# CEED/Laghos

Measured on AMD Instinct MI355X. Metric: Mdofs×steps/s on 3D Sedov -pa (Q3/Q2), higher is better.
Workload: dtype f64; 1 GPU; 3D Sedov -p 1 -m cube01_hex -rs 4 -ok 3 -ot 2 -pa (32^3 elements, E0/2^dim = 0.125); transport=none (one rank), elements=32768, h1_dofs=2738019, l2_dofs=884736, quad_points_per_element=216, rk_stages_executed=1300, ode=RK4, parallelism=elements1x1x1, zones_per_gpu=32x32x32

## Files before the change

include/laghos_hip.h:

```cpp
#ifndef LAGHOS_HIP_H
#define LAGHOS_HIP_H

#ifdef __cplusplus
extern "C" {
#endif

#define LGH_OK 0
#define LGH_ERR_ARG 1
#define LGH_ERR_UNSUPPORTED 2
#define LGH_ERR_HIP 3
#define LGH_ERR_COMM 4

#define LGH_SPACE_H1 0
#define LGH_SPACE_L2 1

typedef struct lgh_ctx lgh_ctx;

typedef struct lgh_config
{
   int dim, NE;
   int D1D, Q1D, L1D;
   int N;
   const int *h1_map;
   const double *B_h1;
   const double *G_h1;
   const double *B_l2;
   const double *weights;
   const double *gamma;
   int ess_count[3];
   const int *ess[3];
   const double *owner;
   int use_viscosity, use_vorticity;
   double cfl;
   int order_v;
   int device;
   void *stream;
} lgh_config;

const char *lgh_last_error(void);
const char *lgh_version(void);

int lgh_create(const lgh_config *cfg, lgh_ctx **out);
int lgh_destroy(lgh_ctx *ctx);
int lgh_sync(lgh_ctx *ctx);
void *lgh_stream(lgh_ctx *ctx);

double *lgh_qdata_stressJinvT(lgh_ctx *ctx);
double *lgh_qdata_Jac0inv(lgh_ctx *ctx);
double *lgh_qdata_rho0DetJ0w(lgh_ctx *ctx);
double *lgh_mass_D(lgh_ctx *ctx);
int lgh_mass_data_form(lgh_ctx *ctx, int *form);
int lgh_jac0inv_form(lgh_ctx *ctx, int *compact);
int lgh_mass_data_changed(lgh_ctx *ctx);
double *lgh_mass_diag(lgh_ctx *ctx);
int lgh_set_h0(lgh_ctx *ctx, double h0);
int lgh_get_h0(lgh_ctx *ctx, double *h0);
int lgh_set_dt_est(lgh_ctx *ctx, double dt_est);
int lgh_get_dt_est(lgh_ctx *ctx, double *dt_est);

int lgh_setup_rho0detj0(lgh_ctx *ctx, const double *x0, const double *rho0_l2,
                        const double *rho0_q, double *volume);

int lgh_force_mult(lgh_ctx *ctx, const double *x_l2, double *y_h1);
int lgh_force_mult_transpose(lgh_ctx *ctx, const double *v_h1, double *y_l2);

int lgh_mass_set_essential_tdofs(lgh_ctx *ctx, int comp);
int lgh_mass_eliminate_rhs(lgh_ctx *ctx, double *b);
int lgh_mass_mult(lgh_ctx *ctx, int space, const double *x, double *y);
int lgh_mass_mult_full(lgh_ctx *ctx, int space, const double *x, double *y);

int lgh_cg_solve(lgh_ctx *ctx, int space, const double *b, double *x, double rel_tol,
                 int max_iter, int *iters);
int lgh_l2_mass_solve_local(lgh_ctx *ctx, const double *b, double *x);

int lgh_qupdate(lgh_ctx *ctx, const double *S);
int lgh_qupdate_set_tiny_grad(lgh_ctx *ctx, double tiny_grad);
int lgh_qupdate_discard(lgh_ctx *ctx, int *mode, double *C_F);
int lgh_set_fused_forces(lgh_ctx *ctx, int on);
int lgh_qupdate_store_stress(lgh_ctx *ctx, int on);
int lgh_qupdate_stores_stress(lgh_ctx *ctx, int *on);
int lgh_qupdate_form(lgh_ctx *ctx, int *form);
int lgh_reset_quadrature_data(lgh_ctx *ctx);
int lgh_fused_force_mult(lgh_ctx *ctx, double *y_h1);
int lgh_fused_force_mult_transpose(lgh_ctx *ctx, double *y_l2);
int lgh_fused_force_e(lgh_ctx *ctx, double *y_e);
int lgh_quadrature_generation(lgh_ctx *ctx, unsigned long *gen, int *f1_valid, int *ftv_valid);
int lgh_get_fused_forces(lgh_ctx *ctx, int *f1, int *ftv);

int lgh_solve_velocity(lgh_ctx *ctx, const double *S, double *dS_dt, const double *one_l2,
                       double *rhs_h1, double *work_B, double rel_tol, int max_iter,
                       int *h1_iters);
int lgh_solve_energy(lgh_ctx *ctx, const double *S, const double *v_h1, double *dS_dt,
                     double *e_rhs, const double *e_source, double rel_tol, int max_iter,
                     int *l2_iters);
int lgh_solve_energy_begin(lgh_ctx *ctx, const double *S, const double *v_h1, double *dS_dt,
                           double *e_rhs, const double *e_source, double rel_tol, int max_iter);
int lgh_solve_energy_end(lgh_ctx *ctx, int *l2_iters);
int lgh_energy_lockstep_stats(lgh_ctx *ctx, long out[4]);

int lgh_vec_set(lgh_ctx *ctx, double *y, double a, long n);
int lgh_vec_copy(lgh_ctx *ctx, double *y, const double *x, long n);
int lgh_vec_axpby_pair(lgh_ctx *ctx, double *z1, double a1, const double *x1, double b1, double *z2, double a2, const double *x2, double b2,
                       const double *y, long n);
int lgh_vec_axpby(lgh_ctx *ctx, double *z, double a, const double *x, double b,
                  const double *y, long n);
int lgh_vec_dot(lgh_ctx *ctx, const double *x, const double *y, long n, double *result);
int lgh_vec_fingerprint(lgh_ctx *ctx, const double *x, long n, unsigned long long offset, unsigned long long out[2]);
int lgh_vec_fingerprint_shape(lgh_ctx *ctx, const double *x, long n, long out[4]);
int lgh_fingerprint_host(const void *words, long n, unsigned long long offset, unsigned long long out[2]);

int lgh_set_velocity_source(lgh_ctx *ctx, const double *accel_h1);

int lgh_tg_source_2d(lgh_ctx *ctx, const double *S, double *e_source);

int lgh_internal_energy(lgh_ctx *ctx, const double *e_l2, double *result);
int lgh_kinetic_energy(lgh_ctx *ctx, const double *v_h1, double *result);

int lgh_sedov_setup(int dim, double gamma, double rho0, double blast_energy, double omega, double par[21]);
int lgh_sedov_shock(const double par[21], double t, double shock[6]);
int lgh_sedov_eval_point(const double par[21], double t, double r, double *rho, double *v, double *P);
int lgh_sedov_eval(lgh_ctx *ctx, const double par[21], double t, long n, const double *r, double *rho, double *v,
                   double *P);
int lgh_compute_density(lgh_ctx *ctx, const double *x_h1, double *rho_l2);
int lgh_sedov_density_error(lgh_ctx *ctx, const double *x_h1, const double *rho_l2, const double par[21], double t,
                            const double origin[3], int n1d, const double *weights, const double *B_h1,
                            const double *G_h1, const double *B_l2, double *err2);

int lgh_sample_fields(lgh_ctx *ctx, const double *S, const double *rho_l2 ,
                      int R1, const double *B_h1_lat ,
                      const double *B_l2_lat ,
                      double *x_out, double *v_out, double *e_out, double *rho_out, double *p_out);

int lgh_sample_derived(lgh_ctx *ctx, const double *S, int R1, const double *B_h1_lat ,
                       const double *G_h1_lat , const double *B_l2_lat ,
                       double *detj_out, double *gradv_out, double *div_out, double *vort_out, double *cs_out);

int lgh_sample_faces(lgh_ctx *ctx, const double *S, const double *rho_l2 , int R1,
                     const double *B_h1_lat , const double *G_h1_lat ,
                     const double *B_l2_lat , int nfaces, const int *faces ,
                     double *x_out, double *v_out, double *e_out, double *rho_out, double *p_out, double *detj_out,
                     double *gradv_out, double *div_out, double *vort_out, double *cs_out, double *an_out);
int lgh_sample_faces_fpb(lgh_ctx *ctx, int R1, int *fpb);
int lgh_mesh_boundary_faces_host(int dim, int NE, int N, int D1D, const int *h1_map, int *faces_out, int *nfaces);

#define LGH_DIAG_ZONE_COUNT 17
#define LGH_DIAG_COUNT 20
int lgh_diagnostics_zones(lgh_ctx *ctx, const double *S, double *zone_out);
int lgh_diagnostics(lgh_ctx *ctx, const double *S, double out[LGH_DIAG_COUNT]);

#define LGH_PROFILE_COLS 10
#define LGH_PROFILE_MAX_BINS 4096
typedef struct lgh_profile_spec {
   int axis;
   int nbins;
   double lo, hi;
   double origin[3];
} lgh_profile_spec;
int lgh_profile(lgh_ctx *ctx, const double *S, const lgh_profile_spec *spec, double *out, long *n_excluded);

#define LGH_MAP_COLS 11
#define LGH_MAP_MAX_CELLS (1 << 20)
typedef struct lgh_map_spec {
   int n[3];
   double lo[3], hi[3];
} lgh_map_spec;
int lgh_map(lgh_ctx *ctx, const double *S, const lgh_map_spec *spec,
            double *out , long *n_excluded);

int lgh_get_timers(lgh_ctx *ctx, double t[4], long c[3]);
int lgh_reset_timers(lgh_ctx *ctx);
int lgh_enable_timers(lgh_ctx *ctx, int on);

#define LGH_KERNEL_MASS_CG_H1 0
#define LGH_KERNEL_CG_UPDATE_H1 1
#define LGH_KERNEL_QUPDATE 2
#define LGH_KERNEL_FORCE_MULT 3
#define LGH_KERNEL_FORCE_MULT_T 4
#define LGH_KERNEL_MASS_CG_L2 5
#define LGH_KERNEL_HALO 6
#define LGH_KERNEL_ALLREDUCE 7
#define LGH_KERNEL_SAMPLE 8
#define LGH_KERNEL_FINGERPRINT 9
#define LGH_KERNEL_DIAG 10
#define LGH_KERNEL_PROFILE 11
#define LGH_KERNEL_DERIVED 12
#define LGH_KERNEL_MAP 13
#define LGH_KERNEL_FACES 14
int lgh_ktime_begin(lgh_ctx *ctx, int which, int max_samples);
int lgh_ktime_end(lgh_ctx *ctx, int *launches, double *mean_seconds);
int lgh_table_symmetry(lgh_ctx *ctx, int *h1, int *l2);
int lgh_k1_form(lgh_ctx *ctx, int *form);
int lgh_l2_mass_form(lgh_ctx *ctx, int *form, int *compact);
int lgh_vcg_layout_stats(lgh_ctx *ctx, long out[4]);

int lgh_mesh_order(lgh_ctx *ctx, long out[8]);
int lgh_mesh_order_host(int dim, int NE, int N, int D1D, const int *h1_map, int *zorder, int *nnum, long out[8]);

int lgh_comm_unique_id(char id_out[128]);
int lgh_comm_init(lgh_ctx *ctx, int nranks, int rank, const char unique_id[128]);
int lgh_comm_unique_id_shm(char id_out[128]);
int lgh_comm_set_neighbors(lgh_ctx *ctx, int n_nbr, const int *nbr_rank, const int *nbr_count,
                           const int *const *nbr_nodes);
int lgh_comm_stats(lgh_ctx *ctx, int *n_neighbours, long *max_nodes_per_neighbour, long *shared_nodes, int *all_pairs,
                   int *second_channel);
int lgh_groups_to_neighbors(int my_rank, int N, int n_groups, const int *group_off, const int *group_ranks,
                            const int *group_master, const int *ldof_off, const int *ldofs, double *owner,
                            int *n_nbr, int *nbr_rank, int *nbr_count, int cap_nbr, int *nbr_nodes, long cap_nodes);
int lgh_halo_sum(lgh_ctx *ctx, double *v_h1, int ncomp);
int lgh_allreduce(lgh_ctx *ctx, double *value, int op);

int lgh_force_mult_E(lgh_ctx *ctx, const double *sJit, const double *x_E, double *y_E);
int lgh_force_mult_transpose_E(lgh_ctx *ctx, const double *sJit, const double *v_E, double *y_E);
int lgh_mass_apply_E(lgh_ctx *ctx, int space, const double *x_E, double *y_E);
int lgh_test_vcg_k1(lgh_ctx *ctx, const double *r, const double *d_old, const double rz[3], const double rz_prev[3],
                    int first, double *y_E, double den[3]);
int lgh_test_vcg_merged_faces(lgh_ctx *ctx, unsigned char *mask, long *n_merged);
int lgh_test_vcg_k2(lgh_ctx *ctx, int it, const double *y_E, double *r, double *d, double *x, const double den[3],
                    const double rz[3], const double rz_prev[3], const double alpha_prev[3], double rz_out[3],
                    int *deferred_x);
int lgh_test_exact_sum(lgh_ctx *ctx, int mode, long n, int G, int E, const double *scale, const double *v,
                       const long long *w_in, long long *w_out, double *d_out, int *i_out);
int lgh_test_set_rank(lgh_ctx *ctx, int nranks, int rank);
int lgh_test_halo_pack(lgh_ctx *ctx, const double *v_h1, int ncomp, double *sendbuf_out);
int lgh_test_halo_combine(lgh_ctx *ctx, const double *recvbuf_in, double *v_h1, int ncomp);
int lgh_test_word_peers(lgh_ctx *ctx, int nwords, long *capacity_words);
int lgh_test_rccl_self_sendrecv(lgh_ctx *ctx, int n, double *max_abs_diff);
int lgh_test_eig(lgh_ctx *ctx, int dim, int n, const double *A, double *lambda, double *vec);
int lgh_test_sqrt(lgh_ctx *ctx, int n, const double *x, double *y);
int lgh_test_singular(lgh_ctx *ctx, int dim, int n, const double *A, double *sv_min);

#ifdef __cplusplus
}
#endif
#endif
```

laghos_amd/_lib.py:

```python
import ctypes
import os

_HERE = os.path.dirname(os.path.abspath(__file__))
LIB_PATH = os.path.join(_HERE, "liblaghos_hip.so")

c_dp = ctypes.c_void_p
c_int_p = ctypes.POINTER(ctypes.c_int)
c_dbl_p = ctypes.POINTER(ctypes.c_double)


class LghConfig(ctypes.Structure):
    _fields_ = [
        ("dim", ctypes.c_int), ("NE", ctypes.c_int),
        ("D1D", ctypes.c_int), ("Q1D", ctypes.c_int), ("L1D", ctypes.c_int),
        ("N", ctypes.c_int),
        ("h1_map", c_int_p),
        ("B_h1", c_dbl_p), ("G_h1", c_dbl_p), ("B_l2", c_dbl_p),
        ("weights", c_dbl_p), ("gamma", c_dbl_p),
        ("ess_count", ctypes.c_int * 3),
        ("ess", c_int_p * 3),
        ("owner", c_dbl_p),
        ("use_viscosity", ctypes.c_int), ("use_vorticity", ctypes.c_int),
        ("cfl", ctypes.c_double),
        ("order_v", ctypes.c_int),
        ("device", ctypes.c_int),
        ("stream", ctypes.c_void_p),
    ]


class LghProfileSpec(ctypes.Structure):
    _fields_ = [("axis", ctypes.c_int), ("nbins", ctypes.c_int), ("lo", ctypes.c_double), ("hi", ctypes.c_double),
                ("origin", ctypes.c_double * 3)]


class LghMapSpec(ctypes.Structure):
    _fields_ = [("n", ctypes.c_int * 3), ("lo", ctypes.c_double * 3), ("hi", ctypes.c_double * 3)]


_I, _D, _P, _L = ctypes.c_int, ctypes.c_double, ctypes.c_void_p, ctypes.c_long
SYMBOLS = {
    "lgh_last_error": (ctypes.c_char_p, []),
    "lgh_version": (ctypes.c_char_p, []),
    "lgh_create": (_I, [ctypes.POINTER(LghConfig), ctypes.POINTER(_P)]),
    "lgh_destroy": (_I, [_P]),
    "lgh_sync": (_I, [_P]),
    "lgh_stream": (_P, [_P]),
    "lgh_qdata_stressJinvT": (_P, [_P]),
    "lgh_qdata_Jac0inv": (_P, [_P]),
    "lgh_qdata_rho0DetJ0w": (_P, [_P]),
    "lgh_mass_D": (_P, [_P]),
    "lgh_mass_diag": (_P, [_P]),
    "lgh_set_h0": (_I, [_P, _D]),
    "lgh_get_h0": (_I, [_P, c_dbl_p]),
    "lgh_set_dt_est": (_I, [_P, _D]),
    "lgh_get_dt_est": (_I, [_P, c_dbl_p]),
    "lgh_setup_rho0detj0": (_I, [_P, _P, _P, _P, c_dbl_p]),
    "lgh_force_mult": (_I, [_P, _P, _P]),
    "lgh_force_mult_transpose": (_I, [_P, _P, _P]),
    "lgh_mass_set_essential_tdofs": (_I, [_P, _I]),
    "lgh_mass_eliminate_rhs": (_I, [_P, _P]),
    "lgh_mass_mult": (_I, [_P, _I, _P, _P]),
    "lgh_mass_mult_full": (_I, [_P, _I, _P, _P]),
    "lgh_cg_solve": (_I, [_P, _I, _P, _P, _D, _I, c_int_p]),
    "lgh_l2_mass_solve_local": (_I, [_P, _P, _P]),
    "lgh_qupdate": (_I, [_P, _P]),
    "lgh_solve_velocity": (_I, [_P, _P, _P, _P, _P, _P, _D, _I, c_int_p]),
    "lgh_solve_energy": (_I, [_P, _P, _P, _P, _P, _P, _D, _I, c_int_p]),
    "lgh_solve_energy_begin": (_I, [_P, _P, _P, _P, _P, _P, _D, _I]),
    "lgh_tg_source_2d": (_I, [_P, _P, _P]),
    "lgh_set_velocity_source": (_I, [_P, _P]),
    "lgh_solve_energy_end": (_I, [_P, c_int_p]),
    "lgh_vec_set": (_I, [_P, _P, _D, _L]),
    "lgh_vec_copy": (_I, [_P, _P, _P, _L]),
    "lgh_vec_axpby": (_I, [_P, _P, _D, _P, _D, _P, _L]),
    "lgh_vec_axpby_pair": (_I, [_P, _P, _D, _P, _D, _P, _D, _P, _D, _P, _L]),
    "lgh_vec_dot": (_I, [_P, _P, _P, _L, c_dbl_p]),
    "lgh_vec_fingerprint": (_I, [_P, _P, _L, ctypes.c_ulonglong, ctypes.POINTER(ctypes.c_ulonglong)]),
    "lgh_vec_fingerprint_shape": (_I, [_P, _P, _L, ctypes.POINTER(ctypes.c_long)]),
    "lgh_fingerprint_host": (_I, [_P, _L, ctypes.c_ulonglong, ctypes.POINTER(ctypes.c_ulonglong)]),
    "lgh_internal_energy": (_I, [_P, _P, c_dbl_p]),
    "lgh_kinetic_energy": (_I, [_P, _P, c_dbl_p]),
    "lgh_sedov_setup": (_I, [_I, _D, _D, _D, _D, c_dbl_p]),
    "lgh_sedov_shock": (_I, [c_dbl_p, _D, c_dbl_p]),
    "lgh_sedov_eval_point": (_I, [c_dbl_p, _D, _D, c_dbl_p, c_dbl_p, c_dbl_p]),
    "lgh_sedov_eval": (_I, [_P, c_dbl_p, _D, _L, _P, _P, _P, _P]),
    "lgh_compute_density": (_I, [_P, _P, _P]),
    "lgh_sedov_density_error": (_I, [_P, _P, _P, c_dbl_p, _D, c_dbl_p, _I, c_dbl_p, c_dbl_p, c_dbl_p, c_dbl_p, c_dbl_p]),
    "lgh_sample_fields": (_I, [_P, _P, _P, _I, c_dbl_p, c_dbl_p, _P, _P, _P, _P, _P]),
    "lgh_sample_derived": (_I, [_P, _P, _I, c_dbl_p, c_dbl_p, c_dbl_p, _P, _P, _P, _P, _P]),
    "lgh_sample_faces": (_I, [_P, _P, _P, _I, c_dbl_p, c_dbl_p, c_dbl_p, _I, c_int_p] + [_P] * 11),
    "lgh_sample_faces_fpb": (_I, [_P, _I, ctypes.POINTER(_I)]),
    "lgh_mesh_boundary_faces_host": (_I, [_I, _I, _I, _I, c_int_p, c_int_p, ctypes.POINTER(_I)]),
    "lgh_diagnostics_zones": (_I, [_P, _P, _P]),
    "lgh_diagnostics": (_I, [_P, _P, c_dbl_p]),
    "lgh_profile": (_I, [_P, _P, ctypes.POINTER(LghProfileSpec), c_dbl_p, ctypes.POINTER(ctypes.c_long)]),
    "lgh_map": (_I, [_P, _P, ctypes.POINTER(LghMapSpec), c_dbl_p, ctypes.POINTER(ctypes.c_long)]),
    "lgh_get_timers": (_I, [_P, c_dbl_p, ctypes.POINTER(ctypes.c_long)]),
    "lgh_reset_timers": (_I, [_P]),
    "lgh_enable_timers": (_I, [_P, _I]),
    "lgh_ktime_begin": (_I, [_P, _I, _I]),
    "lgh_ktime_end": (_I, [_P, c_int_p, c_dbl_p]),
    "lgh_table_symmetry": (_I, [_P, c_int_p, c_int_p]),
    "lgh_k1_form": (_I, [_P, c_int_p]),
    "lgh_l2_mass_form": (_I, [_P, c_int_p, c_int_p]),
    "lgh_vcg_layout_stats": (_I, [_P, ctypes.POINTER(ctypes.c_long)]),
    "lgh_energy_lockstep_stats": (_I, [_P, ctypes.POINTER(ctypes.c_long)]),
    "lgh_mesh_order": (_I, [_P, ctypes.POINTER(ctypes.c_long)]),
    "lgh_mesh_order_host": (_I, [_I, _I, _I, _I, c_int_p, c_int_p, c_int_p, ctypes.POINTER(ctypes.c_long)]),
    "lgh_mass_data_form": (_I, [_P, c_int_p]),
    "lgh_jac0inv_form": (_I, [_P, c_int_p]),
    "lgh_mass_data_changed": (_I, [_P]),
    "lgh_comm_stats": (_I, [_P, c_int_p, ctypes.POINTER(ctypes.c_long), ctypes.POINTER(ctypes.c_long), c_int_p, c_int_p]),
    "lgh_qupdate_set_tiny_grad": (_I, [_P, _D]),
    "lgh_qupdate_discard": (_I, [_P, c_int_p, c_dbl_p]),
    "lgh_set_fused_forces": (_I, [_P, _I]),
    "lgh_qupdate_store_stress": (_I, [_P, _I]),
    "lgh_qupdate_stores_stress": (_I, [_P, c_int_p]),
    "lgh_qupdate_form": (_I, [_P, c_int_p]),
    "lgh_reset_quadrature_data": (_I, [_P]),
    "lgh_fused_force_mult": (_I, [_P, _P]),
    "lgh_fused_force_mult_transpose": (_I, [_P, _P]),
    "lgh_fused_force_e": (_I, [_P, _P]),
    "lgh_quadrature_generation": (_I, [_P, ctypes.POINTER(ctypes.c_ulong), c_int_p, c_int_p]),
    "lgh_get_fused_forces": (_I, [_P, c_int_p, c_int_p]),
    "lgh_comm_unique_id": (_I, [ctypes.c_char_p]),
    "lgh_comm_unique_id_shm": (_I, [ctypes.c_char_p]),
    "lgh_comm_init": (_I, [_P, _I, _I, ctypes.c_char_p]),
    "lgh_comm_set_neighbors": (_I, [_P, _I, c_int_p, c_int_p, ctypes.POINTER(c_int_p)]),
    "lgh_groups_to_neighbors": (_I, [_I, _I, _I, c_int_p, c_int_p, c_int_p, c_int_p, c_int_p, c_dbl_p, c_int_p, c_int_p,
                                     c_int_p, _I, c_int_p, _L]),
    "lgh_halo_sum": (_I, [_P, _P, _I]),
    "lgh_allreduce": (_I, [_P, c_dbl_p, _I]),
    "lgh_force_mult_E": (_I, [_P, _P, _P, _P]),
    "lgh_force_mult_transpose_E": (_I, [_P, _P, _P, _P]),
    "lgh_mass_apply_E": (_I, [_P, _I, _P, _P]),
    "lgh_test_vcg_k1": (_I, [_P, _P, _P, c_dbl_p, c_dbl_p, _I, _P, c_dbl_p]),
    "lgh_test_vcg_merged_faces": (_I, [_P, _P, ctypes.POINTER(ctypes.c_long)]),
    "lgh_test_vcg_k2": (_I, [_P, _I, _P, _P, _P, _P, c_dbl_p, c_dbl_p, c_dbl_p, c_dbl_p, c_dbl_p, ctypes.POINTER(ctypes.c_int)]),
    "lgh_test_exact_sum": (_I, [_P, _I, _L, _I, _I, c_dbl_p, c_dbl_p, ctypes.POINTER(ctypes.c_longlong),
                                ctypes.POINTER(ctypes.c_longlong), c_dbl_p, c_int_p]),
    "lgh_test_set_rank": (_I, [_P, _I, _I]),
    "lgh_test_word_peers": (_I, [_P, _I, ctypes.POINTER(ctypes.c_long)]),
    "lgh_test_halo_pack": (_I, [_P, _P, _I, _P]),
    "lgh_test_halo_combine": (_I, [_P, _P, _P, _I]),
    "lgh_test_rccl_self_sendrecv": (_I, [_P, _I, c_dbl_p]),
    "lgh_test_eig": (_I, [_P, _I, _I, _P, _P, _P]),
    "lgh_test_singular": (_I, [_P, _I, _I, _P, _P]),
    "lgh_test_sqrt": (_I, [_P, _I, _P, _P]),
}

_lib = None


def _preload_torch_hip():
    try:
        import torch
    except Exception:
        pass


def load():
    global _lib
    if _lib is None:
        _preload_torch_hip()
        if not os.path.exists(LIB_PATH):
            raise RuntimeError(
                f"{LIB_PATH} is missing: build it with `python -c 'import __graft_entry__ as g; "
                "g.build()'` (hipcc --offload-arch=gfx950).  There is no CPU fallback.")
        lib = ctypes.CDLL(LIB_PATH)
        for name, (res, args) in SYMBOLS.items():
            fn = getattr(lib, name)
            fn.restype = res
            fn.argtypes = args
        _lib = lib
    return _lib


class LghError(RuntimeError):
    pass


def check(rc):
    if rc != 0:
        raise LghError(f"laghos_hip error {rc}: {load().lgh_last_error().decode()}")
```

laghos_amd/context.py:

```python
import ctypes

import numpy as np
import torch

from . import _lib
from ._lib import LghConfig, check


def _np_i32(a):
    return np.ascontiguousarray(a, dtype=np.int32)


def _np_f64(a):
    return np.ascontiguousarray(a, dtype=np.float64)


def _ptr(t):
    assert t.is_cuda and t.dtype == torch.float64 and t.is_contiguous()
    return ctypes.c_void_p(t.data_ptr())


def _dbl(a):
    assert isinstance(a, np.ndarray) and a.dtype == np.float64 and a.flags.c_contiguous
    return a.ctypes.data_as(_lib.c_dbl_p)
# ... 339 lines not shown
        return out

    def mass_data_form(self):
        f = ctypes.c_int(-1)
        check(self.lib.lgh_mass_data_form(self.h, ctypes.byref(f)))
        return "rank1" if f.value == 1 else "stored"

    def jac0inv_form(self):
        f = ctypes.c_int(-1)
        check(self.lib.lgh_jac0inv_form(self.h, ctypes.byref(f)))
        return "compact" if f.value == 1 else "stored"

    def qupdate_store_stress(self, on):
        check(self.lib.lgh_qupdate_store_stress(self.h, int(bool(on))))

    def set_fused_forces(self, on):
        check(self.lib.lgh_set_fused_forces(self.h, 1 if on else 0))

    def reset_quadrature_data(self):
        check(self.lib.lgh_reset_quadrature_data(self.h))

    def fused_force_mult(self, y_h1):
        return self.lib.lgh_fused_force_mult(self.h, _ptr(y_h1)) == 0

    def fused_force_e(self, y_e):
        return self.lib.lgh_fused_force_e(self.h, _ptr(y_e)) == 0

    def fused_force_mult_transpose(self, y_l2):
        return self.lib.lgh_fused_force_mult_transpose(self.h, _ptr(y_l2)) == 0

    def quadrature_generation(self):
        g, a, b = ctypes.c_ulong(0), ctypes.c_int(-1), ctypes.c_int(-1)
        check(self.lib.lgh_quadrature_generation(self.h, ctypes.byref(g), ctypes.byref(a), ctypes.byref(b)))
        return g.value, a.value, b.value

    def solve_velocity(self, S, dS, one, rhs, work, rel_tol, max_iter):
        it = ctypes.c_int(0)
        check(self.lib.lgh_solve_velocity(self.h, _ptr(S), _ptr(dS), _ptr(one) if one is not None else None, _ptr(rhs), _ptr(work),
                                          rel_tol, max_iter, ctypes.byref(it)))
        return it.value

    def solve_energy(self, S, v, dS, e_rhs, rel_tol, max_iter, e_source=None):
        it = ctypes.c_int(0)
        check(self.lib.lgh_solve_energy(self.h, _ptr(S), _ptr(v), _ptr(dS), _ptr(e_rhs),
                                        _ptr(e_source) if e_source is not None else None,
                                        rel_tol, max_iter, ctypes.byref(it)))
        return it.value

    def set_velocity_source(self, accel):
        check(self.lib.lgh_set_velocity_source(self.h, _ptr(accel) if accel is not None else None))

    def tg_source_2d(self, S, out):
        check(self.lib.lgh_tg_source_2d(self.h, _ptr(S), _ptr(out)))

    def compute_density(self, x, rho_l2):
        check(self.lib.lgh_compute_density(self.h, _ptr(x), _ptr(rho_l2)))

    def sedov_eval(self, par, t, r, rho, v, P):
        check(self.lib.lgh_sedov_eval(self.h, _dbl(par), float(t), r.numel(), _ptr(r), _ptr(rho), _ptr(v), _ptr(P)))

    def sedov_density_error(self, x, rho_l2, par, t, origin, weights, B_h1, G_h1, B_l2):
        import numpy as np
        w = np.ascontiguousarray(weights, dtype=np.float64)
        tabs = [np.ascontiguousarray(a, dtype=np.float64).ravel() for a in (B_h1, G_h1, B_l2)]
        org = np.zeros(3)
        org[:len(origin)] = origin
        out = ctypes.c_double()
        check(self.lib.lgh_sedov_density_error(self.h, _ptr(x), _ptr(rho_l2), _dbl(par), float(t), _dbl(org),
                                               int(w.size), _dbl(w), _dbl(tabs[0]), _dbl(tabs[1]), _dbl(tabs[2]),
                                               ctypes.byref(out)))
        return out.value

    def sample_fields(self, S, rho_l2, B_h1_lat, B_l2_lat, x=None, v=None, e=None, rho=None, p=None):
        Bh = _np_f64(np.asarray(B_h1_lat).T.reshape(-1))
        Bl = _np_f64(np.asarray(B_l2_lat).T.reshape(-1))
        R1 = int(np.asarray(B_h1_lat).shape[0])
        opt = lambda t: _ptr(t) if t is not None else None
        check(self.lib.lgh_sample_fields(self.h, _ptr(S), opt(rho_l2), R1, _dbl(Bh), _dbl(Bl), opt(x), opt(v), opt(e), opt(rho),
                                         opt(p)))

    def sample_derived(self, S, B_h1_lat, G_h1_lat, B_l2_lat, detj=None, grad_v=None, div_v=None, vorticity=None, sound_speed=None):
        Bh = _np_f64(np.asarray(B_h1_lat).T.reshape(-1))
        Gh = _np_f64(np.asarray(G_h1_lat).T.reshape(-1))
        Bl = _np_f64(np.asarray(B_l2_lat).T.reshape(-1))
        R1 = int(np.asarray(B_h1_lat).shape[0])
        opt = lambda t: _ptr(t) if t is not None else None
        check(self.lib.lgh_sample_derived(self.h, _ptr(S), R1, _dbl(Bh), _dbl(Gh), _dbl(Bl), opt(detj), opt(grad_v), opt(div_v), opt(vorticity),
                                          opt(sound_speed)))

    def sample_faces(self, S, rho_l2, B_h1_lat, G_h1_lat, B_l2_lat, faces, x=None, v=None, e=None, rho=None, p=None, detj=None, grad_v=None,
                     div_v=None, vorticity=None, sound_speed=None, area_normal=None):
        tab = lambda T: None if T is None else _np_f64(np.asarray(T).T.reshape(-1))
        Bh, Gh, Bl = tab(B_h1_lat), tab(G_h1_lat), tab(B_l2_lat)
        R1 = int(np.asarray(next(T for T in (B_h1_lat, G_h1_lat, B_l2_lat) if T is not None)).shape[0])
        f = np.ascontiguousarray(np.asarray(faces, dtype=np.int32).reshape(-1))
        assert f.size % 2 == 0
        opt = lambda t: _ptr(t) if t is not None else None
        dbl = lambda a: _dbl(a) if a is not None else None
        fp = f.ctypes.data_as(ctypes.POINTER(ctypes.c_int)) if f.size else None
        check(self.lib.lgh_sample_faces(self.h, _ptr(S), opt(rho_l2), R1, dbl(Bh), dbl(Gh), dbl(Bl), f.size // 2, fp, opt(x), opt(v), opt(e),
                                        opt(rho), opt(p), opt(detj), opt(grad_v), opt(div_v), opt(vorticity), opt(sound_speed), opt(area_normal)))

    def faces_per_block(self, R1):
        n = ctypes.c_int(-1)
        check(self.lib.lgh_sample_faces_fpb(self.h, int(R1), ctypes.byref(n)))
        return n.value

    def boundary_faces(self):
        return boundary_faces_host(self.dim, self.NE, self.N, self.D1D, self._keep["h1"])

    def diagnostics_zones(self, S, out):
        assert out.numel() == DIAG_ZONE_COUNT * self.NE
        check(self.lib.lgh_diagnostics_zones(self.h, _ptr(S), _ptr(out)))

    def diagnostics(self, S, raw=False):
        out = np.full(DIAG_COUNT, np.nan)
        check(self.lib.lgh_diagnostics(self.h, _ptr(S), _dbl(out)))
        return out if raw else diagnostics_dict(out)

    def profile(self, S, axis, nbins, lo, hi, origin=None):
        from ._lib import LghProfileSpec
        spec = LghProfileSpec()
        spec.axis, spec.nbins, spec.lo, spec.hi = int(PROFILE_AXES.get(axis, axis)), int(nbins), float(lo), float(hi)
        o = np.zeros(3) if origin is None else np.asarray(origin, dtype=np.float64).reshape(-1)
        for k in range(min(3, o.size)):
            spec.origin[k] = float(o[k])
        n_rows = max(0, min(int(nbins), PROFILE_MAX_BINS)) + 2
        rows = np.full((n_rows, len(PROFILE_COLS)), np.nan)
        n_excl = ctypes.c_long(-1)
        check(self.lib.lgh_profile(self.h, _ptr(S), ctypes.byref(spec), _dbl(rows), ctypes.byref(n_excl)))
        return profile_dict(rows, n_excl.value, spec.lo, spec.hi)

    def map(self, S, cells, lo, hi):
        from ._lib import LghMapSpec
        n, a, b, n_rows = map_spec(cells, lo, hi)
        spec = LghMapSpec()
        for k in range(3):
            spec.n[k], spec.lo[k], spec.hi[k] = n[k], a[k], b[k]
        rows = np.full((n_rows, len(MAP_COLS)), np.nan)
        n_excl = ctypes.c_long(-1)
        check(self.lib.lgh_map(self.h, _ptr(S), ctypes.byref(spec), _dbl(rows), ctypes.byref(n_excl)))
        return map_dict(rows, n_excl.value, self.dim, n, a, b)

    def solve_energy_begin(self, S, v, dS, e_rhs, rel_tol, max_iter, e_source=None):
        check(self.lib.lgh_solve_energy_begin(self.h, _ptr(S), _ptr(v), _ptr(dS), _ptr(e_rhs),
                                              _ptr(e_source) if e_source is not None else None,
                                              rel_tol, max_iter))

    def solve_energy_end(self):
        it = ctypes.c_int(0)
        check(self.lib.lgh_solve_energy_end(self.h, ctypes.byref(it)))
        return it.value

    def vec_axpby(self, z, a, x, b, y):
        check(self.lib.lgh_vec_axpby(self.h, _ptr(z), a, _ptr(x), b, _ptr(y), z.numel()))

    def vec_axpby_pair(self, z1, a1, x1, b1, z2, a2, x2, b2, y):
        check(self.lib.lgh_vec_axpby_pair(self.h, _ptr(z1), a1, _ptr(x1), b1, _ptr(z2), a2, _ptr(x2), b2, _ptr(y), z1.numel()))

    def vec_copy(self, y, x):
        check(self.lib.lgh_vec_copy(self.h, _ptr(y), _ptr(x), y.numel()))

    def vec_dot(self, x, y):
        v = ctypes.c_double()
        check(self.lib.lgh_vec_dot(self.h, _ptr(x), _ptr(y), x.numel(), ctypes.byref(v)))
        return v.value

    def fingerprint(self, t, offset=0):
        out = (ctypes.c_ulonglong * 2)()
        check(self.lib.lgh_vec_fingerprint(self.h, _ptr(t), t.numel(), int(offset), out))
        return int(out[0]), int(out[1])

    def fingerprint_shape(self, t):
        out = (ctypes.c_long * 4)()
        check(self.lib.lgh_vec_fingerprint_shape(self.h, _ptr(t), t.numel(), out))
        return tuple(out)

    def internal_energy(self, e):
        v = ctypes.c_double()
        check(self.lib.lgh_internal_energy(self.h, _ptr(e), ctypes.byref(v)))
        return v.value

    def kinetic_energy(self, vel):
        v = ctypes.c_double()
        check(self.lib.lgh_kinetic_energy(self.h, _ptr(vel), ctypes.byref(v)))
        return v.value

    def timers(self):
        t = (ctypes.c_double * 4)()
        c = (ctypes.c_long * 3)()
        check(self.lib.lgh_get_timers(self.h, t, c))
        return dict(cgH1=t[0], cgL2=t[1], force=t[2], qdata=t[3], H1iter=c[0], L2iter=c[1],
                    quad_tstep=c[2])

    def reset_timers(self):
        check(self.lib.lgh_reset_timers(self.h))

    def enable_timers(self, on):
        check(self.lib.lgh_enable_timers(self.h, int(on)))

    def force_mult_E(self, sJit, xE, yE):
        check(self.lib.lgh_force_mult_E(self.h, _ptr(sJit), _ptr(xE), _ptr(yE)))

    def force_mult_transpose_E(self, sJit, vE, yE):
        check(self.lib.lgh_force_mult_transpose_E(self.h, _ptr(sJit), _ptr(vE), _ptr(yE)))

    def mass_apply_E(self, space, xE, yE):
        check(self.lib.lgh_mass_apply_E(self.h, space, _ptr(xE), _ptr(yE)))

    def test_eig(self, dim, A, lam, vec):
        check(self.lib.lgh_test_eig(self.h, dim, lam.numel(), _ptr(A), _ptr(lam), _ptr(vec)))

    def test_singular(self, dim, A, sv):
        check(self.lib.lgh_test_singular(self.h, dim, sv.numel(), _ptr(A), _ptr(sv)))

    def test_sqrt(self, x, y):
        check(self.lib.lgh_test_sqrt(self.h, y.numel(), _ptr(x), _ptr(y)))

    def comm_init(self, nranks, rank, unique_id):
        check(self.lib.lgh_comm_init(self.h, nranks, rank, unique_id))

    def comm_set_neighbors(self, nbr_rank, nbr_nodes):
        n = len(nbr_rank)
        ranks = _np_i32(nbr_rank) if n else np.zeros(1, np.int32)
        counts = _np_i32([len(x) for x in nbr_nodes]) if n else np.zeros(1, np.int32)
        lists = [_np_i32(x) for x in nbr_nodes]
        ip = ctypes.POINTER(ctypes.c_int)
        arr = (ip * max(n, 1))(*[l.ctypes.data_as(ip) for l in lists])
        check(self.lib.lgh_comm_set_neighbors(self.h, n, ranks.ctypes.data_as(ip), counts.ctypes.data_as(ip), arr))

    def test_word_peers(self, nwords):
        cap = ctypes.c_long(-1)
        check(self.lib.lgh_test_word_peers(self.h, nwords, ctypes.byref(cap)))
        return cap.value

    def test_set_rank(self, nranks, rank):
        check(self.lib.lgh_test_set_rank(self.h, nranks, rank))

    def test_halo_pack(self, v, ncomp, out):
        check(self.lib.lgh_test_halo_pack(self.h, _ptr(v), ncomp, _ptr(out)))

    def test_halo_combine(self, inp, v, ncomp):
        check(self.lib.lgh_test_halo_combine(self.h, _ptr(inp), _ptr(v), ncomp))

    def halo_sum(self, v, ncomp):
        check(self.lib.lgh_halo_sum(self.h, _ptr(v), ncomp))

    def allreduce(self, value, op=0):
        v = ctypes.c_double(value)
        check(self.lib.lgh_allreduce(self.h, ctypes.byref(v), op))
        return v.value


def unique_id():
    buf = ctypes.create_string_buffer(128)
    check(_lib.load().lgh_comm_unique_id(buf))
    return buf.raw
```

laghos_amd/csrc/lgh_api.hip:

```cpp
#include <cstdarg>
#include <cstdlib>
#include <cmath>
#include <algorithm>
#include <limits>

#include "lgh_comm_transport.hpp"
#include "lgh_vcg.hpp"

#include <atomic>
#include <chrono>
#include <dlfcn.h>

namespace lgh
{

static thread_local char g_err[512] = "";
void set_error(const char *fmt, ...)
{
   va_list ap;
   va_start(ap, fmt);
   vsnprintf(g_err, sizeof(g_err), fmt, ap);
   va_end(ap);
}

// ... 689 lines not shown
int lgh_quadrature_generation(lgh_ctx *c, unsigned long *gen, int *f1_valid, int *ftv_valid)
{
   LGH_CHECK_ARG(c && gen && f1_valid && ftv_valid);
   *gen = c->qgen;
   *f1_valid = c->fused_f1_valid;
   *ftv_valid = c->fused_ftv_valid;
   return LGH_OK;
}
double *lgh_qdata_Jac0inv(lgh_ctx *c) { return c->Jac0inv; }
double *lgh_qdata_rho0DetJ0w(lgh_ctx *c) { return c->rho0DetJ0w; }
double *lgh_mass_D(lgh_ctx *c)
{
   c->mass_rank1 = -1;
   c->mass_gen++;
   return c->massD;
}
int lgh_mass_data_form(lgh_ctx *c, int *form)
{
   LGH_CHECK_ARG(c && form);
   if (c->dim == 1) { *form = 0; return LGH_OK; }
   const double *Dq, *Se;
   int dqs;
   int rc = mass_data(c, &Dq, &dqs, &Se);
   if (rc) { return rc; }
   *form = (c->mass_rank1 == 1) ? 1 : 0;
   return LGH_OK;
}
int lgh_mass_data_changed(lgh_ctx *c)
{
   LGH_CHECK_ARG(c);
   c->mass_rank1 = -1;
   c->mass_gen++;
   if (c->dim == 1) { return mass_changed_1d(c); }
   return mass_assemble_diag(c);
}
double *lgh_mass_diag(lgh_ctx *c) { return c->diagV; }
int lgh_set_h0(lgh_ctx *c, double h0) { LGH_CHECK_ARG(c); c->h0 = h0; return LGH_OK; }
int lgh_get_h0(lgh_ctx *c, double *h0) { LGH_CHECK_ARG(c && h0); *h0 = c->h0; return LGH_OK; }

int lgh_set_dt_est(lgh_ctx *c, double v)
{
   LGH_CHECK_ARG(c);
   hipLaunchKernelGGL(dt_est_set_k, dim3(1), dim3(256), 0, c->stream, c->dt_est_dev, v);
   LGH_HIP_CHECK(hipGetLastError());
   return LGH_OK;
}
int lgh_get_dt_est(lgh_ctx *c, double *v)
{
   LGH_CHECK_ARG(c && v);
   const unsigned long long token = ++c->look_token;
   hipLaunchKernelGGL(dt_est_fold_k, dim3(1), dim3(256), 0, c->stream, c->dt_est_dev, c->dev_flags + 4, c->host_pinned_dev + kPinDt, token);
   LGH_HIP_CHECK(hipGetLastError());
   {
      const int rc = host_wait_token(c, (volatile unsigned long long *)(c->host_pinned + kPinDtToken), token);
      if (rc) { return rc; }
   }
   *v = c->host_pinned[kPinDt];
   if (*(const int *)(c->host_pinned + kPinDtFlag) != 0)
   {
      LGH_HIP_CHECK(hipMemsetAsync(c->dev_flags + 4, 0, sizeof(int), c->stream));
      set_error("lgh_solve_energy was given a velocity other than the state's while the stress was kept in registers "
                "(lgh_qupdate_store_stress(ctx, 0)): its right-hand side is NaN");
      return LGH_ERR_ARG;
   }
   return LGH_OK;
}

int lgh_setup_rho0detj0(lgh_ctx *c, const double *x0, const double *rho0_l2, const double *rho0_q,
                        double *volume)
{
   LGH_CHECK_ARG(c && x0 && rho0_l2 && rho0_q && volume);
   invalidate_fused(c);
   c->mass_rank1 = -1;
   c->mass_gen++;
   int rc = (c->dim == 1) ? setup_1d(c, x0, rho0_l2, rho0_q, volume)
                          : setup_rho0detj0(c, x0, rho0_l2, rho0_q, volume);
   if (rc) { return rc; }
   if (c->dim != 1) { rc = mass_assemble_diag(c); }
   if (rc == LGH_OK) { c->setup_done = 1; }
   return rc;
}

int lgh_force_mult(lgh_ctx *c, const double *x_l2, double *y_h1)
{
   LGH_CHECK_ARG(c && x_l2 && y_h1);
   int rc = stress_on_hand(c, "lgh_force_mult");
   if (rc) { return rc; }
   if (c->dim == 1) { return force_mult_1d(c, x_l2, y_h1); }
   kt_begin(c, LGH_KERNEL_FORCE_MULT);
   rc = force_mult_E(c, c->stressJinvT, x_l2, c->YE);
   kt_end(c, LGH_KERNEL_FORCE_MULT);
   if (rc) { return rc; }
   rc = h1_transpose_gather(c, c->dim, c->YE, y_h1);
   if (rc) { return rc; }
   if (c->multi != 0) { rc = halo_sum(c, y_h1, c->dim); }
   return rc;
}
int lgh_force_mult_transpose(lgh_ctx *c, const double *v_h1, double *y_l2)
{
   LGH_CHECK_ARG(c && v_h1 && y_l2);
   const int rc0 = stress_on_hand(c, "lgh_force_mult_transpose");
   if (rc0) { return rc0; }
   if (c->dim == 1) { return force_mult_t_1d(c, v_h1, y_l2); }
   kt_begin(c, LGH_KERNEL_FORCE_MULT_T);
   const int rc = force_mult_t_L(c, c->stressJinvT, v_h1, y_l2);
   kt_end(c, LGH_KERNEL_FORCE_MULT_T);
   return rc;
}

int lgh_mass_set_essential_tdofs(lgh_ctx *c, int comp)
{
   LGH_CHECK_ARG(c && comp >= -1 && comp < c->dim);
   c->cur_ess = comp;
   return LGH_OK;
}
int lgh_mass_eliminate_rhs(lgh_ctx *c, double *b)
{
   LGH_CHECK_ARG(c && b);
   if (c->cur_ess < 0) { return LGH_OK; }
   return vec_zero_list(c, b, c->ess[c->cur_ess], c->ess_count[c->cur_ess]);
}
int lgh_mass_mult(lgh_ctx *c, int space, const double *x, double *y)
{
   LGH_CHECK_ARG(c && x && y && (space == LGH_SPACE_H1 || space == LGH_SPACE_L2));
   if (c->dim == 1) { return mass_apply_1d(c, space, x, y, true); }
   return space == LGH_SPACE_H1 ? mass_apply_h1(c, x, y, true) : mass_apply_l2(c, x, y);
}
int lgh_mass_mult_full(lgh_ctx *c, int space, const double *x, double *y)
{
   LGH_CHECK_ARG(c && x && y && (space == LGH_SPACE_H1 || space == LGH_SPACE_L2));
   if (c->dim == 1) { return mass_apply_1d(c, space, x, y, false); }
   return space == LGH_SPACE_H1 ? mass_apply_h1(c, x, y, false) : mass_apply_l2(c, x, y);
}

int lgh_cg_solve(lgh_ctx *c, int space, const double *b, double *x, double rel_tol, int max_iter,
                 int *iters)
{
   LGH_CHECK_ARG(c && b && x && (space == LGH_SPACE_H1 || space == LGH_SPACE_L2));
   if (c->dim == 1) { return cg_1d(c, space, b, x, rel_tol, max_iter, iters, false); }
   return cg_solve(c, space, b, x, rel_tol, max_iter, iters, false);
}

int lgh_l2_mass_solve_local(lgh_ctx *c, const double *b, double *x)
{
   LGH_CHECK_ARG(c && b && x);
   if (c->dim != 1)
   {
      set_error("lgh_l2_mass_solve_local: the zone-local energy solve belongs to the 1D (full-assembly) path; 2D/3D run the energy CG");
      return LGH_ERR_UNSUPPORTED;
   }
   return l2_solve_local_1d(c, b, x);
}

int lgh_qupdate(lgh_ctx *c, const double *S)
{
   LGH_CHECK_ARG(c && S);
   RoctxRange range("QUpdate-UpdateQuadratureData");
   timer_start(c);
   kt_begin(c, LGH_KERNEL_QUPDATE);
   int rc = (c->dim == 1) ? qupdate_1d(c, S) : qupdate(c, S);
   kt_end(c, LGH_KERNEL_QUPDATE);
   timer_stop(c, 3);
   c->timers.c[2] += c->NE;
   return rc;
}

__global__ void __launch_bounds__(256) not_all_ones_k(const double *x, const long n, int *flag)
{
   const long i = (long)blockIdx.x * blockDim.x + threadIdx.x;
   if (i < n && x[i] != 1.0) { *flag = 1; }
}
static bool is_the_one_vector(lgh_ctx *c, const double *one_l2)
{
   if (!one_l2) { return true; }
   int *flag = c->dev_flags + 1;
   if (hipMemsetAsync(flag, 0, sizeof(int), c->stream) != hipSuccess) { return false; }
   hipLaunchKernelGGL(not_all_ones_k, dim3(ceil_div(c->L2V, 256)), dim3(256), 0, c->stream, one_l2, (long)c->L2V, flag);
   int h = 1;
   if (hipMemcpyAsync(&h, flag, sizeof(int), hipMemcpyDeviceToHost, c->stream) != hipSuccess) { return false; }
   if (hipStreamSynchronize(c->stream) != hipSuccess) { return false; }
   return h == 0;
}
static int one_vector(lgh_ctx *c, const double *one_l2, const double **out)
{
   if (one_l2) { *out = one_l2; return LGH_OK; }
   if (!c->ones_l2)
   {
      LGH_PASS(c->ones_l2.alloc((size_t)c->L2V));
      const int rc = vec_set(c, c->ones_l2, 1.0, c->L2V);
      if (rc) { return rc; }
   }
   *out = c->ones_l2;
   return LGH_OK;
}

int lgh_solve_velocity(lgh_ctx *c, const double *S, double *dS_dt, const double *one_l2,
                       double *rhs_h1, double *work_B, double rel_tol, int max_iter, int *h1_iters)
{
   LGH_CHECK_ARG(c && S && dS_dt && rhs_h1 && work_B);
   const int dim = c->dim, N = c->N;
   double *dv = dS_dt + c->H1V;
   int rc;
   if (dim == 1)
   {
      LGH_CHECK_ARG(!c->accel_src);
      const double *ones = nullptr;
      rc = one_vector(c, one_l2, &ones);
      if (rc) { return rc; }
      rc = stress_on_hand(c, "lgh_solve_velocity");
      if (rc) { return rc; }
      return solve_velocity_1d(c, ones, dv, rhs_h1, rel_tol, max_iter, h1_iters);
   }
   if (!c->timers.enabled && !c->accel_src && vcg_fused_init_ok(c))
   {
      const double *force_E = c->YE;
      if (c->force_e_q && c->fused_f1_valid && is_the_one_vector(c, one_l2)) { force_E = c->force_e_q; }
      else
      {
         const double *ones = nullptr;
         rc = one_vector(c, one_l2, &ones);
         if (rc) { return rc; }
         rc = stress_on_hand(c, "lgh_solve_velocity (F.1 of a vector other than one, or of changed quadrature data)");
         if (rc) { return rc; }
         kt_begin(c, LGH_KERNEL_FORCE_MULT);
         rc = force_mult_E(c, c->stressJinvT, ones, c->YE);
         kt_end(c, LGH_KERNEL_FORCE_MULT);
         if (rc) { return rc; }
      }
      int its[3] = {0, 0, 0};
      RoctxRange range("SolveVelocity-CGVMass");
      rc = vcg_solve(c, rhs_h1, dv, rel_tol, max_iter, its, force_E);
      if (rc) { return rc; }
      for (int cc = 0; cc < dim; cc++)
      {
         c->timers.c[0] += its[cc];
         if (h1_iters) { *h1_iters += its[cc]; }
      }
      c->cur_ess = dim - 1;
      return LGH_OK;
   }
   rc = vec_set(c, dv, 0.0, c->H1V);
   if (rc) { return rc; }
   {
   RoctxRange range("SolveVelocity-ForcePA");
   timer_start(c);
   if (c->force_e_q && c->fused_f1_valid && is_the_one_vector(c, one_l2))
   {
      rc = h1_transpose_gather(c, c->dim, c->force_e_q, rhs_h1);
      if (rc == LGH_OK && c->multi != 0) { rc = halo_sum(c, rhs_h1, c->dim); }
   }
   else
   {
      const double *ones = nullptr;
      rc = one_vector(c, one_l2, &ones);
      if (rc == LGH_OK) { rc = lgh_force_mult(c, ones, rhs_h1); }
   }
   timer_stop(c, 2);
   }
   if (rc) { return rc; }
   rc = vec_neg_inplace(c, rhs_h1, c->H1V);
   if (rc) { return rc; }
   if (c->accel_src)
   {
      for (int cc = 0; cc < dim; cc++)
      {
         rc = mass_apply_h1(c, c->accel_src + (size_t)cc * N, work_B, false);
         if (rc) { return rc; }
         rc = vec_axpby(c, rhs_h1 + (size_t)cc * N, 1.0, rhs_h1 + (size_t)cc * N, 1.0, work_B, N);
         if (rc) { return rc; }
      }
   }
   {
      for (int cc = 0; cc < dim; cc++)
      {
         rc = vec_zero_list(c, rhs_h1 + (size_t)cc * N, c->ess[cc], c->ess_count[cc]);
         if (rc) { return rc; }
      }
      int its[3] = {0, 0, 0};
      RoctxRange range("SolveVelocity-CGVMass");
      timer_start(c);
      rc = vcg_solve(c, rhs_h1, dv, rel_tol, max_iter, its);
      if (rc == LGH_OK)
      {
         timer_stop(c, 0);
         for (int cc = 0; cc < dim; cc++)
         {
            c->timers.c[0] += its[cc];
            if (h1_iters) { *h1_iters += its[cc]; }
         }
         c->cur_ess = dim - 1;
         return LGH_OK;
      }
      if (rc != LGH_ERR_UNSUPPORTED) { return rc; }
   }
   for (int cc = 0; cc < dim; cc++)
   {
      LGH_HIP_CHECK(hipMemcpyAsync(work_B, rhs_h1 + (size_t)cc * N, sizeof(double) * N,
                                   hipMemcpyDeviceToDevice, c->stream));
      rc = lgh_mass_set_essential_tdofs(c, cc);
      if (rc) { return rc; }
      rc = lgh_mass_eliminate_rhs(c, work_B);
      if (rc) { return rc; }
      int it = 0;
      timer_start(c);
      rc = cg_solve(c, LGH_SPACE_H1, work_B, dv + (size_t)cc * N, rel_tol, max_iter, &it, true);
      timer_stop(c, 0);
      if (rc) { return rc; }
      c->timers.c[0] += it;
      if (h1_iters) { *h1_iters += it; }
   }
   return LGH_OK;
}

int lgh_vec_set(lgh_ctx *c, double *y, double a, long n) { LGH_CHECK_ARG(c && y); return vec_set(c, y, a, n); }
int lgh_vec_copy(lgh_ctx *c, double *y, const double *x, long n)
{
   LGH_CHECK_ARG(c && y && x);
   LGH_HIP_CHECK(hipMemcpyAsync(y, x, sizeof(double) * n, hipMemcpyDeviceToDevice, c->stream));
   return LGH_OK;
}
int lgh_vec_axpby(lgh_ctx *c, double *z, double a, const double *x, double b, const double *y, long n)
{
   LGH_CHECK_ARG(c && z && x && y);
   return vec_axpby(c, z, a, x, b, y, n);
}
int lgh_vec_axpby_pair(lgh_ctx *c, double *z1, double a1, const double *x1, double b1, double *z2, double a2, const double *x2, double b2,
                       const double *y, long n)
{
   LGH_CHECK_ARG(c && z1 && x1 && z2 && x2 && y && n >= 0);
   {
      auto overlap = [n](const double *p, const double *q) { return p < q + n && q < p + n; };
      LGH_CHECK_ARG(!overlap(z1, z2) && !overlap(z1, x2) && !overlap(z1, y));
      LGH_CHECK_ARG(!overlap(z2, y) && !overlap(z2, x1) && (z2 == x2 || !overlap(z2, x2)) && (z1 == x1 || !overlap(z1, x1)));
   }
   return vec_axpby_pair(c, z1, a1, x1, b1, z2, a2, x2, b2, y, n);
}
int lgh_vec_dot(lgh_ctx *c, const double *x, const double *y, long n, double *result)
{
   LGH_CHECK_ARG(c && x && y && result);
   int rc = vec_dot(c, x, y, nullptr, n, c->scal + 1);
   if (rc) { return rc; }
   LGH_HIP_CHECK(hipMemcpyAsync(c->host_pinned + kPinDot, c->scal + 1, sizeof(double), hipMemcpyDeviceToHost, c->stream));
   LGH_HIP_CHECK(hipStreamSynchronize(c->stream));
   *result = c->host_pinned[kPinDot];
   return LGH_OK;
}

int lgh_set_velocity_source(lgh_ctx *c, const double *accel_h1)
{
   LGH_CHECK_ARG(c);
   if (accel_h1)
   {
      const int rc = no_1d(c, "lgh_set_velocity_source");
      if (rc) { return rc; }
   }
   c->accel_src = accel_h1;
   return LGH_OK;
}

int lgh_tg_source_2d(lgh_ctx *c, const double *S, double *e_source)
{
   LGH_CHECK_ARG(c && S && e_source);
   const int rc = no_1d(c, "lgh_tg_source_2d");
   if (rc) { return rc; }
   return tg_source_2d(c, S, e_source);
}

int lgh_internal_energy(lgh_ctx *c, const double *e_l2, double *result)
{
   LGH_CHECK_ARG(c && e_l2 && result);
   if (c->dim == 1) { return energy_1d(c, 0, e_l2, result); }
   return interp_energy(c, 0, e_l2, result);
}
int lgh_kinetic_energy(lgh_ctx *c, const double *v_h1, double *result)
{
   LGH_CHECK_ARG(c && v_h1 && result);
   if (c->dim == 1) { return energy_1d(c, 1, v_h1, result); }
   return interp_energy(c, 1, v_h1, result);
}

int lgh_get_timers(lgh_ctx *c, double t[4], long n[3])
{
   LGH_CHECK_ARG(c && t && n);
   for (int i = 0; i < 4; i++) { t[i] = c->timers.t[i]; }
   for (int i = 0; i < 3; i++) { n[i] = c->timers.c[i]; }
   return LGH_OK;
}
int lgh_reset_timers(lgh_ctx *c)
{
   LGH_CHECK_ARG(c);
   for (int i = 0; i < 4; i++) { c->timers.t[i] = 0; }
   for (int i = 0; i < 3; i++) { c->timers.c[i] = 0; }
   return LGH_OK;
}
int lgh_enable_timers(lgh_ctx *c, int on)
{
   LGH_CHECK_ARG(c);
   c->timers.enabled = on != 0;
   return LGH_OK;
}

int lgh_ktime_begin(lgh_ctx *c, int which, int max_samples)
{
   LGH_CHECK_ARG(c && which >= 0 && max_samples > 0);
   if (!c->ktime) { c->ktime.reset(new KTime()); }
   KTime *k = c->ktime.get();
   while ((int)k->ev.size() < 2 * max_samples)
   {
      hipEvent_t e;
      LGH_HIP_CHECK(hipEventCreate(&e));
      k->ev.push_back(e);
   }
   k->which = which;
   k->max = max_samples;
   k->n = 0;
   return LGH_OK;
}
int lgh_ktime_end(lgh_ctx *c, int *launches, double *mean_seconds)
{
   LGH_CHECK_ARG(c && launches && mean_seconds && c->ktime);
   KTime *k = c->ktime.get();
   LGH_HIP_CHECK(hipStreamSynchronize(c->stream));
   double tot = 0.0;
   for (int i = 0; i < k->n; i++)
   {
      float ms = 0.f;
      LGH_HIP_CHECK(hipEventElapsedTime(&ms, k->ev[2 * i], k->ev[2 * i + 1]));
      tot += 1e-3 * ms;
   }
   *launches = k->n;
   *mean_seconds = k->n ? tot / k->n : 0.0;
   k->which = -1;
   return LGH_OK;
}

int lgh_set_fused_forces(lgh_ctx *c, int on)
{
   LGH_CHECK_ARG(c);
   if (c->fused_forces_off == (on ? 0 : 1)) { return LGH_OK; }
   c->fused_forces_off = on ? 0 : 1;
   invalidate_fused(c);
   return LGH_OK;
}

int lgh_get_fused_forces(lgh_ctx *c, int *f1, int *ftv)
{
   LGH_CHECK_ARG(c && f1 && ftv);
   *f1 = (c->force_e_q && !c->fused_forces_off) ? 1 : 0;
   *ftv = (c->erhs_q && !c->fused_forces_off) ? 1 : 0;
   return LGH_OK;
}

int lgh_qupdate_set_tiny_grad(lgh_ctx *c, double tiny_grad)
{
   LGH_CHECK_ARG(c);
   c->q_tiny_grad = tiny_grad;
   return LGH_OK;
}

int lgh_table_symmetry(lgh_ctx *c, int *h1, int *l2)
{
   LGH_CHECK_ARG(c && h1 && l2);
   *h1 = c->b_h1_sym;
   *l2 = c->b_l2_sym;
   return LGH_OK;
// ... 100 lines not shown
```

laghos_amd/csrc/lgh_common.hpp:

```cpp
#pragma once
#include <hip/hip_runtime.h>

#include <algorithm>
#include <cstdint>
#include <cstdio>
#include <cstring>
#include <memory>
#include <string>
#include <vector>

#include "../../include/laghos_hip.h"

namespace lgh
{

void set_error(const char *fmt, ...);

#define LGH_HIP_CHECK(expr)                                                              \
   do                                                                                    \
   {                                                                                     \
      hipError_t e_ = (expr);                                                            \
      if (e_ != hipSuccess)                                                              \
      {                                                                                  \
         lgh::set_error("HIP error %s at %s:%d: %s", hipGetErrorName(e_), __FILE__,      \
// ... 7 lines not shown
   {                                                                                     \
      if (!(cond))                                                                       \
      {                                                                                  \
         lgh::set_error("bad argument: %s (%s:%d)", #cond, __FILE__, __LINE__);          \
         return LGH_ERR_ARG;                                                             \
      }                                                                                  \
   } while (0)

#define LGH_PASS(call) do { const int rc_ = (call); if (rc_ != LGH_OK) { return rc_; } } while (0)

constexpr int kWave = 64;

template <typename T> struct DevPtr
{
   T *p = nullptr;
   DevPtr() = default;
   DevPtr(DevPtr &&o) noexcept : p(o.p) { o.p = nullptr; }
   DevPtr &operator=(DevPtr &&o) noexcept { std::swap(p, o.p); return *this; }
   ~DevPtr() { reset(); }
   operator T *() const { return p; }
   T *operator->() const { return p; }
   void reset() { if (p) { (void)hipFree(p); p = nullptr; } }
   int alloc(const size_t n, const bool zero = false)
   {
      reset();
      LGH_HIP_CHECK(hipMalloc((void **)&p, n * sizeof(T)));
      if (zero)
      {
         LGH_HIP_CHECK(hipMemset(p, 0, n * sizeof(T)));
         LGH_HIP_CHECK(hipStreamSynchronize(nullptr));
      }
      return LGH_OK;
   }
   int upload(const T *host, const size_t n)
   {
      const int rc = alloc(n);
      if (rc != LGH_OK) { return rc; }
      LGH_HIP_CHECK(hipMemcpy(p, host, n * sizeof(T), hipMemcpyHostToDevice));
      return LGH_OK;
   }
};
template <typename T> int ctx_buffer(DevPtr<T> &d, const size_t n, const T *src = nullptr)
{
   const int rc = d.alloc(std::max<size_t>(n, 1), !src);
   if (rc != LGH_OK || !src || !n) { return rc; }
   LGH_HIP_CHECK(hipMemcpy(d.p, src, n * sizeof(T), hipMemcpyHostToDevice));
   return LGH_OK;
}

struct CgScalars
{
   double rz;
   double rz_prev;
   double den;
   double r0;
   double nom0;
   double rel_tol2;
   int done;
   int iters;
   int first;
   int pad;
};

constexpr int kPinDoubles = 96;
constexpr int kPinResult = 0;
constexpr int kPinDot = 1;
constexpr int kPinReduceOut = 2, kPinReduceIn = 3;
constexpr int kPinDt = 8, kPinDtFlag = 9, kPinDtToken = 10;
constexpr int kPinVcg = 32;
constexpr int kPinVcgToken = 80;
static_assert(sizeof(CgScalars) <= kPinDt * sizeof(double) && kPinDtFlag == kPinDt + 1 && kPinDtToken == kPinDt + 2 && kPinDtToken < kPinVcg &&
              kPinVcgToken < kPinDoubles, "slots of the pinned block: disjoint, inside the allocation");

struct Timers
{
   bool enabled = true;
   hipEvent_t ev[2] = {nullptr, nullptr};
   Timers() = default;
   Timers(const Timers &) = delete;
   Timers &operator=(const Timers &) = delete;
   ~Timers() { for (hipEvent_t e : ev) { if (e) { (void)hipEventDestroy(e); } } }
   double t[4] = {0, 0, 0, 0};
   long c[3] = {0, 0, 0};
};

struct KTime
{
   int which = -1, max = 0, n = 0;
   std::vector<hipEvent_t> ev;
   KTime() = default;
   KTime(const KTime &) = delete;
   KTime &operator=(const KTime &) = delete;
   ~KTime() { for (hipEvent_t e : ev) { (void)hipEventDestroy(e); } }
};

struct Comm;
struct VcgScalars;
struct VcgAux;

struct MeshOrder
{
   bool structured = false, identity = true;
   int components = 0, extent[3] = {0, 0, 0};
   std::vector<int> zorder;
   std::vector<int> nnum;
   std::vector<int> ncaller;
   DevPtr<int> zorder_d, ncaller_d, nnum_d;
};

constexpr double kMassRank1Tol = 1e-12;
constexpr double kJac0Tol = 1e-12;

struct Switches
{
   int vcg_variant;
   int slab_wide, slab_exact, slab_merge, slab_defer, slab_ye_wide;
   int slab_dyn;
   int rz_limbs, kron_neb, fused_init;
   int k2p, k2_skip, k2_grid;
   long k2_node_weight;
   int order, order_multi;
   int comm2;
   int force_multi, halo_piggyback, halo_fused_pack, overlap, energy_lockstep, spin;
   int mass_sep, mass_kron, mass_rank1, l2_neb, l2_plane, l2_fused;
   double mass_rank1_tol;
   int q_form, q_ppt, q_swz, fused_ftv, fused_f1, b_sym, jac0_compact;
   int q_occ4;
   int q_discard;
   double q_tiny_grad;
   double jac0_tol;
   int profile_fold;
   int map_fold;
   int roctx, vcg_trace_phases, q_trace_call;
   std::string vcg_trace, q_trace;
};
Switches read_switches();

struct ScalarCg;
void cg_l2_free(ScalarCg *r);

struct EnergySolve
{
   enum Mode
   {
      Idle,
      Overlapped,
      Deferred,
      Lockstep
   };
   Mode mode = Idle;
   bool polled = false;
   int iters = 0;
   struct { const double *S, *v; double *dS, *e_rhs; const double *src; double tol; int maxit; } args = {};
};

struct CtxHandles
{
   int device = 0;
   hipStream_t stream = nullptr;
   bool own_stream = false;
   hipStream_t stream2 = nullptr;
   hipEvent_t ev_fork = nullptr, ev_join = nullptr;
   double *host_pinned = nullptr;
   double *host_pinned_dev = nullptr;
   CtxHandles() = default;
   CtxHandles(const CtxHandles &) = delete;
   CtxHandles &operator=(const CtxHandles &) = delete;
   ~CtxHandles();
};

}

struct lgh_ctx : lgh::CtxHandles
{
   lgh_ctx();
   ~lgh_ctx();
   lgh::Switches sw;
   int dim = 0, NE = 0, D1D = 0, Q1D = 0, L1D = 0, ND = 0, NQ = 0, NL = 0, N = 0, H1V = 0, L2V = 0;
   int kid = 0;
   bool visc = false, vort = false;
   double cfl = 0.0, h0 = 0.0, h1order = 0.0;
   double q_tiny_grad = 0.0;
   int q_discard = 0;
   double q_cF = 0.0;
   int on_stream2 = 0;
   std::unique_ptr<lgh::ScalarCg, void (*)(lgh::ScalarCg *)> l2run{nullptr, lgh::cg_l2_free};
   const double *accel_src = nullptr;
   lgh::EnergySolve energy;
   long ls_stats[3] = {0, 0, 0};

   lgh::DevPtr<double> B, G, Bl, W, gamma;
   lgh::DevPtr<int> h1map;
   lgh::DevPtr<int> t_off;
   lgh::DevPtr<int> t_idx;
   lgh::DevPtr<int> t_ell;
   int t_deg = 0;
   lgh::DevPtr<uint8_t> essmask[3];
   lgh::DevPtr<int> ess[3];
   int ess_count[3] = {0, 0, 0};
   lgh::DevPtr<double> owner;
   int cur_ess = -1;

   lgh::DevPtr<double> stressJinvT, Jac0inv, rho0DetJ0w, massD, diagV, dinvV;
   lgh::DevPtr<double> Jac0inv_soa;
   lgh::DevPtr<double> Jac0inv_e;
   int jac0_compact = 0;
   lgh::DevPtr<double> massS, ones_ne;
   lgh::DevPtr<double> M1h, M1l;
   lgh::DevPtr<double> w1d;
   int mass_rank1 = -1;
   lgh::DevPtr<double> dt_est_dev;
   lgh::DevPtr<double> erhs_q;
   lgh::DevPtr<double> v_snap;
   lgh::DevPtr<double> force_e_q;
   int fused_ftv_valid = 0, fused_f1_valid = 0;
   unsigned long qgen = 0;
   lgh::DevPtr<int> dev_flags;
   lgh::DevPtr<double> ones_l2;
   int stress_store = 1;
   int stress_current = 0;
   int fused_forces_off = 0;
   lgh::DevPtr<double> XE;
   lgh::DevPtr<double> YE;
   lgh::DevPtr<double> cg_r, cg_z, cg_d0, cg_d1, cg_y;
   lgh::DevPtr<double> partials;
   int part_stride = 0;
   lgh::DevPtr<unsigned int> tickets;
   lgh::DevPtr<lgh::CgScalars> cgs;
   lgh::DevPtr<double> scal;
   unsigned long long look_token = 0;

   lgh::DevPtr<lgh::VcgScalars> vcg_s;
   lgh::DevPtr<double> vcg_vec, vcg_partials;
   lgh::DevPtr<unsigned int> vcg_tickets;
   unsigned vcg_stride = 0;
   int vcg_last = 0;
   int vcg_grid = 0;
   int b_h1_sym = 0, b_l2_sym = 0;
   int ncu = 0;
   std::unique_ptr<lgh::VcgAux> vcg_aux;

   lgh::Timers timers;
   std::unique_ptr<lgh::KTime> ktime;
   int cg_last_iters[2][3] = {{0, 0, 0}, {0, 0, 0}};
   std::unique_ptr<lgh::Comm> comm;
   int nranks = 1, rank = 0;
   int multi = 0;
   lgh::DevPtr<unsigned long long> q_trace_dev;
   int q_trace_n = 0, q_trace_calls = 0;
   std::unique_ptr<lgh::MeshOrder> order;
   unsigned long mass_gen = 0;
   lgh::DevPtr<double> me_fac;
   int setup_done = 0;
   lgh::DevPtr<double> diag_dev;
   lgh::DevPtr<char> prof_dev;
   int prof_rows = 0;
   lgh::DevPtr<char> map_dev;
   int map_rows = 0;
   lgh::DevPtr<int> faces_dev;
   int faces_cap = 0;
   lgh::DevPtr<unsigned long long> fp_dev;
};

namespace lgh
{

template <int CTRL, int ROW_MASK>
__device__ __forceinline__ double dpp_f64(const double old, const double src)
{
   const int lo = __builtin_amdgcn_update_dpp(__double2loint(old), __double2loint(src), CTRL, ROW_MASK, 0xF, false);
   const int hi = __builtin_amdgcn_update_dpp(__double2hiint(old), __double2hiint(src), CTRL, ROW_MASK, 0xF, false);
   return __hiloint2double(hi, lo);
}
__device__ __forceinline__ double wave_bcast_f64(const double v, const int src_lane )
{
   const int lo = __builtin_amdgcn_readlane(__double2loint(v), src_lane);
   const int hi = __builtin_amdgcn_readlane(__double2hiint(v), src_lane);
   return __hiloint2double(hi, lo);
}
__device__ __forceinline__ double wave_sum(double v, const int lane, const int nact)
{
   (void)lane;
   v += dpp_f64<0x111, 0xF>(0.0, v);
   v += dpp_f64<0x112, 0xF>(0.0, v);
   v += dpp_f64<0x114, 0xF>(0.0, v);
   v += dpp_f64<0x118, 0xF>(0.0, v);
   v += dpp_f64<0x142, 0xA>(0.0, v);
   v += dpp_f64<0x143, 0xC>(0.0, v);
   return wave_bcast_f64(v, nact - 1);
}
__device__ __forceinline__ double wave_min(double v, const int lane, const int nact)
{
   (void)lane;
   v = fmin(v, dpp_f64<0x111, 0xF>(v, v));
   v = fmin(v, dpp_f64<0x112, 0xF>(v, v));
   v = fmin(v, dpp_f64<0x114, 0xF>(v, v));
   v = fmin(v, dpp_f64<0x118, 0xF>(v, v));
   v = fmin(v, dpp_f64<0x142, 0xA>(v, v));
   v = fmin(v, dpp_f64<0x143, 0xC>(v, v));
   return wave_bcast_f64(v, nact - 1);
}

__device__ __forceinline__ double uniform_f64(const double v)
{
   const int lo = __builtin_amdgcn_readfirstlane(__double2loint(v));
   const int hi = __builtin_amdgcn_readfirstlane(__double2hiint(v));
// ... 20 lines not shown
__device__ __forceinline__ void block_sum3(const double v0, const double v1, const double v2, double *red, double out[3])
{
   const int tid = threadIdx.x + blockDim.x * (threadIdx.y + blockDim.y * threadIdx.z);
   const int nthr = blockDim.x * blockDim.y * blockDim.z;
   const int lane = tid & 63, wid = tid >> 6, nw = (nthr + 63) >> 6;
   const int nact = min(64, nthr - (wid << 6));
   const double a0 = wave_sum(v0, lane, nact), a1 = wave_sum(v1, lane, nact), a2 = wave_sum(v2, lane, nact);
   __syncthreads();
   if (lane == 0)
   {
      red[3 * wid + 0] = a0;
      red[3 * wid + 1] = a1;
      red[3 * wid + 2] = a2;
   }
   __syncthreads();
   out[0] = out[1] = out[2] = 0.0;
   if (tid == 0)
   {
      for (int w = 0; w < nw; w++)
      {
         out[0] += red[3 * w + 0];
         out[1] += red[3 * w + 1];
         out[2] += red[3 * w + 2];
      }
   }
   __syncthreads();
}
__device__ __forceinline__ double block_min(double v, double *red)
{
   const int tid = threadIdx.x + blockDim.x * (threadIdx.y + blockDim.y * threadIdx.z);
   const int nthr = blockDim.x * blockDim.y * blockDim.z;
   const int lane = tid & 63, wid = tid >> 6, nw = (nthr + 63) >> 6;
   const int nact = min(64, nthr - (wid << 6));
   v = wave_min(v, lane, nact);
   __syncthreads();
   if (lane == 0) { red[wid] = v; }
   __syncthreads();
   double s = v;
   if (tid == 0)
   {
      s = red[0];
      for (int w = 1; w < nw; w++) { s = fmin(s, red[w]); }
   }
   return s;
}

#if defined(__HIP_DEVICE_COMPILE__) && !defined(__gfx950__) && !defined(__gfx942__) && !defined(__gfx90a__)
#error "lgh_common.hpp: the grid reductions rely on gfx9-family vmcnt / sc1 semantics (see comment)"
#endif
constexpr unsigned kShards = 64;
constexpr unsigned kTicketStride = 32;
constexpr unsigned kTicketSlot = (kShards + 1) * kTicketStride;

template <bool IS_MIN>
__device__ __forceinline__ bool grid_reduce_last_block(double block_partial ,
                                                       double *partials, const unsigned shard_off,
                                                       unsigned int *ticket, double *red, double &total)
{
   const int tid = threadIdx.x + blockDim.x * (threadIdx.y + blockDim.y * threadIdx.z);
   const int nthr = blockDim.x * blockDim.y * blockDim.z;
   const unsigned int nblk = gridDim.x * gridDim.y * gridDim.z;
   const unsigned int bid = blockIdx.x + gridDim.x * (blockIdx.y + gridDim.y * blockIdx.z);
   const unsigned s = bid % kShards;
   const unsigned cnt = nblk / kShards + ((s < nblk % kShards) ? 1u : 0u);
   const unsigned nsh = nblk < kShards ? nblk : kShards;
   unsigned int *t1 = ticket + s * kTicketStride;
   unsigned int *t2 = ticket + kShards * kTicketStride;
   const double ident = IS_MIN ? INFINITY : 0.0;
   __shared__ unsigned int s_flag;
   if (tid == 0)
   {
      __hip_atomic_store(&partials[bid], block_partial, __ATOMIC_RELAXED, __HIP_MEMORY_SCOPE_AGENT);
      asm volatile("s_waitcnt vmcnt(0)" ::: "memory");
      const unsigned a = __hip_atomic_fetch_add(t1, 1u, __ATOMIC_RELAXED, __HIP_MEMORY_SCOPE_AGENT);
      s_flag = (a == cnt - 1) ? 1u : 0u;
   }
   __syncthreads();
   if (!s_flag) { return false; }
   double v = ident;
   for (unsigned int i = tid; i < cnt; i += nthr)
   {
      const double p = __hip_atomic_load(&partials[s + kShards * i], __ATOMIC_RELAXED, __HIP_MEMORY_SCOPE_AGENT);
      v = IS_MIN ? fmin(v, p) : v + p;
   }
   const double ssum = IS_MIN ? block_min(v, red) : block_sum(v, red);
   __syncthreads();
   if (tid == 0)
   {
      __hip_atomic_store(&partials[shard_off + s], ssum, __ATOMIC_RELAXED, __HIP_MEMORY_SCOPE_AGENT);
      asm volatile("s_waitcnt vmcnt(0)" ::: "memory");
      __hip_atomic_store(t1, 0u, __ATOMIC_RELAXED, __HIP_MEMORY_SCOPE_AGENT);
      const unsigned b = __hip_atomic_fetch_add(t2, 1u, __ATOMIC_RELAXED, __HIP_MEMORY_SCOPE_AGENT);
      s_flag = (b == nsh - 1) ? 1u : 0u;
      if (s_flag) { __hip_atomic_store(t2, 0u, __ATOMIC_RELAXED, __HIP_MEMORY_SCOPE_AGENT); }
   }
   __syncthreads();
   if (!s_flag) { return false; }
   v = ident;
   for (unsigned int i = tid; i < nsh; i += nthr)
   {
      const double p = __hip_atomic_load(&partials[shard_off + i], __ATOMIC_RELAXED, __HIP_MEMORY_SCOPE_AGENT);
      v = IS_MIN ? fmin(v, p) : v + p;
   }
   total = IS_MIN ? block_min(v, red) : block_sum(v, red);
   return true;
}
__device__ __forceinline__ bool grid_sum_last_block(double bp, double *partials, unsigned int *ticket,
                                                    double *red, double &total)
{
   const unsigned nblk = gridDim.x * gridDim.y * gridDim.z;
   return grid_reduce_last_block<false>(bp, partials, nblk, ticket, red, total);
}
__device__ __forceinline__ bool grid_min_last_block(double bp, double *partials, unsigned int *ticket,
                                                    double *red, double &total)
{
   const unsigned nblk = gridDim.x * gridDim.y * gridDim.z;
   return grid_reduce_last_block<true>(bp, partials, nblk, ticket, red, total);
}

__device__ __forceinline__ int xcd_swizzle(const int b, const int nblocks)
{
   const int per = nblocks >> 3;
   const int main = per << 3;
   if (b >= main) { return b; }
   return (b & 7) * per + (b >> 3);
}

inline int ceil_div(long a, long b) { return (int)((a + b - 1) / b); }
inline int grid_for(long n) { return (int)std::min<long>(std::max<long>((n + 255) / 256, 1), 2048); }

int mesh_order_build(lgh_ctx *c, const int *map_host);
inline const MeshOrder *mesh_order(const lgh_ctx *c)
{
   const MeshOrder *o = c->order.get();
   return (o && !o->identity) ? o : nullptr;
}
int order_gather_nodes(lgh_ctx *c, const double *in, double *out, int ncomp);
int order_scatter_nodes(lgh_ctx *c, const double *in, double *out, int ncomp);
int order_gather_bytes(lgh_ctx *c, const uint8_t *in, uint8_t *out);
int order_zone_blocks(lgh_ctx *c, const double *in, double *out, int per, bool to_caller);

int force_mult_E(lgh_ctx *c, const double *sJit, const double *xE, double *yE);
int force_mult_t_L(lgh_ctx *c, const double *sJit, const double *v_h1, double *y_l2, const int *guard = nullptr);
int force_mult_t_E(lgh_ctx *c, const double *sJit, const double *vE, double *y_l2);
int h1_transpose_gather(lgh_ctx *c, int ncomp, const double *YE, double *yL);
int mass_apply_h1(lgh_ctx *c, const double *x, double *y, bool eliminate);
int mass_apply_l2(lgh_ctx *c, const double *x, double *y);
int mass_apply_E(lgh_ctx *c, int space, const double *xE, double *yE);
int mass_assemble_diag(lgh_ctx *c);
int qupdate_form(lgh_ctx *c);
int mass_data(lgh_ctx *c, const double **Dq, int *dqs, const double **Se);
int l2_mass_form(lgh_ctx *c, int *form, int *compact);
int vcg_solve(lgh_ctx *c, double *B, double *X, double rel_tol, int max_iter, int iters[3],
              const double *force_E = nullptr);
bool vcg_fused_init_ok(const lgh_ctx *c);
int partition_nodes_by_cost(lgh_ctx *c, int W, DevPtr<int> &out, const std::vector<int> *valence = nullptr);
int make_ellz(lgh_ctx *c, DevPtr<unsigned> &out, const int *ell = nullptr, int deg = 0);
int vcg_test_merged_faces(lgh_ctx *c, unsigned char *mask, long *n_merged);
int vcg_layout_stats(lgh_ctx *c, long out[4]);
int make_essbits(lgh_ctx *c, DevPtr<uint8_t> &out);
void vcg_free(lgh_ctx *c);
constexpr int kDtSlots = 256, kDtSlotStride = 16;
constexpr int kDtHint = 1;
enum { kQDiscardDt = 1, kQDiscardF1 = 2 };
constexpr int kYePad = 16;
bool vcg_available(const lgh_ctx *c);
int vcg_test_k1(lgh_ctx *c, const double *r, const double *d_old, const double rz[3], const double rz_prev[3], int first,
                double *YE_out, double den_out[3]);
int vcg_test_k2(lgh_ctx *c, int it, const double *YE_in, double *r, double *d, double *x, const double den[3], const double rz[3],
                const double rz_prev[3], const double alpha_prev[3], double rz_out[3], int *deferred_x);
int vcg_test_exact_sum(lgh_ctx *c, int mode, long n, int G, int E, const double *scale, const double *v, const long long *w_in,
                       long long *w_out, double *d_out, int *i_out);
int vcg_k1_form(lgh_ctx *c);
void comm_shared_nodes(const lgh_ctx *c, const uint8_t **hmask, const int **sh_node, int *n_shared);
int energy_overlap_poll(lgh_ctx *c);
int host_wait_token(lgh_ctx *c, volatile unsigned long long *word, unsigned long long token);
constexpr int kLsWord = 50;
constexpr int kLsWordsPerSet = 56;
struct LockstepWords { const long long *own; const long long *peers; int n_peers, before; };
bool l2_lockstep_possible(lgh_ctx *c);
int cg_l2_begin_lockstep(lgh_ctx *c, const double *b, double *x, double rel_tol, int max_iter);
int l2_lockstep_limit(lgh_ctx *c);
int l2_lockstep_apply(lgh_ctx *c, int it, const LockstepWords &prev, double *den_mirror);
int l2_lockstep_update(lgh_ctx *c, int it, const double *den_src, long long *word_out);
int l2_lockstep_fold(lgh_ctx *c, int it, const LockstepWords &last);
int cg_l2_end_lockstep(lgh_ctx *c, int *iters);
int comm_ranks_before(const lgh_ctx *c);
bool vcg_lockstep_ready(const lgh_ctx *c);
int cg_l2_begin(lgh_ctx *c, const double *b, double *x, double rel_tol, int max_iter);
int cg_l2_end(lgh_ctx *c, int *iters);
int cg_solve(lgh_ctx *c, int space, const double *b, double *x, double rel_tol, int max_iter,
             int *iters, bool x_is_zero);
int stress_on_hand(lgh_ctx *c, const char *who);
int qupdate(lgh_ctx *c, const double *S);
int setup_rho0detj0(lgh_ctx *c, const double *x0, const double *rho0_l2, const double *rho0_q,
                    double *volume);
int interp_energy(lgh_ctx *c, int which, const double *vec, double *result);
int tg_source_2d(lgh_ctx *c, const double *S, double *out);
int test_eig(lgh_ctx *c, int dim, int n, const double *A, double *lambda, double *vec);
int test_singular(lgh_ctx *c, int dim, int n, const double *A, double *sv);
int test_sqrt(lgh_ctx *c, int n, const double *x, double *y);
int vec_set(lgh_ctx *c, double *y, double a, long n);
int vec_axpby(lgh_ctx *c, double *z, double a, const double *x, double b, const double *y, long n);
int vec_axpby_pair(lgh_ctx *c, double *z1, double a1, const double *x1, double b1, double *z2, double a2, const double *x2, double b2,
                   const double *y, long n);
int vec_neg_inplace(lgh_ctx *c, double *y, long n);
int vec_zero_list(lgh_ctx *c, double *y, const int *list, int n);
int vec_dot(lgh_ctx *c, const double *x, const double *y, const double *w, long n, double *dev_out);
struct HaloNodeAlias { const int *nodes, *sh_node; };
int halo_sum(lgh_ctx *c, double *v, int ncomp, double *extra = nullptr, int nextra = 0, bool packed = false, const HaloNodeAlias *alias = nullptr);
void comm_node_lists(const lgh_ctx *c, const int **nodes, int *total, const int **sh_node, int *n_shared);
struct HaloPackTables
{
   const int *sh_off, *sh_src;
   const int *pos, *cnt;
   const int *base, *ncnt;
   double *sbuf;
   int n_nbr;
};
bool comm_pack_tables(const lgh_ctx *c, HaloPackTables *t);
bool halo_can_piggyback(const lgh_ctx *c);
bool comm_second_channel(const lgh_ctx *c);
int exchange_words(lgh_ctx *c, const long long *src, int nwords);
int comm_word_peers(lgh_ctx *c, int nwords, const long long **peers, int *n_peers);
int allreduce_dev_n(lgh_ctx *c, double *dev, long count, int op);
int allreduce_dev(lgh_ctx *c, double *dev, int count, int op, bool packed = false);

bool kernel_id_supported_1d(int kid);
int create_common(const lgh_config *cfg, lgh_ctx *c, std::vector<int> &t_off, std::vector<int> &t_idx);
int create_1d(const lgh_config *cfg, lgh_ctx *c);
int setup_1d(lgh_ctx *c, const double *x0, const double *rho0_l2, const double *rho0_q, double *volume);
int mass_changed_1d(lgh_ctx *c);
int force_mult_1d(lgh_ctx *c, const double *x_l2, double *y_h1);
int force_mult_t_1d(lgh_ctx *c, const double *v_h1, double *y_l2);
int mass_apply_1d(lgh_ctx *c, int space, const double *x, double *y, bool eliminate);
int l2_solve_local_1d(lgh_ctx *c, const double *b, double *x);
int cg_1d(lgh_ctx *c, int space, const double *b, double *x, double rel_tol, int max_iter, int *iters, bool x_is_zero);
int qupdate_1d(lgh_ctx *c, const double *S);
int solve_velocity_1d(lgh_ctx *c, const double *ones, double *dv, double *rhs, double rel_tol, int max_iter, int *h1_iters);
int solve_energy_1d(lgh_ctx *c, const double *v_h1, double *de, double *e_rhs, const double *e_source, int *l2_iters);
int density_1d(lgh_ctx *c, const double *x_h1, double *rho_l2);
int energy_1d(lgh_ctx *c, int which, const double *vec, double *result);
int sedov_density_error_1d(lgh_ctx *c, const double *x_h1, const double *rho_l2, const double par[21], double t,
                           const double origin[3], int n1d, const double *weights, const double *B_h1, const double *G_h1,
                           const double *B_l2, double *err2);

inline void kt_begin(lgh_ctx *c, int id)
{
   KTime *k = c->ktime.get();
   if (k && k->which == id && k->n < k->max) { (void)hipEventRecord(k->ev[2 * k->n], c->stream); }
}
inline void kt_end(lgh_ctx *c, int id)
{
   KTime *k = c->ktime.get();
   if (k && k->which == id && k->n < k->max) { (void)hipEventRecord(k->ev[2 * k->n + 1], c->stream); k->n++; }
}

struct KtScope
{
   lgh_ctx *c;
   int id;
   KtScope(lgh_ctx *c_, int id_) : c(c_), id(id_) { kt_begin(c, id); }
   ~KtScope() { kt_end(c, id); }
   KtScope(const KtScope &) = delete;
   KtScope &operator=(const KtScope &) = delete;
};

void timer_start(lgh_ctx *c);
void timer_stop(lgh_ctx *c, int which);
struct RoctxRange
{
   bool on;
   explicit RoctxRange(const char *name);
   ~RoctxRange();
   RoctxRange(const RoctxRange &) = delete;
   RoctxRange &operator=(const RoctxRange &) = delete;
};

}
```

laghos_amd/csrc/lgh_energy.hip:

```cpp
#include <algorithm>

#include "lgh_common.hpp"

extern "C"
{

__global__ void __launch_bounds__(256) vec_differs_k(const double *__restrict__ a, const double *__restrict__ b, const long n, int *flag)
{
   const long stride = (long)gridDim.x * blockDim.x, t = (long)blockIdx.x * blockDim.x + threadIdx.x;
   bool diff = false;
   if (((((uintptr_t)a) | ((uintptr_t)b)) & 15u) == 0)
   {
      const longlong2 *a2 = (const longlong2 *)a, *b2 = (const longlong2 *)b;
      for (long i = t; i < n / 2; i += stride)
      {
         const longlong2 p = a2[i], q = b2[i];
         diff = diff || p.x != q.x || p.y != q.y;
      }
      if ((n & 1) && t == 0) { diff = diff || __double_as_longlong(a[n - 1]) != __double_as_longlong(b[n - 1]); }
   }
   else
   {
      for (long i = t; i < n; i += stride) { diff = diff || __double_as_longlong(a[i]) != __double_as_longlong(b[i]); }
   }
   if (diff) { *flag = 1; }
}
__global__ void __launch_bounds__(256) erhs_take_or_poison_k(double *__restrict__ y, const double *__restrict__ x, const long n, const int *__restrict__ flag, int *err)
{
   const long i = (long)blockIdx.x * blockDim.x + threadIdx.x;
   if (*flag != 0)
   {
      if (i < n) { y[i] = __builtin_nan(""); }
      if (i == 0) { *err = 1; }
      return;
   }
   if (i < n) { y[i] = x[i]; }
}
__global__ void __launch_bounds__(256) copy_unless_k(double *__restrict__ y, const double *__restrict__ x, const long n, const int *__restrict__ flag)
{
   if (*flag != 0) { return; }
   const long i = (long)blockIdx.x * blockDim.x + threadIdx.x;
   if (i < n) { y[i] = x[i]; }
}

}

namespace lgh
{

struct Stream2Scope
{
   lgh_ctx *c;
   explicit Stream2Scope(lgh_ctx *c_) : c(c_) { flip(1); }
   ~Stream2Scope() { flip(0); }
   Stream2Scope(const Stream2Scope &) = delete;
   Stream2Scope &operator=(const Stream2Scope &) = delete;

private:
   void flip(const int on)
   {
      std::swap(c->stream, c->stream2);
      c->on_stream2 = on;
   }
};

static int energy_rhs(lgh_ctx *c, const double *v_h1, double *e_rhs)
{
   RoctxRange range("SolveEnergy-ForcePA");
   if (c->erhs_q && c->fused_ftv_valid)
   {
      int *flag = c->dev_flags + (c->on_stream2 ? 2 : 0);
      LGH_HIP_CHECK(hipMemsetAsync(flag, 0, sizeof(int), c->stream));
      hipLaunchKernelGGL(vec_differs_k, dim3(grid_for((c->H1V + 1) / 2)), dim3(256), 0, c->stream, v_h1, c->v_snap, (long)c->H1V, flag);
      LGH_HIP_CHECK(hipGetLastError());
      if (c->stress_current)
      {
         const int rc = force_mult_t_L(c, c->stressJinvT, v_h1, e_rhs, flag);
         if (rc) { return rc; }
         hipLaunchKernelGGL(copy_unless_k, dim3(ceil_div(c->L2V, 256)), dim3(256), 0, c->stream, e_rhs, c->erhs_q, (long)c->L2V, flag);
      }
      else
      {
         hipLaunchKernelGGL(erhs_take_or_poison_k, dim3(ceil_div(c->L2V, 256)), dim3(256), 0, c->stream, e_rhs, c->erhs_q, (long)c->L2V, flag, c->dev_flags + 4);
      }
      LGH_HIP_CHECK(hipGetLastError());
      return LGH_OK;
   }
   return lgh_force_mult_transpose(c, v_h1, e_rhs);
}
static int energy_rhs_with_source(lgh_ctx *c, const double *v_h1, double *e_rhs, const double *e_source)
{
   timer_start(c);
   int rc = energy_rhs(c, v_h1, e_rhs);
   timer_stop(c, 2);
   if (rc == LGH_OK && e_source) { rc = vec_axpby(c, e_rhs, 1.0, e_rhs, 1.0, e_source, c->L2V); }
   return rc;
}
static void count_l2(lgh_ctx *c, const int it, int *l2_iters)
{
   const int counted = (it == 0) ? 1 : it;
   c->timers.c[1] += counted;
   if (l2_iters) { *l2_iters += counted; }
}

static int create_stream2(lgh_ctx *c)
{
   int least = 0, greatest = 0;
   if (hipDeviceGetStreamPriorityRange(&least, &greatest) == hipSuccess && least != greatest)
   {
      LGH_HIP_CHECK(hipStreamCreateWithPriority(&c->stream2, hipStreamNonBlocking, least));
   }
   else { LGH_HIP_CHECK(hipStreamCreateWithFlags(&c->stream2, hipStreamNonBlocking)); }
   LGH_HIP_CHECK(hipEventCreateWithFlags(&c->ev_fork, hipEventDisableTiming));
   LGH_HIP_CHECK(hipEventCreateWithFlags(&c->ev_join, hipEventDisableTiming));
   return LGH_OK;
}

static bool energy_quiet(const lgh_ctx *c)
{
   return c->sw.overlap && !c->timers.enabled && !(c->ktime && c->ktime->which >= 0) && vcg_available(c);
}
static bool energy_second_channel_free(const lgh_ctx *c)
{
   return c->multi == 0 || comm_second_channel(c);
}
static bool energy_lockstep_capable(lgh_ctx *c)
{
   return c->multi != 0 && !comm_second_channel(c) && l2_lockstep_possible(c) && vcg_lockstep_ready(c);
}
static EnergySolve::Mode energy_mode(lgh_ctx *c)
{
   if (c->dim == 1) { return EnergySolve::Deferred; }
   if (!energy_quiet(c)) { return EnergySolve::Deferred; }
   if (energy_second_channel_free(c)) { return EnergySolve::Overlapped; }
   return (c->sw.energy_lockstep && energy_lockstep_capable(c)) ? EnergySolve::Lockstep : EnergySolve::Deferred;
}

static int energy_overlapped_finish(lgh_ctx *c, int *it)
{
   Stream2Scope on2(c);
   const int rc = cg_l2_end(c, it);
   if (rc) { return rc; }
   LGH_HIP_CHECK(hipEventRecord(c->ev_join, c->stream));
   return LGH_OK;
}
int energy_overlap_poll(lgh_ctx *c)
{
   EnergySolve &e = c->energy;
   if (e.mode != EnergySolve::Overlapped || e.polled) { return LGH_OK; }
   int it = 0;
   const int rc = energy_overlapped_finish(c, &it);
   if (rc) { return rc; }
   e.polled = true;
   e.iters = it;
   return LGH_OK;
}

}

using namespace lgh;

extern "C"
{

int lgh_solve_energy(lgh_ctx *c, const double *S, const double *v_h1, double *dS_dt, double *e_rhs,
                     const double *e_source, double rel_tol, int max_iter, int *l2_iters)
{
   LGH_CHECK_ARG(c && S && v_h1 && dS_dt && e_rhs);
   (void)S;
   double *de = dS_dt + 2 * (size_t)c->H1V;
   if (c->dim == 1)
   {
      const int rc1 = stress_on_hand(c, "lgh_solve_energy");
      if (rc1) { return rc1; }
      return solve_energy_1d(c, v_h1, de, e_rhs, e_source, l2_iters);
   }
   int rc = energy_rhs_with_source(c, v_h1, e_rhs, e_source);
   if (rc) { return rc; }
   int it = 0;
   RoctxRange range("SolveEnergy-CGEMass");
   timer_start(c);
   rc = cg_solve(c, LGH_SPACE_L2, e_rhs, de, rel_tol, max_iter, &it, true);
   timer_stop(c, 1);
   if (rc) { return rc; }
   count_l2(c, it, l2_iters);
   return LGH_OK;
}

int lgh_solve_energy_begin(lgh_ctx *c, const double *S, const double *v_h1, double *dS_dt, double *e_rhs,
                           const double *e_source, double rel_tol, int max_iter)
{
   LGH_CHECK_ARG(c && S && v_h1 && dS_dt && e_rhs);
   EnergySolve &e = c->energy;
   e = EnergySolve{};
   e.args = {S, v_h1, dS_dt, e_rhs, e_source, rel_tol, max_iter};
   double *de = dS_dt + 2 * (size_t)c->H1V;
   const EnergySolve::Mode mode = energy_mode(c);
   if (mode == EnergySolve::Lockstep)
   {
      int rc = energy_rhs_with_source(c, v_h1, e_rhs, e_source);
      if (rc == LGH_OK) { rc = cg_l2_begin_lockstep(c, e_rhs, de, rel_tol, max_iter); }
      if (rc) { return rc; }
   }
   if (mode == EnergySolve::Overlapped)
   {
      if (!c->stream2)
      {
         const int rc2 = create_stream2(c);
         if (rc2) { return rc2; }
      }
      LGH_HIP_CHECK(hipEventRecord(c->ev_fork, c->stream));
      LGH_HIP_CHECK(hipStreamWaitEvent(c->stream2, c->ev_fork, 0));
      Stream2Scope on2(c);
      int rc = energy_rhs_with_source(c, v_h1, e_rhs, e_source);
      if (rc == LGH_OK)
      {
         RoctxRange range("SolveEnergy-CGEMass");
         rc = cg_l2_begin(c, e_rhs, de, rel_tol, max_iter);
      }
      if (rc) { return rc; }
   }
   e.mode = mode;
   return LGH_OK;
}
int lgh_energy_lockstep_stats(lgh_ctx *c, long out[4])
{
   LGH_CHECK_ARG(c && out);
   out[0] = c->ls_stats[0]; out[1] = c->ls_stats[1]; out[2] = c->ls_stats[2];
   out[3] = (vcg_available(c) && energy_lockstep_capable(c)) ? 1 : 0;
   return LGH_OK;
}
int lgh_solve_energy_end(lgh_ctx *c, int *l2_iters)
{
   LGH_CHECK_ARG(c && c->energy.mode != EnergySolve::Idle);
   const EnergySolve e = c->energy;
   c->energy = EnergySolve{};
   int it = 0;
   switch (e.mode)
   {
      case EnergySolve::Deferred:
         return lgh_solve_energy(c, e.args.S, e.args.v, e.args.dS, e.args.e_rhs, e.args.src, e.args.tol, e.args.maxit, l2_iters);
      case EnergySolve::Lockstep:
      {
         const int rc = cg_l2_end_lockstep(c, &it);
         if (rc) { return rc; }
         break;
      }
      case EnergySolve::Overlapped:
         if (e.polled) { it = e.iters; }
         else
         {
            const int rc = energy_overlapped_finish(c, &it);
            if (rc) { return rc; }
         }
         LGH_HIP_CHECK(hipStreamWaitEvent(c->stream, c->ev_join, 0));
         break;
      case EnergySolve::Idle: break;
   }
   count_l2(c, it, l2_iters);
   return LGH_OK;
}

}
```

laghos_amd/csrc/lgh_qupdate.hip:

```cpp
#include "lgh_qpoint.hpp"
#include "lgh_qrows.hpp"

namespace lgh
{

int qupdate_form(lgh_ctx *c);
int qupdate(lgh_ctx *c, const double *S)
{
   QArgs a = q_base(c);
   a.x = S;
   a.v = S + c->H1V;
   a.e = S + 2 * (size_t)c->H1V;
   a.result = c->dt_est_dev;
   a.Jac0inv_e = (c->jac0_compact == 1) ? c->Jac0inv_e : nullptr;
   const bool keep = !c->stress_store && a.erhs_q && a.force_e && c->v_snap;
   if (keep) { a.stressJinvT = nullptr; }
   const int form = qupdate_form(c);
   const int rc = (form == 1) ? launch_qrows(c, a) : launch_q<QMODE_UPDATE>(c, a);
   c->qgen++;
   c->stress_current = (rc == LGH_OK && !keep) ? 1 : 0;
   c->fused_ftv_valid = (rc == LGH_OK && a.erhs_q && c->v_snap) ? 1 : 0;
   c->fused_f1_valid = (rc == LGH_OK && a.force_e) ? 1 : 0;
   if (c->fused_ftv_valid)
   {
      LGH_HIP_CHECK(hipMemcpyAsync(c->v_snap, S + c->H1V, sizeof(double) * (size_t)c->H1V, hipMemcpyDeviceToDevice, c->stream));
   }
   return rc;
}

int qupdate_form(lgh_ctx *c)
{
   return (qrows_available(c) && c->sw.q_form) ? 1 : 0;
}

int interp_energy(lgh_ctx *c, int which, const double *vec, double *result)
{
   QArgs a = q_base(c);
   a.result = c->scal;
   int rc;
   if (which == 0)
   {
      a.e = vec;
      rc = launch_q<QMODE_IE>(c, a);
   }
   else
   {
      a.v = vec;
      rc = launch_q<QMODE_KE>(c, a);
   }
   if (rc) { return rc; }
   if (c->multi != 0)
   {
      rc = allreduce_dev(c, c->scal, 1, 0);
      if (rc) { return rc; }
   }
   LGH_HIP_CHECK(hipMemcpyAsync(c->host_pinned + kPinResult, c->scal, sizeof(double), hipMemcpyDeviceToHost, c->stream));
   LGH_HIP_CHECK(hipStreamSynchronize(c->stream));
   *result = (which == 0) ? c->host_pinned[kPinResult] : 0.5 * c->host_pinned[kPinResult];
   return LGH_OK;
}

__global__ void __launch_bounds__(128)
tg_source_2d_k(const int NE, const int N, const int D, const int Q, const int L, const int *__restrict__ map,
               const double *__restrict__ B, const double *__restrict__ G, const double *__restrict__ Bl,
               const double *__restrict__ W, const double *__restrict__ x, double *__restrict__ out)
{
   __shared__ double sx[2 * 36], ss[100];
   const int e = blockIdx.x, t = threadIdx.x;
   const int ND = D * D, NQ = Q * Q, NL = L * L;
   for (int i = t; i < 2 * ND; i += blockDim.x)
   {
      const int c = i / ND, d = i - c * ND;
      sx[i] = x[(size_t)c * N + map[(size_t)e * ND + d]];
   }
   __syncthreads();
   if (t < NQ)
   {
      const int qx = t % Q, qy = t / Q;
      double v[2] = {0.0, 0.0}, gx[2] = {0.0, 0.0}, gy[2] = {0.0, 0.0};
      for (int dy = 0; dy < D; dy++)
      {
         for (int dx = 0; dx < D; dx++)
         {
            const double bb = B[qx + Q * dx] * B[qy + Q * dy];
            const double gb = G[qx + Q * dx] * B[qy + Q * dy];
            const double bg = B[qx + Q * dx] * G[qy + Q * dy];
            for (int c = 0; c < 2; c++)
            {
               const double u = sx[c * ND + dx + D * dy];
               v[c] += bb * u;
               gx[c] += gb * u;
               gy[c] += bg * u;
            }
         }
      }
      const double det = gx[0] * gy[1] - gx[1] * gy[0];
      const double f = 3.0 / 8.0 * M_PI * (cos(3.0 * M_PI * v[0]) * cos(M_PI * v[1]) - cos(M_PI * v[0]) * cos(3.0 * M_PI * v[1]));
      ss[t] = W[t] * det * f;
   }
   __syncthreads();
   if (t < NL)
   {
      const int lx = t % L, ly = t / L;
      double s = 0.0;
      for (int qy = 0; qy < Q; qy++)
      {
         for (int qx = 0; qx < Q; qx++) { s += ss[qx + Q * qy] * Bl[qx + Q * lx] * Bl[qy + Q * ly]; }
      }
      out[t + (size_t)NL * e] = s;
   }
}
int tg_source_2d(lgh_ctx *c, const double *S, double *out)
{
   if (c->dim != 2) { set_error("the Taylor-Green energy source is the 2D one (laghos_solver.cpp:448)"); return LGH_ERR_ARG; }
   if (c->D1D > 6 || c->Q1D > 10 || c->NQ > 128) { return LGH_ERR_UNSUPPORTED; }
   hipLaunchKernelGGL(tg_source_2d_k, dim3(c->NE), dim3(128), 0, c->stream, c->NE, c->N, c->D1D, c->Q1D, c->L1D,
                      c->h1map, c->B, c->G, c->Bl, c->W, S, out);
   LGH_HIP_CHECK(hipGetLastError());
   return LGH_OK;
}

template <int DIM>
__global__ void test_eig_k(int n, const double *A, double *lambda, double *vec)
{
   const int i = blockIdx.x * blockDim.x + threadIdx.x;
   if (i >= n) { return; }
   double a[DIM * DIM], v[DIM], l;
   for (int k = 0; k < DIM * DIM; k++) { a[k] = A[(size_t)i * DIM * DIM + k]; }
   sm::min_eigenpair<DIM>(a, l, v);
   lambda[i] = l;
   for (int k = 0; k < DIM; k++) { vec[(size_t)i * DIM + k] = v[k]; }
}
template <int DIM>
__global__ void test_sv_k(int n, const double *A, double *sv)
{
   const int i = blockIdx.x * blockDim.x + threadIdx.x;
   if (i >= n) { return; }
   double a[DIM * DIM];
   for (int k = 0; k < DIM * DIM; k++) { a[k] = A[(size_t)i * DIM * DIM + k]; }
   sv[i] = sm::min_singular<DIM>(a);
}
__global__ void test_sqrt_k(int n, const double *x, double *y)
{
   const int i = blockIdx.x * blockDim.x + threadIdx.x;
   if (i < n) { y[i] = sm::fsqrt(x[i]); }
}
int test_sqrt(lgh_ctx *c, int n, const double *x, double *y)
{
   hipLaunchKernelGGL(test_sqrt_k, dim3(ceil_div(n, 256)), dim3(256), 0, c->stream, n, x, y);
   LGH_HIP_CHECK(hipGetLastError());
   return LGH_OK;
}
int test_eig(lgh_ctx *c, int dim, int n, const double *A, double *lambda, double *vec)
{
   if (dim == 2) { hipLaunchKernelGGL(test_eig_k<2>, dim3(ceil_div(n, 128)), dim3(128), 0, c->stream, n, A, lambda, vec); }
   else { hipLaunchKernelGGL(test_eig_k<3>, dim3(ceil_div(n, 128)), dim3(128), 0, c->stream, n, A, lambda, vec); }
   LGH_HIP_CHECK(hipGetLastError());
   return LGH_OK;
}
int test_singular(lgh_ctx *c, int dim, int n, const double *A, double *sv)
{
   if (dim == 2) { hipLaunchKernelGGL(test_sv_k<2>, dim3(ceil_div(n, 128)), dim3(128), 0, c->stream, n, A, sv); }
   else { hipLaunchKernelGGL(test_sv_k<3>, dim3(ceil_div(n, 128)), dim3(128), 0, c->stream, n, A, sv); }
   LGH_HIP_CHECK(hipGetLastError());
   return LGH_OK;
}

}
```

laghos_amd/csrc/lgh_vcg.hip:

```cpp
#include "lgh_vcg.hpp"

namespace lgh
{
typedef unsigned v4u_ __attribute__((ext_vector_type(4)));

__device__ __forceinline__ double vcg_ld(const double *base, const unsigned off) { return *(const double *)((const char *)base + off); }
__device__ __forceinline__ double *vcg_ptr(double *base, const unsigned off) { return (double *)((char *)base + off); }

__device__ __forceinline__ void vcg_reset_accumulators(const VcgArgs &a)
{
   if (!a.reset || blockIdx.x != 0) { return; }
   if (a.limbs) { for (int i = threadIdx.x; i < 2 * kLimbWords + 8 * 16; i += blockDim.x) { a.limbs[i] = 0; } }
   if (a.rzl) { for (int i = threadIdx.x; i < 3 * kLimbWords; i += blockDim.x) { a.rzl[i] = 0; } }
}
__device__ __forceinline__ void vcg_reset_scalars(const VcgArgs &a, VcgScalars *s)
{
   if (!a.reset) { return; }
   s->rel_tol2 = a.reset_tol2;
   s->all_done = 0;
   s->first = 1;
   for (int c = 0; c < kVC; c++) { s->done[c] = 0; s->iters[c] = 0; s->nupd[c] = 0; s->alpha_last[c] = 0.0; s->alpha_hist[0][c] = s->alpha_hist[1][c] = 0.0; s->rzh[0][c] = s->rzh[1][c] = 0.0; }
}

__global__ void __launch_bounds__(256)
vcg_init_k(const VcgArgs a)
{
   vcg_reset_accumulators(a);
   __shared__ double red[48];
   const int n = xcd_swizzle(blockIdx.x, gridDim.x) * blockDim.x + threadIdx.x;
   double part[kVC] = {0.0, 0.0, 0.0};
   if (n < a.N)
   {
      const double di = a.dinv[n];
      const double ow = a.owner ? a.owner[n] : 1.0;
#pragma unroll
      for (int c = 0; c < kVC; c++)
      {
         const size_t i = (size_t)c * a.N + n;
         const double rv = a.b[(size_t)c * a.N + (a.ncaller ? a.ncaller[n] : n)];
         a.r[i] = rv;
         part[c] = ow * __dmul_rn(rv, di) * rv;
      }
   }
   double bp[kVC], total[kVC];
   block_sum3(part[0], part[1], part[2], red, bp);
   if (grid_sum3_last_block(bp, a.partials, a.stride, a.ticket, red, total))
   {
      if (threadIdx.x == 0)
      {
         VcgScalars *s = a.s;
         int all = 1;
         vcg_reset_scalars(a, s);
         for (int c = 0; c < kVC; c++)
         {
            s->rz[c] = s->rz_prev[c] = total[c];
            s->iters[c] = 0;
            if (!a.multi)
            {
               s->r0[c] = fmax(total[c] * s->rel_tol2, 0.0);
               s->done[c] = (total[c] < 0.0 || total[c] <= s->r0[c]) ? 1 : 0;
               all = all && s->done[c];
            }
         }
         s->first = 1;
         if (!a.multi) { s->all_done = all; }
      }
   }
}
template <int DEG>
__global__ void __launch_bounds__(256)
vcg_init_force_k(const VcgArgs a, const double *__restrict__ FE, const int ND, double *__restrict__ bout, const int *__restrict__ ellc, const int degc)
{
   vcg_reset_accumulators(a);
   __shared__ double red[48];
   const int n = xcd_swizzle(blockIdx.x, gridDim.x) * blockDim.x + threadIdx.x;
   double part[kVC] = {0.0, 0.0, 0.0};
   if (n < a.N)
   {
      long pos[DEG];
#pragma unroll
      for (int j = 0; j < DEG; j++)
      {
         const int p = (j < degc) ? ellc[(size_t)j * a.N + n] : -1;
         const int e = p / ND;
         pos[j] = (p >= 0) ? (long)kVC * ND * e + (p - e * ND) : -1;
      }
      const double di = a.dinv[n];
#pragma unroll
      for (int c = 0; c < kVC; c++)
      {
         double s = 0.0;
#pragma unroll
         for (int j = 0; j < DEG; j++) { if (pos[j] >= 0) { s += FE[pos[j] + (long)ND * c]; } }
         double bv = -s;
         if (a.ess[c] && a.ess[c][n]) { bv = 0.0; }
         const size_t i = (size_t)c * a.N + n;
         bout[(size_t)c * a.N + (a.ncaller ? a.ncaller[n] : n)] = bv;
         a.r[i] = bv;
         a.x[i] = 0.0;
         part[c] = __dmul_rn(bv, di) * bv;
      }
   }
   double bp[kVC], total[kVC];
   block_sum3(part[0], part[1], part[2], red, bp);
   if (grid_sum3_last_block(bp, a.partials, a.stride, a.ticket, red, total))
   {
      if (threadIdx.x == 0)
      {
         VcgScalars *s = a.s;
         int all = 1;
         vcg_reset_scalars(a, s);
         for (int c = 0; c < kVC; c++)
         {
            s->rz[c] = s->rz_prev[c] = total[c];
            s->iters[c] = 0;
            s->r0[c] = fmax(total[c] * s->rel_tol2, 0.0);
            s->done[c] = (total[c] < 0.0 || total[c] <= s->r0[c]) ? 1 : 0;
            all = all && s->done[c];
         }
         s->first = 1;
         s->all_done = all;
      }
   }
}
__global__ void __launch_bounds__(256)
vcg_init_force_z_k(const VcgArgs a, const double *__restrict__ FE, const unsigned compb_fe, const unsigned *__restrict__ ellf,
                   double *__restrict__ bout)
{
   vcg_reset_accumulators(a);
   __shared__ double red[48];
   const int n = xcd_swizzle(blockIdx.x, gridDim.x) * blockDim.x + threadIdx.x;
   const bool ok = n < a.N;
   const unsigned nn = (unsigned)(ok ? n : a.N - 1);
   const unsigned rowb = 4u * (unsigned)a.N;
   unsigned ix[8];
#pragma unroll
   for (int j = 0; j < 8; j++) { ix[j] = *(const unsigned *)((const char *)ellf + (4u * nn + (unsigned)j * rowb)); }
   const double di = vcg_ld(a.dinv, 8u * nn);
   const unsigned es = a.essbits[nn];
   const unsigned zoff = 8u * (unsigned)kVC * (unsigned)(a.ye_stride - kYePad);
   double fe[kVC][8];
#pragma unroll
   for (int j = 0; j < 8; j++)
   {
      if (j == 0 || __any(ix[j] != zoff))
      {
#pragma unroll
         for (int c = 0; c < kVC; c++) { fe[c][j] = vcg_ld(FE, ix[j] + (unsigned)c * compb_fe); }
      }
      else
      {
#pragma unroll
         for (int c = 0; c < kVC; c++) { fe[c][j] = 0.0; }
      }
   }
   double part[kVC];
#pragma unroll
   for (int c = 0; c < kVC; c++)
   {
      double s = 0.0;
#pragma unroll
      for (int j = 0; j < 8; j++) { s += fe[c][j]; }
      double bv = -s;
      if ((es >> c) & 1u) { bv = 0.0; }
      part[c] = ok ? __dmul_rn(bv, di) * bv : 0.0;
      if (ok)
      {
         const size_t i = (size_t)c * a.N + n;
         bout[(size_t)c * a.N + (a.ncaller ? a.ncaller[n] : n)] = bv;
         a.r[i] = bv;
         a.x[i] = 0.0;
      }
   }
   double bp[kVC], total[kVC];
   block_sum3(part[0], part[1], part[2], red, bp);
   if (grid_sum3_last_block(bp, a.partials, a.stride, a.ticket, red, total))
   {
      if (threadIdx.x == 0)
      {
         VcgScalars *s = a.s;
         int all = 1;
         vcg_reset_scalars(a, s);
         for (int c = 0; c < kVC; c++)
         {
            s->rz[c] = s->rz_prev[c] = total[c];
            s->iters[c] = 0;
            s->r0[c] = fmax(total[c] * s->rel_tol2, 0.0);
            s->done[c] = (total[c] < 0.0 || total[c] <= s->r0[c]) ? 1 : 0;
            all = all && s->done[c];
         }
         s->first = 1;
         s->all_done = all;
      }
   }
}
__global__ void vcg_init_finish_k(VcgScalars *s)
{
   int all = 1;
   for (int c = 0; c < kVC; c++)
   {
      s->rz_prev[c] = s->rz[c];
      s->r0[c] = fmax(s->rz[c] * s->rel_tol2, 0.0);
      s->done[c] = (s->rz[c] < 0.0 || s->rz[c] <= s->r0[c]) ? 1 : 0;
      all = all && s->done[c];
   }
   s->all_done = all;
}
__global__ void vcg_set_tol_k(VcgScalars *s, double rel_tol2, long long *limbs, long long *rzl)
{
   if (limbs) { for (int i = 0; i < 2 * kLimbWords + 8 * 16; i++) { limbs[i] = 0; } }
   if (rzl) { for (int i = 0; i < 3 * kLimbWords; i++) { rzl[i] = 0; } }
   s->rel_tol2 = rel_tol2;
   s->all_done = 0;
   s->first = 1;
   for (int c = 0; c < kVC; c++) { s->done[c] = 0; s->iters[c] = 0; s->nupd[c] = 0; s->alpha_last[c] = 0.0; s->alpha_hist[0][c] = s->alpha_hist[1][c] = 0.0; s->rzh[0][c] = s->rzh[1][c] = 0.0; }
}
__global__ void vcg_update_finish_k(VcgScalars *s, int iter, VcgScalars *host_out, unsigned long long *host_token, const unsigned long long token)
{
   int all = 1;
   for (int c = 0; c < kVC; c++)
   {
      if (!s->done[c])
      {
         s->iters[c] = iter;
         if (s->rz[c] < 0.0 || s->rz[c] <= s->r0[c]) { s->done[c] = 1; }
      }
      if (s->done[c]) { s->rz[c] = 0.0; s->den[c] = 0.0; }
      all = all && s->done[c];
   }
   s->all_done = all;
   if (host_out)
   {
      *host_out = *s;
      __threadfence_system();
      __hip_atomic_store(host_token, token, __ATOMIC_RELEASE, __HIP_MEMORY_SCOPE_SYSTEM);
   }
}

__global__ void vcg_rz_finish_k(VcgScalars *s, const long long *rzl, const int last, const long long *peers, const int n_peers, VcgScalars *host_out,
                                unsigned long long *host_token, const unsigned long long token)
{
   long long set[kLimbWords];
   for (int i = 0; i <= kLimbShards * kVC * kLimbs; i++)
   {
      long long w = rzl[(last % 3) * kLimbWords + i];
      for (int p = 0; p < n_peers; p++) { w += peers[p * kLimbWords + i]; }
      set[i] = w;
   }
   double cur[kVC];
   bool dn[kVC];
   for (int k = 0; k < kVC; k++)
   {
      const double before = (last > 1) ? s->rzh[(last - 1) & 1][k] : s->rz[k];
      cur[k] = exact_fold(set, k, exact_scale(before));
      dn[k] = s->done[k] != 0 || vcg_rz_converged(last + 1, cur[k], s->r0[k]);
   }
   vcg_rz_commit(s, last + 1, cur, dn);
   if (host_out)
   {
      *host_out = *s;
      __threadfence_system();
      __hip_atomic_store(host_token, token, __ATOMIC_RELEASE, __HIP_MEMORY_SCOPE_SYSTEM);
   }
}

template <bool FUSED_GATHER, int DEG>
__global__ void __launch_bounds__(256)
vcg_update_k(const VcgArgs a)
{
   __shared__ double red[48];
   if (a.s->all_done) { return; }
   const bool it1 = (a.iter == 1);
   const int n = xcd_swizzle(blockIdx.x, gridDim.x) * blockDim.x + threadIdx.x;
   const bool ok = n < a.N;
   const int nn = ok ? n : a.N - 1;
   double part[kVC] = {0.0, 0.0, 0.0};
   int pidx[DEG > 0 ? DEG : 1];
   if (FUSED_GATHER)
   {
#pragma unroll
      for (int j = 0; j < DEG; j++) { pidx[j] = (j < a.deg) ? a.ell[(size_t)j * a.N + nn] : -1; }
   }
   const double di = a.dinv[nn];
   const double ow = a.owner ? a.owner[nn] : 1.0;
   const bool shared = FUSED_GATHER && a.hmask && a.hmask[nn];
#pragma unroll 1
   for (int c = 0; c < kVC; c++)
   {
      if (a.s->done[c]) { continue; }
      if (a.multi && vcg_pending_den(a.s, c, blockIdx.x == 0 && threadIdx.x == 0)) { continue; }
      const double alpha = a.s->rz[c] / a.s->den[c];
      const double beta = it1 ? 0.0 : a.s->rz[c] / a.s->rz_prev[c];
      const size_t i = (size_t)c * a.N + nn;
      double zv;
      if (FUSED_GATHER)
      {
         if (shared) { zv = a.yL[i]; }
         else
         {
            const double *yc = a.YE + (size_t)c * a.ye_stride;
            zv = 0.0;
#pragma unroll
            for (int j = 0; j < DEG; j++) { if (pidx[j] >= 0) { zv += yc[pidx[j]]; } }
         }
      }
      else { zv = a.yL[i]; }
      if (a.ess[c] && a.ess[c][nn]) { zv = 0.0; }
      const double ro = a.r[i];
      double dv = __dmul_rn(ro, di);
      if (!it1) { dv = fma(beta, a.d[i], dv); }
      const double xv = a.x[i] + alpha * dv;
      const double rv = ro - alpha * zv;
      const double pz = __dmul_rn(rv, di);
      if (ok)
      {
         a.d[i] = dv;
         a.x[i] = xv;
         a.r[i] = rv;
         part[c] = ow * rv * pz;
      }
   }
   double bp[kVC], total[kVC];
// ... 417 lines not shown
   m.k2p = aux->ellz != nullptr && c->sw.k2p;
   m.limbs = c->sw.slab_exact && m.k2p && k1.form == kK1Slab && aux->limbs != nullptr;
   m.rz_words = m.limbs && (!m.multi || ((halo_can_piggyback(c) || c->nranks == 1) && c->t_deg <= 8)) && c->sw.rz_limbs;
   HaloPackTables hp;
   const uint8_t *hmask = nullptr;
   const int *sh_node = nullptr;
   if (m.multi) { comm_shared_nodes(c, &hmask, &sh_node, &m.n_shared); }
   if (m.multi && m.rz_words)
   {
      m.ls_mine = m.k2p && c->t_deg <= 8 && l2_lockstep_possible(c) && comm_ranks_before(c) >= 0 &&
                  (m.n_shared == 0 || (c->sw.halo_fused_pack && halo_can_piggyback(c) && comm_pack_tables(c, &hp)));
   }
   if (m.multi && c->nranks == 1) { aux->ls_all = m.ls_mine ? 1 : 0; }
   if (m.multi && c->nranks > 1) { LGH_VCG_TRY(vcg_mode_collective(c, aux, k1, in_solve, m)); }
   m.rzl = m.rz_words && c->sw.slab_defer && aux->rzl != nullptr;
   m.den_limbs = (m.limbs && c->sw.slab_defer) ? (m.multi ? 2 : 1) : 0;
   if (c->sw.halo_fused_pack && m.mixed && m.k2p && m.n_shared > 0 && comm_pack_tables(c, &hp))
   {
      m.pack_halo = 1;
      m.nx_den = halo_can_piggyback(c) ? (c->energy.mode == EnergySolve::Lockstep ? kVC + 1 : kVC) : 0;
      m.pack_rz = (halo_can_piggyback(c) && !m.rzl) ? 1 : 0;
   }
   if (in_solve)
   {
      aux->ls_ready = (m.multi && aux->ls_all == 1 && m.ls_mine && m.rzl && (m.n_shared == 0 || (m.pack_halo && halo_can_piggyback(c)))) ? 1 : 0;
   }
   m.ls = c->energy.mode == EnergySolve::Lockstep && m.multi && m.rzl && aux->ls_ready && (m.n_shared == 0 || m.nx_den == kVC + 1);
   return LGH_OK;
}

static int vcg_fill_internal_order(lgh_ctx *c, VcgAux *aux, const VcgK1 &k1, const VcgMode &m, VcgArgs &a)
{
   const bool need_table = a.dqs != 0 || k1.form == kK1Column;
   if (aux->o_mass_gen != c->mass_gen)
   {
      LGH_VCG_TRY(order_gather_nodes(c, c->dinvV, aux->o_dinv, 1));
      if (a.dqs == 0) { LGH_VCG_TRY(order_zone_blocks(c, a.Se, aux->o_Se, 1, false)); }
      if (need_table)
      {
         if (!aux->o_massD) { LGH_VCG_TRY(aux->o_massD.alloc((size_t)c->NE * c->NQ + 2048, true)); }
         LGH_VCG_TRY(order_zone_blocks(c, c->massD, aux->o_massD, c->NQ, false));
      }
      aux->o_mass_gen = c->mass_gen;
   }
   if (a.dqs == 0) { a.Se = aux->o_Se; }
   else { a.Dq = aux->o_massD; }
   a.DqFull = need_table ? aux->o_massD.p : nullptr;
   a.map = aux->o_map;
   a.ell = aux->o_ell;
   for (int k = 0; k < kVC; k++) { a.ess[k] = aux->o_ess[k]; }
   a.dinv = aux->o_dinv;
   a.owner = m.multi ? aux->o_owner.p : nullptr;
   a.ncaller = aux->ord->ncaller_d;
   a.x = aux->o_x;
   return LGH_OK;
}

static int vcg_fill_args(lgh_ctx *c, VcgAux *aux, const VcgK1 &k1, const VcgMode &m, double *B, double *X, const double rel_tol, const bool in_solve, VcgArgs &a)
{
   const size_t N = (size_t)c->N;
   memset(&a, 0, sizeof(a));
   a.NE = c->NE;
   a.N = c->N;
   a.B = c->B;
   a.DqFull = c->massD;
   LGH_VCG_TRY(mass_data(c, &a.Dq, &a.dqs, &a.Se));
   a.w1 = (a.dqs == 0) ? c->w1d : nullptr;
   a.M1 = (a.dqs == 0 && c->w1d) ? c->M1h : nullptr;
   a.map = c->h1map;
   a.ell = c->t_ell;
   a.deg = c->t_deg;
   for (int k = 0; k < kVC; k++) { a.ess[k] = c->essmask[k]; }
   a.dinv = c->dinvV;
   a.owner = m.multi ? c->owner : nullptr;
   a.b = B;
   a.x = X;
   if (aux->ord) { LGH_VCG_TRY(vcg_fill_internal_order(c, aux, k1, m, a)); }
   a.r = c->vcg_vec;
   a.d = c->vcg_vec + kVC * N;
   a.yL = c->vcg_vec + 2 * kVC * N;
   a.YE = aux->ye;
   a.ye_stride = (size_t)c->NE * c->ND + kYePad;
   a.ye_wide = (a.ye_stride * 8 * kVC >= 0xffffffffull || c->sw.slab_ye_wide) ? 1 : 0;
   a.ellz = aux->ellz;
   a.essbits = aux->essbits;
   a.nstart = aux->nstart;
   a.mapb = aux->mapb;
   a.map_xrows = aux->map_xrows;
   if (k1.form == kK1Slab && aux->settab)
   {
      a.settab = aux->settab;
      a.ell = aux->ellm;
      a.deg = aux->degm;
      a.ellz = aux->ellzm;
      a.nstart = aux->nstartm;
   }
   a.limbs = m.limbs ? aux->limbs.p : nullptr;
   a.rzl = m.rzl ? aux->rzl.p : nullptr;
   a.reset = in_solve ? 1 : 0;
   a.reset_tol2 = rel_tol * rel_tol;
   if (m.rzl && m.multi) { LGH_VCG_TRY(comm_word_peers(c, kLimbWords, &a.rzl_peers, &a.n_rz_peers)); }
   a.queue = a.limbs ? (unsigned *)(a.limbs + 2 * kLimbWords) : nullptr;
   a.den_limbs = m.den_limbs;
   a.k2_skip = c->sw.k2_skip;
   a.s = c->vcg_s;
   a.stride = c->vcg_stride;
   a.multi = m.multi ? 1 : 0;
   if (!c->sw.vcg_trace.empty())
   {
      if (!aux->trace) { (void)aux->trace.alloc((size_t)kTraceRec * kTraceBlocks, true); }
      a.trace = aux->trace;
      if (a.trace) { (void)hipMemsetAsync(a.trace, 0, (size_t)kTraceRec * kTraceBlocks * sizeof(unsigned long long), c->stream); }
   }
   if (m.multi)
   {
      comm_shared_nodes(c, &a.hmask, &a.sh_node, &a.n_shared);
      if (aux->ord && a.n_shared > 0) { a.hmask = aux->o_hmask; a.sh_node = aux->o_shnode; }
   }
   if (m.pack_halo) { (void)comm_pack_tables(c, &a.hp); }
   a.pack_halo = m.pack_halo;
   a.nx_den = m.nx_den;
   a.pack_rz = m.pack_rz;
   return LGH_OK;
}

int vcg_prepare(lgh_ctx *c, double *B, double *X, double rel_tol, VcgPlan &plan, const bool in_solve)
{
   LGH_VCG_TRY(vcg_work_buffers(c));
   if (!c->vcg_aux) { LGH_VCG_TRY(vcg_build_aux(c)); }
   VcgAux *aux = c->vcg_aux.get();
   plan.aux = aux;
   plan.k1 = vcg_resolve_k1(c);
   LGH_VCG_TRY(vcg_mode(c, aux, plan.k1, in_solve, plan.mode));
   const VcgMode &m = plan.mode;
   if (!in_solve)
   {
      hipLaunchKernelGGL(vcg_set_tol_k, dim3(1), dim3(1), 0, c->stream, c->vcg_s.p, rel_tol * rel_tol, m.limbs ? aux->limbs.p : nullptr,
                         m.rzl ? aux->rzl.p : nullptr);
   }
   return vcg_fill_args(c, aux, plan.k1, m, B, X, rel_tol, in_solve, plan.a);
}

static_assert((kPinVcg + (sizeof(VcgScalars) + sizeof(double) - 1) / sizeof(double)) <= (size_t)kPinVcgToken, "VcgScalars ends before the token slot of the pinned block");

struct VcgRun
{
   VcgScalars *ds, *hs;
   const HaloNodeAlias *alias;
   int max_iter, chunk, it = 0, looks = 0;
   bool energy_polled = false;
   int ls_limit, ls_before;
};

static int vcg_start(lgh_ctx *c, VcgPlan &plan, double *B, const double *force_E)
{
   VcgArgs &a = plan.a;
   const VcgAux *aux = plan.aux;
   const int nb = ceil_div(a.N, 256);
   a.partials = c->vcg_partials;
   a.ticket = c->vcg_tickets;
   if (force_E)
   {
      if (!plan.mode.direct) { set_error("vcg_solve: fused init is single-rank, degree <= 8"); return LGH_ERR_ARG; }
      if (aux->ellf && aux->essbits) { hipLaunchKernelGGL(vcg_init_force_z_k, dim3(nb), dim3(256), 0, c->stream, a, force_E, 8u * (unsigned)c->ND, aux->ellf, B); }
      else { hipLaunchKernelGGL(vcg_init_force_k<8>, dim3(nb), dim3(256), 0, c->stream, a, force_E, c->ND, B, aux->o_ellc ? aux->o_ellc : c->t_ell, c->t_deg); }
   }
   else
   {
      if (aux->ord) { LGH_HIP_CHECK(hipMemsetAsync(a.x, 0, kVC * (size_t)a.N * sizeof(double), c->stream)); }
      hipLaunchKernelGGL(vcg_init_k, dim3(nb), dim3(256), 0, c->stream, a);
   }
   LGH_HIP_CHECK(hipGetLastError());
   if (plan.mode.multi)
   {
      LGH_VCG_TRY(allreduce_dev(c, a.s->rz, kVC, 0));
      hipLaunchKernelGGL(vcg_init_finish_k, dim3(1), dim3(1), 0, c->stream, a.s);
   }
   return LGH_OK;
}

static int vcg_look(lgh_ctx *c, const VcgPlan &plan, VcgRun &r, bool &stop)
{
   const VcgArgs &a = plan.a;
   VcgScalars *hs_dev = (VcgScalars *)(c->host_pinned_dev + kPinVcg);
   unsigned long long *tok_dev = (unsigned long long *)(c->host_pinned_dev + kPinVcgToken);
   volatile unsigned long long *tok = (volatile unsigned long long *)(c->host_pinned + kPinVcgToken);
   const unsigned long long token = ++c->look_token;
   bool copied = false;
   if (!r.energy_polled) { r.energy_polled = true; LGH_VCG_TRY(energy_overlap_poll(c)); }
   if (plan.mode.multi && !a.rzl && r.it > 0) { hipLaunchKernelGGL(vcg_update_finish_k, dim3(1), dim3(1), 0, c->stream, r.ds, r.it, hs_dev, tok_dev, token); copied = true; }
   if (a.rzl && r.it > 0) { vcg_launch_rz_finish(c, a, r.it, hs_dev, tok_dev, token); copied = true; }
   if (copied)
   {
      LGH_VCG_TRY(host_wait_token(c, tok, token));
   }
   else
   {
      LGH_HIP_CHECK(hipMemcpyAsync(r.hs, r.ds, sizeof(VcgScalars), hipMemcpyDeviceToHost, c->stream));
      LGH_HIP_CHECK(hipStreamSynchronize(c->stream));
   }
   stop = r.hs->all_done || r.it >= r.max_iter;
   if (!stop) { r.chunk = (++r.looks <= 2) ? 2 : std::min(64, 2 * r.chunk); }
   return LGH_OK;
}

static int vcg_step_k1(lgh_ctx *c, const VcgPlan &plan, VcgArgs &a)
{
   a.partials = c->vcg_partials + (size_t)kVC * c->vcg_stride;
   a.ticket = c->vcg_tickets + kTicketSlot;
   kt_begin(c, LGH_KERNEL_MASS_CG_H1);
   vcg_launch_k1(c, plan, a);
   kt_end(c, LGH_KERNEL_MASS_CG_H1);
   LGH_HIP_CHECK(hipGetLastError());
   a.partials = c->vcg_partials;
   a.ticket = c->vcg_tickets;
   return LGH_OK;
}

static int vcg_iterate_direct(lgh_ctx *c, const VcgPlan &plan, VcgArgs &a)
{
   LGH_VCG_TRY(vcg_step_k1(c, plan, a));
   if (plan.mode.k2p) { vcg_launch_k2p(c, plan, a, a.iter); }
   else { kt_begin(c, LGH_KERNEL_CG_UPDATE_H1); vcg_launch_update(c, a, true); kt_end(c, LGH_KERNEL_CG_UPDATE_H1); }
   LGH_HIP_CHECK(hipGetLastError());
   return LGH_OK;
}

static int vcg_iterate_exchange(lgh_ctx *c, const VcgPlan &plan, VcgArgs &a, const VcgRun &r, const int upto)
{
   const VcgMode &m = plan.mode;
   const int it = a.iter, nb = ceil_div(a.N, 256);
   const bool ls_it = m.ls && it <= r.ls_limit;
   auto ls_words = [&](const int set_it) { return LockstepWords{a.rzl + (set_it % 3) * kLimbWords, a.rzl_peers, a.n_rz_peers, r.ls_before}; };
   LGH_VCG_TRY(vcg_step_k1(c, plan, a));
   if (ls_it) { LGH_VCG_TRY(l2_lockstep_apply(c, it, ls_words(it - 1), &r.ds->den_e)); }
   if (m.mixed)
   {
      if (a.n_shared > 0) { hipLaunchKernelGGL(vcg_gather_list_k, dim3(ceil_div(a.n_shared, 256)), dim3(256), 0, c->stream, a); }
      else if (a.den_limbs == 2) { vcg_launch_fold_den(c, a); }
   }
   else
   {
      if (a.den_limbs == 2) { vcg_launch_fold_den(c, a); }
      hipLaunchKernelGGL(vcg_gather_k, dim3(nb), dim3(256), 0, c->stream, a);
   }
   LGH_HIP_CHECK(hipGetLastError());
   if (m.multi)
   {
      const bool ride = halo_can_piggyback(c);
      LGH_VCG_TRY(halo_sum(c, a.yL, kVC, ride ? r.ds->den : nullptr, ride ? std::max(a.nx_den, kVC) : 0, a.pack_halo != 0, r.alias));
      if (!ride) { LGH_VCG_TRY(allreduce_dev(c, r.ds->den, kVC, 0)); }
   }
   if (m.mixed && m.k2p) { vcg_launch_k2p(c, plan, a, it); }
   else { vcg_launch_update(c, a, m.mixed); }
   if (ls_it) { LGH_VCG_TRY(l2_lockstep_update(c, it, &r.ds->den_e, a.rzl + (it % 3) * kLimbWords)); }
   if (m.multi && a.rzl)
   {
      LGH_VCG_TRY(exchange_words(c, a.rzl + (it % 3) * kLimbWords, kLimbWords));
      if (ls_it && (it == r.ls_limit || it == upto))
      {
         LGH_VCG_TRY(l2_lockstep_fold(c, it, ls_words(it)));
      }
   }
   else if (m.multi) { LGH_VCG_TRY(allreduce_dev(c, r.ds->rz, kVC, 0, a.pack_rz != 0 && m.mixed && m.k2p)); }
   LGH_HIP_CHECK(hipGetLastError());
   return LGH_OK;
}

static int vcg_finish(lgh_ctx *c, const VcgPlan &plan, const VcgRun &r, double *X, int iters[3])
{
   const VcgArgs &a = plan.a;
   const int nb = ceil_div(a.N, 256);
   if (plan.aux->ord)
   {
      hipLaunchKernelGGL(vcg_xout_k, dim3(nb), dim3(256), 0, c->stream, a, X);
      LGH_HIP_CHECK(hipGetLastError());
   }
   else if (plan.mode.k2p && ((r.hs->nupd[0] | r.hs->nupd[1] | r.hs->nupd[2]) & 1))
   {
      hipLaunchKernelGGL(vcg_xfix_k, dim3(nb), dim3(256), 0, c->stream, a);
      LGH_HIP_CHECK(hipGetLastError());
   }
   FILE *f = a.trace ? fopen(c->sw.vcg_trace.c_str(), "w") : nullptr;
   if (f)
   {
      std::vector<unsigned long long> h((size_t)kTraceRec * kTraceBlocks);
      (void)hipMemcpy(h.data(), a.trace, h.size() * 8, hipMemcpyDeviceToHost);
      for (int i = 0; i < kTraceBlocks; i++)
      {
         if (h[(size_t)kTraceRec * i] == 0) { continue; }
         fprintf(f, "%d", i);
         for (int k = 0; k < kTraceRec; k++) { fprintf(f, " %llu", h[(size_t)kTraceRec * i + k]); }
         fprintf(f, "\n");
      }
      fclose(f);
   }
   int mx = 0;
   for (int k = 0; k < kVC; k++)
   {
      int fin = r.hs->iters[k];
      if (!r.hs->done[k] && r.it >= r.max_iter) { fin = r.max_iter; }
      iters[k] = fin;
      mx = std::max(mx, fin);
   }
   c->vcg_last = mx;
   return LGH_OK;
}

int vcg_solve(lgh_ctx *c, double *B, double *X, double rel_tol, int max_iter, int iters[3], const double *force_E)
{
   if (!vcg_available(c)) { return LGH_ERR_UNSUPPORTED; }
   VcgPlan plan;
   LGH_VCG_TRY(vcg_prepare(c, B, X, rel_tol, plan, true));
   VcgArgs &a = plan.a;
   const VcgMode &m = plan.mode;
   VcgRun r;
   r.ds = a.s;
   r.hs = (VcgScalars *)(c->host_pinned + kPinVcg);
   r.alias = (plan.aux->ord && plan.aux->o_alias.nodes) ? &plan.aux->o_alias : nullptr;
   r.max_iter = max_iter;
   r.chunk = c->vcg_last > 0 ? c->vcg_last : 8;
   r.ls_limit = m.ls ? std::min(l2_lockstep_limit(c), max_iter) : 0;
   r.ls_before = m.ls ? comm_ranks_before(c) : 0;
   LGH_VCG_TRY(vcg_start(c, plan, B, force_E));
   for (bool first_look = true;; first_look = false)
   {
      if (!first_look || max_iter <= 0)
      {
         bool stop = false;
         LGH_VCG_TRY(vcg_look(c, plan, r, stop));
         if (stop) { break; }
      }
      const int upto = std::min(max_iter, r.it + r.chunk);
      while (r.it < upto)
      {
         a.iter = ++r.it;
         LGH_VCG_TRY(m.direct ? vcg_iterate_direct(c, plan, a) : vcg_iterate_exchange(c, plan, a, r, upto));
      }
   }
   return vcg_finish(c, plan, r, X, iters);
}

}
```

laghos_amd/host/laghos_solver.cpp:

```cpp
#include "laghos_solver.hpp"

#include <cmath>
#include <cstdlib>
#include <cstring>
#include <iomanip>
#include <iostream>
#include <limits>

namespace laghos
{
namespace hydrodynamics
{

void AbortWithLghError(const char *where)
{
   std::fprintf(stderr, "%s failed: %s\n", where, lgh_last_error());
   std::abort();
}

LagrangianHydroOperator::LagrangianHydroOperator(const Discretization &d, const std::vector<double> &S0,
                                                 const std::vector<double> &rho0_l2,
                                                 const std::vector<double> &gamma,
                                                 const std::vector<double> &rho0_q, double cfl,
                                                 double cgt, int cgiter, int device, const char *nccl_id)
   : disc(d), ctx(nullptr), dim(d.dim), NE(d.NE), H1Vsize(d.H1V), L2Vsize(d.L2V),
     H1GTVSize(d.dim * d.global_N), L2GTVSize(d.global_NE * d.NL), cg_rel_tol(cgt),
     cg_max_iter(cgiter), qdata_is_current(false), volume(0.0)
{
   lgh_config cfg;
   std::memset(&cfg, 0, sizeof(cfg));
   cfg.dim = dim;
   cfg.NE = NE;
   cfg.D1D = d.tab.D1D;
   cfg.Q1D = d.tab.Q1D;
   cfg.L1D = d.tab.L1D;
   cfg.N = d.N;
   cfg.h1_map = d.h1map.data();
   cfg.B_h1 = d.tab.B.data();
   cfg.G_h1 = d.tab.G.data();
   cfg.B_l2 = d.tab.Bl.data();
   cfg.weights = d.W.data();
   cfg.gamma = gamma.data();
   for (int c = 0; c < 3; c++)
   {
      cfg.ess_count[c] = (c < dim) ? (int)d.ess[c].size() : 0;
      cfg.ess[c] = (c < dim) ? d.ess[c].data() : nullptr;
   }
   const char *force_env = std::getenv("LGH_FORCE_MULTI");
   const bool force_multi = (force_env && force_env[0] == '1' && d.part.nranks == 1);
   const bool multi = d.part.nranks > 1 || force_multi;
   cfg.owner = multi ? d.owner.data() : nullptr;
   cfg.use_viscosity = d.UseViscosity();
   cfg.use_vorticity = d.UseVorticity() ? 1 : 0;
   cfg.cfl = cfl;
   cfg.order_v = d.tab.order_v;
   cfg.device = device;
   cfg.stream = nullptr;
   LGH_VERIFY(lgh_create(&cfg, &ctx));
   if (multi)
   {
      char self_id[128];
      if (!nccl_id && force_multi)
      {
         LGH_VERIFY(lgh_comm_unique_id(self_id));
         nccl_id = self_id;
      }
      if (!nccl_id) { std::fprintf(stderr, "multi-rank run needs an RCCL unique id\n"); std::abort(); }
      LGH_VERIFY(lgh_comm_init(ctx, d.part.nranks, d.part.rank, nccl_id));
      std::vector<int> cnt;
      std::vector<const int *> ptrs;
      for (auto &l : d.nbr_nodes) { cnt.push_back((int)l.size()); ptrs.push_back(l.data()); }
      LGH_VERIFY(lgh_comm_set_neighbors(ctx, (int)d.nbr_rank.size(), d.nbr_rank.data(), cnt.data(), ptrs.data()));
   }
   qdata.reset(new QuadratureData(ctx));
   qupdate.reset(new QUpdate(ctx));
   ForcePA.reset(new ForcePAOperator(*qdata, ctx));
   VMassPA.reset(new MassPAOperator(ctx, LGH_SPACE_H1));
   EMassPA.reset(new MassPAOperator(ctx, LGH_SPACE_L2));
   timer.L2dof = L2Vsize;

   Vector x0((long)H1Vsize), r_l2, r_q;
   {
      std::vector<double> xh(S0.begin(), S0.begin() + H1Vsize);
      x0.FromHost(xh);
   }
   r_l2.FromHost(rho0_l2);
   r_q.FromHost(rho0_q);
   double vol = 0.0;
   LGH_VERIFY(lgh_setup_rho0detj0(ctx, x0.Read(), r_l2.Read(), r_q.Read(), &vol));
   double ne = (double)NE;
   if (multi)
   {
      LGH_VERIFY(lgh_allreduce(ctx, &vol, 0));
      LGH_VERIFY(lgh_allreduce(ctx, &ne, 0));
   }
   volume = vol;
   qdata->h0 = std::pow(vol / ne, 1.0 / dim) / (double)d.tab.order_v;
   LGH_VERIFY(lgh_set_h0(ctx, qdata->h0));

   one.SetSize(L2Vsize);
   LGH_VERIFY(lgh_vec_set(ctx, one.Write(), 1.0, L2Vsize));
   rhs.SetSize(H1Vsize);
   e_rhs.SetSize(L2Vsize);
   source_type = d.SourceType();
   if (source_type == 1) { e_source.SetSize(L2Vsize); }
   if (source_type == 2)
   {
      std::vector<double> acc((size_t)H1Vsize, 0.0);
      for (long i = H1Vsize / dim; i < 2 * (H1Vsize / dim); i++) { acc[i] = -1.0; }
      accel_src.FromHost(acc);
      LGH_VERIFY(lgh_set_velocity_source(ctx, accel_src.Read()));
   }
   B.SetSize(d.N);
   LGH_VERIFY(lgh_sync(ctx));
}

LagrangianHydroOperator::~LagrangianHydroOperator() { lgh_destroy(ctx); }

void LagrangianHydroOperator::Mult(const Vector &S, Vector &dS_dt) const
{
   UpdateMesh(S);
   LGH_VERIFY(lgh_vec_copy(ctx, dS_dt.Write(), S.Read() + H1Vsize, H1Vsize));
   UpdateQuadratureData(S);
   if (source_type == 1) { LGH_VERIFY(lgh_tg_source_2d(ctx, S.Read(), e_source.Write())); }
   LGH_VERIFY(lgh_solve_energy_begin(ctx, S.Read(), S.Read() + H1Vsize, dS_dt.Write(), e_rhs.Write(),
                                     source_type == 1 ? e_source.Read() : nullptr, cg_rel_tol, cg_max_iter));
   SolveVelocity(S, dS_dt);
   int it = 0;
   LGH_VERIFY(lgh_solve_energy_end(ctx, &it));
   qdata_is_current = false;
}

void LagrangianHydroOperator::SolveVelocity(const Vector &S, Vector &dS_dt) const
{
   UpdateQuadratureData(S);
   int it = 0;
   LGH_VERIFY(lgh_solve_velocity(ctx, S.Read(), dS_dt.Write(), nullptr, rhs.Write(), B.Write(),
                                 cg_rel_tol, cg_max_iter, &it));
}

void LagrangianHydroOperator::SolveEnergy(const Vector &S, const Vector &v, Vector &dS_dt) const
{
   UpdateQuadratureData(S);
   int it = 0;
   if (source_type == 1) { LGH_VERIFY(lgh_tg_source_2d(ctx, S.Read(), e_source.Write())); }
   LGH_VERIFY(lgh_solve_energy(ctx, S.Read(), v.Read(), dS_dt.Write(), e_rhs.Write(),
                               source_type == 1 ? e_source.Read() : nullptr,
                               cg_rel_tol, cg_max_iter, &it));
}

void LagrangianHydroOperator::UpdateQuadratureData(const Vector &S) const
{
   unsigned long gen = 0;
   int f1 = 0, ftv = 0;
   LGH_VERIFY(lgh_quadrature_generation(ctx, &gen, &f1, &ftv));
   if (qdata_is_current && gen == qdata_gen) { return; }
   qdata_is_current = true;
   qupdate->UpdateQuadratureData(S, *qdata);
   LGH_VERIFY(lgh_quadrature_generation(ctx, &gen, &f1, &ftv));
   qdata_gen = gen;
}

double LagrangianHydroOperator::GetTimeStepEstimate(const Vector &S) const
{
   UpdateMesh(S);
   UpdateQuadratureData(S);
   double dt = qdata->GetDtEst();
   if (disc.part.nranks > 1) { LGH_VERIFY(lgh_allreduce(ctx, &dt, 1)); }
   return dt;
}

void LagrangianHydroOperator::ResetTimeStepEstimate() const
{
   qdata->SetDtEst(std::numeric_limits<double>::infinity());
}

double LagrangianHydroOperator::InternalEnergy(const Vector &S) const
{
   double r;
   LGH_VERIFY(lgh_internal_energy(ctx, S.Read() + 2 * (long)H1Vsize, &r));
   return r;
}
double LagrangianHydroOperator::KineticEnergy(const Vector &S) const
{
   double r;
   LGH_VERIFY(lgh_kinetic_energy(ctx, S.Read() + H1Vsize, &r));
   return r;
}
double LagrangianHydroOperator::ENorm(const Vector &S) const
{
   double n2;
   const double *e = S.Read() + 2 * (long)H1Vsize;
   LGH_VERIFY(lgh_vec_dot(ctx, e, e, L2Vsize, &n2));
   if (disc.part.nranks > 1) { LGH_VERIFY(lgh_allreduce(ctx, &n2, 0)); }
   return std::sqrt(n2);
}

void LagrangianHydroOperator::ComputeDensity(const Vector &S, Vector &rho) const
{
   if (rho.Size() != L2Vsize) { rho.SetSize(L2Vsize); }
   LGH_VERIFY(lgh_compute_density(ctx, S.Read(), rho.Write()));
}

double LagrangianHydroOperator::SedovDensityError(const Vector &S, const Vector &rho, const double par[21], double t,
                                                  const double origin[3], int err_order) const
{
   const int n1 = err_order / 2 + 1;
   std::vector<double> pts, wts, Bh, Gh, Bl;
   GaussLegendre(n1, pts, wts);
   LagrangeTables(disc.tab.gll, pts, Bh, Gh);
   BernsteinTable(disc.tab.order_e, pts, Bl);
   double err2 = 0;
   LGH_VERIFY(lgh_sedov_density_error(ctx, S.Read(), rho.Read(), par, t, origin, n1, wts.data(), Bh.data(), Gh.data(),
                                      Bl.data(), &err2));
   return std::sqrt(err2);
}

long LagrangianHydroOperator::SamplePoints(int R) const
{
   long np = NE;
   for (int a = 0; a < dim; a++) { np *= R + 1; }
   return np;
}

void LagrangianHydroOperator::SampleFields(const Vector &S, const Vector &rho, int R, Vector &out) const
{
   const long NP = SamplePoints(R);
   if (out.Size() < (2 * dim + 3) * NP) { out.SetSize((2 * dim + 3) * NP); }
   std::vector<double> Bh, Bl;
   LatticeTables(disc.tab.order_v, disc.tab.order_e, R, Bh, Bl);
   double *o = out.Write();
   LGH_VERIFY(lgh_sample_fields(ctx, S.Read(), rho.Read(), R + 1, Bh.data(), Bl.data(), o, o + dim * NP, o + 2 * dim * NP,
                                o + (2 * dim + 1) * NP, o + (2 * dim + 2) * NP));
}

long LagrangianHydroOperator::DerivedSize(int R) const
{
   const int nv = (dim == 3) ? 3 : (dim == 2 ? 1 : 0);
   return (3 + dim * dim + nv) * SamplePoints(R);
}

void LagrangianHydroOperator::SampleDerived(const Vector &S, int R, unsigned mask, Vector &out, long offset) const
{
   if (out.Size() < offset + DerivedSize(R)) { out.SetSize(offset + DerivedSize(R)); }
   std::vector<double> Bh, Bl, Gh;
   LatticeTables(disc.tab.order_v, disc.tab.order_e, R, Bh, Bl);
   LatticeGradTable(disc.tab.order_v, R, Gh);
   const DerivedBlocks<double> b(out.Write() + offset, dim, SamplePoints(R));
   LGH_VERIFY(lgh_sample_derived(ctx, S.Read(), R + 1, Bh.data(), Gh.data(), Bl.data(), (mask & DERIVED_DETJ) ? b.detj : nullptr,
                                 (mask & DERIVED_GRAD) ? b.grad : nullptr, (mask & DERIVED_DIV) ? b.div : nullptr,
                                 (mask & DERIVED_VORT) ? b.vort : nullptr, (mask & DERIVED_CS) ? b.cs : nullptr));
}

long LagrangianHydroOperator::FacePoints(int R, long nfaces) const
{
   long np = nfaces;
   for (int a = 0; a < dim - 1; a++) { np *= R + 1; }
   return np;
}

long LagrangianHydroOperator::FacesSize(int R, long nfaces) const
{
   const int nv = (dim == 3) ? 3 : (dim == 2 ? 1 : 0);
   return (2 * dim + 3 + 3 + dim * dim + nv + dim) * FacePoints(R, nfaces);
}

void LagrangianHydroOperator::SampleFaces(const Vector &S, const Vector &rho, int R, const std::vector<int> &faces, unsigned mask, Vector &out) const
{
   const long nfaces = (long)faces.size() / 2, NPt = FacePoints(R, nfaces);
   if (out.Size() < FacesSize(R, nfaces)) { out.SetSize(FacesSize(R, nfaces)); }
   if (nfaces == 0) { return; }
   std::vector<double> Bh, Bl, Gh;
   LatticeTables(disc.tab.order_v, disc.tab.order_e, R, Bh, Bl);
   LatticeGradTable(disc.tab.order_v, R, Gh);
   double *o = out.Write();
   double *x = o, *v = x + dim * NPt, *e = v + dim * NPt, *r = e + NPt, *p = r + NPt;
   const DerivedBlocks<double> b(p + NPt, dim, NPt);
   LGH_VERIFY(lgh_sample_faces(ctx, S.Read(), rho.Read(), R + 1, Bh.data(), Gh.data(), Bl.data(), (int)nfaces, faces.data(), x, v, e, r, p,
                               (mask & DERIVED_DETJ) ? b.detj : nullptr, (mask & DERIVED_GRAD) ? b.grad : nullptr, (mask & DERIVED_DIV) ? b.div : nullptr,
                               (mask & DERIVED_VORT) ? b.vort : nullptr, (mask & DERIVED_CS) ? b.cs : nullptr, b.end));
}

void LagrangianHydroOperator::Diagnostics(const Vector &S, double out[LGH_DIAG_COUNT]) const
{
   LGH_VERIFY(lgh_diagnostics(ctx, S.Read(), out));
}

void LagrangianHydroOperator::Profile(const Vector &S, const lgh_profile_spec &spec, double *rows, long *n_excluded) const
{
   LGH_VERIFY(lgh_profile(ctx, S.Read(), &spec, rows, n_excluded));
}

void LagrangianHydroOperator::Map(const Vector &S, const lgh_map_spec &spec, double *rows, long *n_excluded) const
{
   LGH_VERIFY(lgh_map(ctx, S.Read(), &spec, rows, n_excluded));
}

void LagrangianHydroOperator::SedovEval(const double par[21], double t, const std::vector<double> &r, std::vector<double> &rho,
                                        std::vector<double> &v, std::vector<double> &p) const
{
   const long n = (long)r.size();
   Vector dev(4 * n);
   std::vector<double> h(4 * n, 0.0);
   std::copy(r.begin(), r.end(), h.begin());
   dev.FromHost(h);
   double *d = dev.Write();
   LGH_VERIFY(lgh_sedov_eval(ctx, par, t, n, d, d + n, d + 2 * n, d + 3 * n));
   Sync();
   dev.ToHost(h);
   rho.assign(h.begin() + n, h.begin() + 2 * n);
   v.assign(h.begin() + 2 * n, h.begin() + 3 * n);
   p.assign(h.begin() + 3 * n, h.end());
}

double LagrangianHydroOperator::AllReduce(double v, int op) const
{
   if (disc.part.nranks > 1) { LGH_VERIFY(lgh_allreduce(ctx, &v, op)); }
   return v;
}
// ... 74 lines not shown
   if (!fom) { return; }
   const long ndofs = 2 * H1GTVSize + L2GTVSize + (long)NQ * (long)zones;
   cout << endl;
   cout << "| Ranks | Zones   | H1 dofs | L2 dofs | QP | N dofs   | FOM0   | FOM1   | T1   | FOM2   | T2   "
           "| FOM3   | T3   | FOM    | TT   |" << endl;
   cout << setprecision(3);
   cout << "| " << setw(6) << disc.part.nranks << "| " << setw(8) << (long)zones << "| " << setw(8)
        << H1GTVSize << "| " << setw(8) << L2GTVSize << "| " << setw(3) << NQ << "| " << setw(9) << ndofs
        << "| " << setw(7) << FOM0 << "| " << setw(7) << FOM1 << "| " << setw(5) << T[0] << "| " << setw(7)
        << FOM2 << "| " << setw(5) << T[2] << "| " << setw(7) << FOM3 << "| " << setw(5) << T[3] << "| "
        << setw(7) << FOM << "| " << setw(5) << T[4] << "| " << endl;
}

}

void ForwardEulerSolver::Init(hydrodynamics::LagrangianHydroOperator &op)
{
   ODESolver::Init(op);
   k.SetSize(op.Size());
}
void ForwardEulerSolver::Step(Vector &S, double &t, double &dt)
{
   f->Mult(S, k);
   f->Add(S, 1.0, S, dt, k);
   t += dt;
}

void RK2Solver::Init(hydrodynamics::LagrangianHydroOperator &op)
{
   ODESolver::Init(op);
   k.SetSize(op.Size());
   x1.SetSize(op.Size());
}
void RK2Solver::Step(Vector &S, double &t, double &dt)
{
   const double b = 0.5 / a;
   f->Mult(S, k);
   f->Add(x1, 1.0, S, (1. - b) * dt, k);
   f->Add(S, 1.0, S, a * dt, k);
   f->Mult(S, k);
   f->Add(S, 1.0, x1, b * dt, k);
   t += dt;
}

void RK3SSPSolver::Init(hydrodynamics::LagrangianHydroOperator &op)
{
   ODESolver::Init(op);
   k.SetSize(op.Size());
   y.SetSize(op.Size());
}
void RK3SSPSolver::Step(Vector &S, double &t, double &dt)
{
   f->Mult(S, k);
   f->Add(y, 1.0, S, dt, k);
   f->Mult(y, k);
   f->Add(y, 1.0, y, dt, k);
   f->Add(y, 3. / 4, S, 1. / 4, y);
   f->Mult(y, k);
   f->Add(y, 1.0, y, dt, k);
   f->Add(S, 1. / 3, S, 2. / 3, y);
   t += dt;
}

void RK4Solver::Init(hydrodynamics::LagrangianHydroOperator &op)
{
   ODESolver::Init(op);
   k.SetSize(op.Size());
   y.SetSize(op.Size());
   z.SetSize(op.Size());
}

void RK4Solver::Step(Vector &S, double &t, double &dt)
{
   f->Mult(S, k);
   f->Add2(y, 1.0, S, dt / 2, z, 1.0, S, dt / 6, k);
   f->Mult(y, k);
   f->Add2(y, 1.0, S, dt / 2, z, 1.0, z, dt / 3, k);
   f->Mult(y, k);
   f->Add2(y, 1.0, S, dt, z, 1.0, z, dt / 3, k);
   f->Mult(y, k);
   f->Add(S, 1.0, z, dt / 6, k);
   t += dt;
}

void ExplicitRKSolver::Init(hydrodynamics::LagrangianHydroOperator &op)
{
   ODESolver::Init(op);
   y.SetSize(op.Size());
   k.resize(s);
   for (int i = 0; i < s; i++) { k[i].SetSize(op.Size()); }
}
void ExplicitRKSolver::Step(Vector &S, double &t, double &dt)
{
   f->Mult(S, k[0]);
   for (int l = 0, i = 1; i < s; i++)
   {
      f->Add(y, 1.0, S, a[l++] * dt, k[0]);
      for (int j = 1; j < i; j++) { f->Add(y, 1.0, y, a[l++] * dt, k[j]); }
      f->Mult(y, k[i]);
   }
   for (int i = 0; i < s; i++) { f->Add(S, 1.0, S, b[i] * dt, k[i]); }
   t += dt;
}
const double RK6Solver::a[] = {
   .6e-1,
   .1923996296296296296296296296296296296296e-1,
   .7669337037037037037037037037037037037037e-1,
   .35975e-1,
   0.,
   .107925,
   1.318683415233148260919747276431735612861,
   0.,
   -5.042058063628562225427761634715637693344,
   4.220674648395413964508014358284402080483,
   -41.87259166432751461803757780644346812905,
   0.,
   159.4325621631374917700365669070346830453,
   -122.1192135650100309202516203389242140663,
   5.531743066200053768252631238332999150076,
   -54.43015693531650433250642051294142461271,
   0.,
   207.0672513650184644273657173866509835987,
   -158.6108137845899991828742424365058599469,
   6.991816585950242321992597280791793907096,
   -.1859723106220323397765171799549294623692e-1,
   -54.66374178728197680241215648050386959351,
   0.,
   207.9528062553893734515824816699834244238,
   -159.2889574744995071508959805871426654216,
   7.018743740796944434698170760964252490817,
   -.1833878590504572306472782005141738268361e-1,
   -.5119484997882099077875432497245168395840e-3};
const double RK6Solver::b[] = {
   .3438957868357036009278820124728322386520e-1,
   0.,
   0.,
   .2582624555633503404659558098586120858767,
   .4209371189673537150642551514069801967032,
   4.405396469669310170148836816197095664891,
   -176.4831190242986576151740942499002125029,
   172.3641334014150730294022582711902413315};
const double RK6Solver::c[] = {
   .6e-1,
   .9593333333333333333333333333333333333333e-1,
   .1439,
   .4973,
   .9725,
   .9995,
   1.};

void RK2AvgSolver::Init(hydrodynamics::LagrangianHydroOperator &op)
{
   ODESolver::Init(op);
   V.SetSize(op.H1VSize());
   dS_dt.SetSize(op.Size());
   S0.SetSize(op.Size());
}

void RK2AvgSolver::Step(Vector &S, double &t, double &dt)
{
   const long h1v = f->H1VSize();
   Vector v0, dx_dt, dv_dt;
   f->Copy(S0, S);
   v0.MakeRef(S0, h1v, h1v);
   dx_dt.MakeRef(dS_dt, 0, h1v);
   dv_dt.MakeRef(dS_dt, h1v, h1v);
   f->UpdateMesh(S);
   f->SolveVelocity(S, dS_dt);
   f->Add(V, 1.0, v0, 0.5 * dt, dv_dt);
   f->SolveEnergy(S, V, dS_dt);
   f->Copy(dx_dt, V);
   f->Add(S, 1.0, S0, 0.5 * dt, dS_dt);
   f->ResetQuadratureData();
   f->UpdateMesh(S);
   f->SolveVelocity(S, dS_dt);
   f->Add(V, 1.0, v0, 0.5 * dt, dv_dt);
   f->SolveEnergy(S, V, dS_dt);
   f->Copy(dx_dt, V);
   f->Add(S, 1.0, S0, dt, dS_dt);
   f->ResetQuadratureData();
   t += dt;
}

}
```

laghos_amd/host/laghos_solver.hpp:

```cpp
#pragma once
#include <memory>

#include "fem.hpp"
#include "laghos_assembly.hpp"

namespace laghos
{

template <class T> struct DerivedBlocks
{
   T *detj, *grad, *div, *vort, *cs, *end;
   DerivedBlocks(T *p, int dim, long NP)
      : detj(p), grad(detj + NP), div(grad + (long)dim * dim * NP), vort(div + NP), cs(vort + (dim == 3 ? 3 : (dim == 2 ? 1 : 0)) * NP), end(cs + NP) {}
};

namespace hydrodynamics
{

struct TimingData
{
   double sw_cgH1 = 0, sw_cgL2 = 0, sw_force = 0, sw_qdata = 0;
   long L2dof = 0, H1iter = 0, L2iter = 0, quad_tstep = 0;
};

class QUpdate
{
   lgh_ctx *ctx;

public:
   explicit QUpdate(lgh_ctx *c) : ctx(c) {}
   void UpdateQuadratureData(const Vector &S, QuadratureData &) { LGH_VERIFY(lgh_qupdate(ctx, S.Read())); }
};

class LagrangianHydroOperator
{
protected:
   const Discretization &disc;
   lgh_ctx *ctx;
   const int dim, NE;
   const int H1Vsize, L2Vsize;
   const long H1GTVSize, L2GTVSize;
   const double cg_rel_tol;
   const int cg_max_iter;
   std::unique_ptr<QuadratureData> qdata;
   mutable bool qdata_is_current;
   mutable unsigned long qdata_gen = 0;
   std::unique_ptr<ForcePAOperator> ForcePA;
   std::unique_ptr<MassPAOperator> VMassPA, EMassPA;
   std::unique_ptr<QUpdate> qupdate;
   mutable Vector one, rhs, e_rhs, B;
   Vector accel_src;
   mutable Vector e_source;
   int source_type = 0;
   mutable TimingData timer;
   double volume;

public:
   LagrangianHydroOperator(const Discretization &disc, const std::vector<double> &S0,
                           const std::vector<double> &rho0_l2, const std::vector<double> &gamma,
                           const std::vector<double> &rho0_q, double cfl, double cgt, int cgiter,
                           int device, const char *nccl_id);
   ~LagrangianHydroOperator();

   int Size() const { return 2 * H1Vsize + L2Vsize; }
   int H1VSize() const { return H1Vsize; }
   int L2VSize() const { return L2Vsize; }
   void Mult(const Vector &S, Vector &dS_dt) const;
   void SolveVelocity(const Vector &S, Vector &dS_dt) const;
   void SolveEnergy(const Vector &S, const Vector &v, Vector &dS_dt) const;
   void UpdateMesh(const Vector &) const {}
   void UpdateQuadratureData(const Vector &S) const;
   double GetTimeStepEstimate(const Vector &S) const;
   void ResetTimeStepEstimate() const;
   void ResetQuadratureData() const { qdata_is_current = false; LGH_VERIFY(lgh_reset_quadrature_data(ctx)); }
   double InternalEnergy(const Vector &S) const;
   double KineticEnergy(const Vector &S) const;
   double ENorm(const Vector &S) const;
   void ComputeDensity(const Vector &S, Vector &rho) const;
   double SedovDensityError(const Vector &S, const Vector &rho, const double par[21], double t,
                            const double origin[3], int err_order) const;
   void SampleFields(const Vector &S, const Vector &rho, int R, Vector &out) const;
   long SamplePoints(int R) const;
   enum { DERIVED_DIV = 1, DERIVED_VORT = 2, DERIVED_GRAD = 4, DERIVED_DETJ = 8, DERIVED_CS = 16, DERIVED_ALL = 31 };
   void SampleDerived(const Vector &S, int R, unsigned mask, Vector &out, long offset = 0) const;
   long DerivedSize(int R) const;
   void SampleFaces(const Vector &S, const Vector &rho, int R, const std::vector<int> &faces, unsigned mask, Vector &out) const;
   long FacePoints(int R, long nfaces) const;
   long FacesSize(int R, long nfaces) const;
   void Diagnostics(const Vector &S, double out[LGH_DIAG_COUNT]) const;
   void Profile(const Vector &S, const lgh_profile_spec &spec, double *rows, long *n_excluded) const;
   void Map(const Vector &S, const lgh_map_spec &spec, double *rows, long *n_excluded) const;
   void SedovEval(const double par[21], double t, const std::vector<double> &r, std::vector<double> &rho, std::vector<double> &v,
                  std::vector<double> &p) const;
   void PrintTimingData(bool IamRoot, int steps, bool fom) const;
   const TimingData &Timing() const;
   void ResetTiming();
   void EnableTimers(bool on);
   lgh_ctx *Context() const { return ctx; }
   long GlobalH1Size() const { return H1GTVSize; }
   long GlobalL2Size() const { return L2GTVSize; }
   int Rank() const { return disc.part.rank; }
   int NRanks() const { return disc.part.nranks; }
   double AllReduce(double v, int op) const;
   void Add(Vector &z, double a, const Vector &x, double b, const Vector &y) const;
   void Add2(Vector &z1, double a1, const Vector &x1, double b1, Vector &z2, double a2, const Vector &x2, double b2, const Vector &y) const;
   void Copy(Vector &y, const Vector &x) const;
   void Sync() const;
};

}

class ODESolver
{
protected:
   hydrodynamics::LagrangianHydroOperator *f = nullptr;

public:
   virtual ~ODESolver() {}
   virtual void Init(hydrodynamics::LagrangianHydroOperator &op) { f = &op; }
   virtual void Step(Vector &S, double &t, double &dt) = 0;
   virtual int Stages() const = 0;
};

class ForwardEulerSolver : public ODESolver
{
   Vector k;

public:
   void Init(hydrodynamics::LagrangianHydroOperator &op) override;
   void Step(Vector &S, double &t, double &dt) override;
   int Stages() const override { return 1; }
};
class RK2Solver : public ODESolver
{
   Vector k, x1;
   double a;

public:
   explicit RK2Solver(double a_ = 0.5) : a(a_) {}
   void Init(hydrodynamics::LagrangianHydroOperator &op) override;
   void Step(Vector &S, double &t, double &dt) override;
   int Stages() const override { return 2; }
};
class RK3SSPSolver : public ODESolver
{
   Vector k, y;

public:
   void Init(hydrodynamics::LagrangianHydroOperator &op) override;
   void Step(Vector &S, double &t, double &dt) override;
   int Stages() const override { return 3; }
};

class RK4Solver : public ODESolver
{
   Vector k, y, z;

public:
   void Init(hydrodynamics::LagrangianHydroOperator &op) override;
   void Step(Vector &S, double &t, double &dt) override;
   int Stages() const override { return 4; }
};

class ExplicitRKSolver : public ODESolver
{
   int s;
   const double *a, *b, *c;
   Vector y;
   std::vector<Vector> k;

public:
   ExplicitRKSolver(int s_, const double *a_, const double *b_, const double *c_) : s(s_), a(a_), b(b_), c(c_) {}
   void Init(hydrodynamics::LagrangianHydroOperator &op) override;
   void Step(Vector &S, double &t, double &dt) override;
   int Stages() const override { return s; }
};
class RK6Solver : public ExplicitRKSolver
{
   static const double a[28], b[8], c[7];

public:
   RK6Solver() : ExplicitRKSolver(8, a, b, c) {}
};

class RK2AvgSolver : public ODESolver
{
   Vector V, dS_dt, S0;

public:
   void Init(hydrodynamics::LagrangianHydroOperator &op) override;
   void Step(Vector &S, double &t, double &dt) override;
   int Stages() const override { return 2; }
};

}
```

Before: 1730 Mdofs*steps/s.

## Add fused hydro_mult stage entry that skips velocity snapshot and RHS stores

Adds lgh_hydro_mult, a single device-side stage call that runs the quadrature update, energy begin, velocity solve and energy end. In stage mode the velocity snapshot copy is skipped (ftv_valid=2), the precomputed F^T v is copied directly, and the CG init kernel no longer writes the B vector. The dS_dt velocity copy moves onto the energy stream when overlapped. The aim is to cut redundant device-to-device copies and writes per RK stage. The cost is extra state modes, plus an error path when a different velocity is later supplied.

```diff
diff --git a/include/laghos_hip.h b/include/laghos_hip.h
--- a/include/laghos_hip.h
+++ b/include/laghos_hip.h
@@ -96,6 +96,9 @@
 int lgh_solve_energy_begin(lgh_ctx *ctx, const double *S, const double *v_h1, double *dS_dt,
                            double *e_rhs, const double *e_source, double rel_tol, int max_iter);
 int lgh_solve_energy_end(lgh_ctx *ctx, int *l2_iters);
+int lgh_hydro_mult(lgh_ctx *ctx, const double *S, double *dS_dt, double *rhs_h1, double *work_B, double *e_rhs,
+                   const double *e_source, int qdata_current, double rel_tol, int max_iter, int *h1_iters, int *l2_iters);
+int lgh_qupdate_state(lgh_ctx *ctx, const double *S);
 int lgh_energy_lockstep_stats(lgh_ctx *ctx, long out[4]);
 
 int lgh_vec_set(lgh_ctx *ctx, double *y, double a, long n);
@@ -228,6 +231,7 @@
 int lgh_test_eig(lgh_ctx *ctx, int dim, int n, const double *A, double *lambda, double *vec);
 int lgh_test_sqrt(lgh_ctx *ctx, int n, const double *x, double *y);
 int lgh_test_singular(lgh_ctx *ctx, int dim, int n, const double *A, double *sv_min);
+int lgh_test_vec_copy(lgh_ctx *ctx, double *y, const double *x, long n);
 
 #ifdef __cplusplus
 }
diff --git a/laghos_amd/_lib.py b/laghos_amd/_lib.py
--- a/laghos_amd/_lib.py
+++ b/laghos_amd/_lib.py
@@ -64,6 +64,9 @@
     "lgh_cg_solve": (_I, [_P, _I, _P, _P, _D, _I, c_int_p]),
     "lgh_l2_mass_solve_local": (_I, [_P, _P, _P]),
     "lgh_qupdate": (_I, [_P, _P]),
+    "lgh_qupdate_state": (_I, [_P, _P]),
+    "lgh_hydro_mult": (_I, [_P, _P, _P, _P, _P, _P, _P, _I, _D, _I, c_int_p, c_int_p]),
+    "lgh_test_vec_copy": (_I, [_P, _P, _P, _L]),
     "lgh_solve_velocity": (_I, [_P, _P, _P, _P, _P, _P, _D, _I, c_int_p]),
     "lgh_solve_energy": (_I, [_P, _P, _P, _P, _P, _P, _D, _I, c_int_p]),
     "lgh_solve_energy_begin": (_I, [_P, _P, _P, _P, _P, _P, _D, _I]),
diff --git a/laghos_amd/context.py b/laghos_amd/context.py
--- a/laghos_amd/context.py
+++ b/laghos_amd/context.py
@@ -515,6 +515,19 @@
         check(self.lib.lgh_solve_energy_end(self.h, ctypes.byref(it)))
         return it.value
 
+    def qupdate_state(self, S):
+        check(self.lib.lgh_qupdate_state(self.h, _ptr(S)))
+
+    def hydro_mult(self, S, dS, rhs, work, e_rhs, rel_tol, max_iter, e_source=None, qdata_current=False):
+        h1, l2 = ctypes.c_int(0), ctypes.c_int(0)
+        check(self.lib.lgh_hydro_mult(self.h, _ptr(S), _ptr(dS), _ptr(rhs), _ptr(work), _ptr(e_rhs),
+                                      _ptr(e_source) if e_source is not None else None, 1 if qdata_current else 0,
+                                      rel_tol, max_iter, ctypes.byref(h1), ctypes.byref(l2)))
+        return h1.value, l2.value
+
+    def test_vec_copy(self, y, x, n):
+        check(self.lib.lgh_test_vec_copy(self.h, _ptr(y), _ptr(x), int(n)))
+
     def vec_axpby(self, z, a, x, b, y):
         check(self.lib.lgh_vec_axpby(self.h, _ptr(z), a, _ptr(x), b, _ptr(y), z.numel()))
 
diff --git a/laghos_amd/csrc/lgh_api.hip b/laghos_amd/csrc/lgh_api.hip
--- a/laghos_amd/csrc/lgh_api.hip
+++ b/laghos_amd/csrc/lgh_api.hip
@@ -865,17 +865,27 @@
    return l2_solve_local_1d(c, b, x);
 }
 
-int lgh_qupdate(lgh_ctx *c, const double *S)
-{
-   LGH_CHECK_ARG(c && S);
+}
+namespace lgh
+{
+int qupdate_region(lgh_ctx *c, const double *S, const bool snapshot)
+{
    RoctxRange range("QUpdate-UpdateQuadratureData");
    timer_start(c);
    kt_begin(c, LGH_KERNEL_QUPDATE);
-   int rc = (c->dim == 1) ? qupdate_1d(c, S) : qupdate(c, S);
+   int rc = (c->dim == 1) ? qupdate_1d(c, S) : qupdate(c, S, snapshot);
    kt_end(c, LGH_KERNEL_QUPDATE);
    timer_stop(c, 3);
    c->timers.c[2] += c->NE;
    return rc;
+}
+}
+extern "C"
+{
+int lgh_qupdate(lgh_ctx *c, const double *S)
+{
+   LGH_CHECK_ARG(c && S);
+   return qupdate_region(c, S, true);
 }
 
 __global__ void __launch_bounds__(256) not_all_ones_k(const double *x, const long n, int *flag)
@@ -911,6 +921,12 @@
                        double *rhs_h1, double *work_B, double rel_tol, int max_iter, int *h1_iters)
 {
    LGH_CHECK_ARG(c && S && dS_dt && rhs_h1 && work_B);
+   return solve_velocity(c, S, dS_dt, one_l2, rhs_h1, work_B, rel_tol, max_iter, h1_iters, false);
+}
+}
+int lgh::solve_velocity(lgh_ctx *c, const double *S, double *dS_dt, const double *one_l2, double *rhs_h1, double *work_B, double rel_tol,
+                        int max_iter, int *h1_iters, const bool rhs_is_scratch)
+{
    const int dim = c->dim, N = c->N;
    double *dv = dS_dt + c->H1V;
    int rc;
@@ -942,7 +958,7 @@
       }
       int its[3] = {0, 0, 0};
       RoctxRange range("SolveVelocity-CGVMass");
-      rc = vcg_solve(c, rhs_h1, dv, rel_tol, max_iter, its, force_E);
+      rc = vcg_solve(c, rhs_h1, dv, rel_tol, max_iter, its, force_E, !rhs_is_scratch);
       if (rc) { return rc; }
       for (int cc = 0; cc < dim; cc++)
       {
@@ -1024,6 +1040,8 @@
    }
    return LGH_OK;
 }
+extern "C"
+{
 
 int lgh_vec_set(lgh_ctx *c, double *y, double a, long n) { LGH_CHECK_ARG(c && y); return vec_set(c, y, a, n); }
 int lgh_vec_copy(lgh_ctx *c, double *y, const double *x, long n)
diff --git a/laghos_amd/csrc/lgh_common.hpp b/laghos_amd/csrc/lgh_common.hpp
--- a/laghos_amd/csrc/lgh_common.hpp
+++ b/laghos_amd/csrc/lgh_common.hpp
@@ -183,6 +183,7 @@
    bool polled = false;
    int iters = 0;
    struct { const double *S, *v; double *dS, *e_rhs; const double *src; double tol; int maxit; } args = {};
+   bool stage = false;
 };
 
 struct CtxHandles
@@ -509,7 +510,7 @@
 int mass_data(lgh_ctx *c, const double **Dq, int *dqs, const double **Se);
 int l2_mass_form(lgh_ctx *c, int *form, int *compact);
 int vcg_solve(lgh_ctx *c, double *B, double *X, double rel_tol, int max_iter, int iters[3],
-              const double *force_E = nullptr);
+              const double *force_E = nullptr, bool store_b = true);
 bool vcg_fused_init_ok(const lgh_ctx *c);
 int partition_nodes_by_cost(lgh_ctx *c, int W, DevPtr<int> &out, const std::vector<int> *valence = nullptr);
 int make_ellz(lgh_ctx *c, DevPtr<unsigned> &out, const int *ell = nullptr, int deg = 0);
@@ -549,7 +550,15 @@
 int cg_solve(lgh_ctx *c, int space, const double *b, double *x, double rel_tol, int max_iter,
              int *iters, bool x_is_zero);
 int stress_on_hand(lgh_ctx *c, const char *who);
-int qupdate(lgh_ctx *c, const double *S);
+int qupdate(lgh_ctx *c, const double *S, bool snapshot = true);
+int qupdate_region(lgh_ctx *c, const double *S, bool snapshot);
+int solve_velocity(lgh_ctx *c, const double *S, double *dS_dt, const double *one_l2, double *rhs_h1, double *work_B, double rel_tol,
+                   int max_iter, int *h1_iters, bool rhs_is_scratch);
+int solve_energy(lgh_ctx *c, const double *S, const double *v_h1, double *dS_dt, double *e_rhs, const double *e_source, double rel_tol,
+                 int max_iter, int *l2_iters, bool stage);
+int solve_energy_begin(lgh_ctx *c, const double *S, const double *v_h1, double *dS_dt, double *e_rhs, const double *e_source,
+                       double rel_tol, int max_iter, bool stage);
+int vec_copy(lgh_ctx *c, double *y, const double *x, long n);
 int setup_rho0detj0(lgh_ctx *c, const double *x0, const double *rho0_l2, const double *rho0_q,
                     double *volume);
 int interp_energy(lgh_ctx *c, int which, const double *vec, double *result);
diff --git a/laghos_amd/csrc/lgh_energy.hip b/laghos_amd/csrc/lgh_energy.hip
--- a/laghos_amd/csrc/lgh_energy.hip
+++ b/laghos_amd/csrc/lgh_energy.hip
@@ -64,10 +64,22 @@
    }
 };
 
-static int energy_rhs(lgh_ctx *c, const double *v_h1, double *e_rhs)
+static int energy_rhs(lgh_ctx *c, const double *v_h1, double *e_rhs, const bool stage)
 {
    RoctxRange range("SolveEnergy-ForcePA");
-   if (c->erhs_q && c->fused_ftv_valid)
+   if (c->erhs_q && c->fused_ftv_valid == 2)
+   {
+      if (stage) { return vec_copy(c, e_rhs, c->erhs_q, c->L2V); }
+      if (!c->stress_current)
+      {
+         set_error("lgh_solve_energy: F^T v on hand belongs to the state of a stage call (lgh_hydro_mult, lgh_qupdate_state) and the "
+                   "stress was kept in registers (lgh_qupdate_store_stress(ctx, 0)): a separately given velocity cannot be served - "
+                   "call lgh_qupdate first");
+         return LGH_ERR_ARG;
+      }
+      return lgh_force_mult_transpose(c, v_h1, e_rhs);
+   }
+   if (c->erhs_q && c->fused_ftv_valid == 1)
    {
       int *flag = c->dev_flags + (c->on_stream2 ? 2 : 0);
       LGH_HIP_CHECK(hipMemsetAsync(flag, 0, sizeof(int), c->stream));
@@ -88,10 +100,10 @@
    }
    return lgh_force_mult_transpose(c, v_h1, e_rhs);
 }
-static int energy_rhs_with_source(lgh_ctx *c, const double *v_h1, double *e_rhs, const double *e_source)
+static int energy_rhs_with_source(lgh_ctx *c, const double *v_h1, double *e_rhs, const double *e_source, const bool stage)
 {
    timer_start(c);
-   int rc = energy_rhs(c, v_h1, e_rhs);
+   int rc = energy_rhs(c, v_h1, e_rhs, stage);
    timer_stop(c, 2);
    if (rc == LGH_OK && e_source) { rc = vec_axpby(c, e_rhs, 1.0, e_rhs, 1.0, e_source, c->L2V); }
    return rc;
@@ -156,17 +168,9 @@
    return LGH_OK;
 }
 
-}
-
-using namespace lgh;
-
-extern "C"
-{
-
-int lgh_solve_energy(lgh_ctx *c, const double *S, const double *v_h1, double *dS_dt, double *e_rhs,
-                     const double *e_source, double rel_tol, int max_iter, int *l2_iters)
-{
-   LGH_CHECK_ARG(c && S && v_h1 && dS_dt && e_rhs);
+int solve_energy(lgh_ctx *c, const double *S, const double *v_h1, double *dS_dt, double *e_rhs, const double *e_source, double rel_tol,
+                 int max_iter, int *l2_iters, const bool stage)
+{
    (void)S;
    double *de = dS_dt + 2 * (size_t)c->H1V;
    if (c->dim == 1)
@@ -175,7 +179,7 @@
       if (rc1) { return rc1; }
       return solve_energy_1d(c, v_h1, de, e_rhs, e_source, l2_iters);
    }
-   int rc = energy_rhs_with_source(c, v_h1, e_rhs, e_source);
+   int rc = energy_rhs_with_source(c, v_h1, e_rhs, e_source, stage);
    if (rc) { return rc; }
    int it = 0;
    RoctxRange range("SolveEnergy-CGEMass");
@@ -187,18 +191,23 @@
    return LGH_OK;
 }
 
-int lgh_solve_energy_begin(lgh_ctx *c, const double *S, const double *v_h1, double *dS_dt, double *e_rhs,
-                           const double *e_source, double rel_tol, int max_iter)
-{
-   LGH_CHECK_ARG(c && S && v_h1 && dS_dt && e_rhs);
+int solve_energy_begin(lgh_ctx *c, const double *S, const double *v_h1, double *dS_dt, double *e_rhs, const double *e_source,
+                       double rel_tol, int max_iter, const bool stage)
+{
    EnergySolve &e = c->energy;
    e = EnergySolve{};
    e.args = {S, v_h1, dS_dt, e_rhs, e_source, rel_tol, max_iter};
+   e.stage = stage;
    double *de = dS_dt + 2 * (size_t)c->H1V;
    const EnergySolve::Mode mode = energy_mode(c);
+   if (stage && mode != EnergySolve::Overlapped)
+   {
+      const int rc = vec_copy(c, dS_dt, v_h1, c->H1V);
+      if (rc) { return rc; }
+   }
    if (mode == EnergySolve::Lockstep)
    {
-      int rc = energy_rhs_with_source(c, v_h1, e_rhs, e_source);
+      int rc = energy_rhs_with_source(c, v_h1, e_rhs, e_source, stage);
       if (rc == LGH_OK) { rc = cg_l2_begin_lockstep(c, e_rhs, de, rel_tol, max_iter); }
       if (rc) { return rc; }
    }
@@ -212,7 +221,8 @@
       LGH_HIP_CHECK(hipEventRecord(c->ev_fork, c->stream));
       LGH_HIP_CHECK(hipStreamWaitEvent(c->stream2, c->ev_fork, 0));
       Stream2Scope on2(c);
-      int rc = energy_rhs_with_source(c, v_h1, e_rhs, e_source);
+      int rc = stage ? vec_copy(c, dS_dt, v_h1, c->H1V) : LGH_OK;
+      if (rc == LGH_OK) { rc = energy_rhs_with_source(c, v_h1, e_rhs, e_source, stage); }
       if (rc == LGH_OK)
       {
          RoctxRange range("SolveEnergy-CGEMass");
@@ -222,6 +232,26 @@
    }
    e.mode = mode;
    return LGH_OK;
+}
+
+}
+
+using namespace lgh;
+
+extern "C"
+{
+
+int lgh_solve_energy(lgh_ctx *c, const double *S, const double *v_h1, double *dS_dt, double *e_rhs,
+                     const double *e_source, double rel_tol, int max_iter, int *l2_iters)
+{
+   LGH_CHECK_ARG(c && S && v_h1 && dS_dt && e_rhs);
+   return solve_energy(c, S, v_h1, dS_dt, e_rhs, e_source, rel_tol, max_iter, l2_iters, false);
+}
+int lgh_solve_energy_begin(lgh_ctx *c, const double *S, const double *v_h1, double *dS_dt, double *e_rhs,
+                           const double *e_source, double rel_tol, int max_iter)
+{
+   LGH_CHECK_ARG(c && S && v_h1 && dS_dt && e_rhs);
+   return solve_energy_begin(c, S, v_h1, dS_dt, e_rhs, e_source, rel_tol, max_iter, false);
 }
 int lgh_energy_lockstep_stats(lgh_ctx *c, long out[4])
 {
@@ -239,7 +269,7 @@
    switch (e.mode)
    {
       case EnergySolve::Deferred:
-         return lgh_solve_energy(c, e.args.S, e.args.v, e.args.dS, e.args.e_rhs, e.args.src, e.args.tol, e.args.maxit, l2_iters);
+         return solve_energy(c, e.args.S, e.args.v, e.args.dS, e.args.e_rhs, e.args.src, e.args.tol, e.args.maxit, l2_iters, e.stage);
       case EnergySolve::Lockstep:
       {
          const int rc = cg_l2_end_lockstep(c, &it);
diff --git a/laghos_amd/csrc/lgh_qupdate.hip b/laghos_amd/csrc/lgh_qupdate.hip
--- a/laghos_amd/csrc/lgh_qupdate.hip
+++ b/laghos_amd/csrc/lgh_qupdate.hip
@@ -5,7 +5,7 @@
 {
 
 int qupdate_form(lgh_ctx *c);
-int qupdate(lgh_ctx *c, const double *S)
+int qupdate(lgh_ctx *c, const double *S, const bool snapshot)
 {
    QArgs a = q_base(c);
    a.x = S;
@@ -19,9 +19,9 @@
    const int rc = (form == 1) ? launch_qrows(c, a) : launch_q<QMODE_UPDATE>(c, a);
    c->qgen++;
    c->stress_current = (rc == LGH_OK && !keep) ? 1 : 0;
-   c->fused_ftv_valid = (rc == LGH_OK && a.erhs_q && c->v_snap) ? 1 : 0;
+   c->fused_ftv_valid = (rc == LGH_OK && a.erhs_q && c->v_snap) ? (snapshot ? 1 : 2) : 0;
    c->fused_f1_valid = (rc == LGH_OK && a.force_e) ? 1 : 0;
-   if (c->fused_ftv_valid)
+   if (c->fused_ftv_valid == 1)
    {
       LGH_HIP_CHECK(hipMemcpyAsync(c->v_snap, S + c->H1V, sizeof(double) * (size_t)c->H1V, hipMemcpyDeviceToDevice, c->stream));
    }
diff --git a/laghos_amd/csrc/lgh_stage.hip b/laghos_amd/csrc/lgh_stage.hip
--- /dev/null
+++ b/laghos_amd/csrc/lgh_stage.hip
@@ -0,0 +1,76 @@
+#include "lgh_common.hpp"
+
+extern "C"
+{
+
+__global__ void __launch_bounds__(256) vec_copy_k(double *__restrict__ y, const double *__restrict__ x, const long n)
+{
+   const long stride = (long)gridDim.x * blockDim.x, t = (long)blockIdx.x * blockDim.x + threadIdx.x;
+   if (((((uintptr_t)y) | ((uintptr_t)x)) & 15u) == 0)
+   {
+      const double2 *x2 = (const double2 *)x;
+      double2 *y2 = (double2 *)y;
+      for (long i = t; i < n / 2; i += stride) { y2[i] = x2[i]; }
+      if ((n & 1) && t == 0) { y[n - 1] = x[n - 1]; }
+   }
+   else
+   {
+      for (long i = t; i < n; i += stride) { y[i] = x[i]; }
+   }
+}
+
+}
+
+namespace lgh
+{
+
+int vec_copy(lgh_ctx *c, double *y, const double *x, const long n)
+{
+   if (n <= 0) { return LGH_OK; }
+   hipLaunchKernelGGL(vec_copy_k, dim3(grid_for((n + 1) / 2)), dim3(256), 0, c->stream, y, x, n);
+   LGH_HIP_CHECK(hipGetLastError());
+   return LGH_OK;
+}
+
+}
+
+using namespace lgh;
+
+extern "C"
+{
+
+int lgh_qupdate_state(lgh_ctx *c, const double *S)
+{
+   LGH_CHECK_ARG(c && S);
+   return qupdate_region(c, S, false);
+}
+
+int lgh_hydro_mult(lgh_ctx *c, const double *S, double *dS_dt, double *rhs_h1, double *work_B, double *e_rhs, const double *e_source,
+                   int qdata_current, double rel_tol, int max_iter, int *h1_iters, int *l2_iters)
+{
+   LGH_CHECK_ARG(c && S && dS_dt && rhs_h1 && work_B && e_rhs);
+   const double *v = S + c->H1V;
+   if (!(qdata_current && (c->fused_ftv_valid != 0 || c->stress_current)))
+   {
+      const int rc = qupdate_region(c, S, false);
+      if (rc) { return rc; }
+   }
+   int rc = solve_energy_begin(c, S, v, dS_dt, e_rhs, e_source, rel_tol, max_iter, true);
+   if (rc) { return rc; }
+   rc = solve_velocity(c, S, dS_dt, nullptr, rhs_h1, work_B, rel_tol, max_iter, h1_iters, true);
+   if (rc)
+   {
+      if (c->energy.mode == EnergySolve::Overlapped) { (void)hipStreamSynchronize(c->stream2); }
+      c->energy = EnergySolve{};
+      return rc;
+   }
+   return lgh_solve_energy_end(c, l2_iters);
+}
+
+int lgh_test_vec_copy(lgh_ctx *c, double *y, const double *x, long n)
+{
+   LGH_CHECK_ARG(c && (n == 0 || (y && x)) && n >= 0);
+   return vec_copy(c, y, x, n);
+}
+
+}
diff --git a/laghos_amd/csrc/lgh_vcg.hip b/laghos_amd/csrc/lgh_vcg.hip
--- a/laghos_amd/csrc/lgh_vcg.hip
+++ b/laghos_amd/csrc/lgh_vcg.hip
@@ -67,7 +67,7 @@
       }
    }
 }
-template <int DEG>
+template <int DEG, bool STORE_B>
 __global__ void __launch_bounds__(256)
 vcg_init_force_k(const VcgArgs a, const double *__restrict__ FE, const int ND, double *__restrict__ bout, const int *__restrict__ ellc, const int degc)
 {
@@ -95,7 +95,7 @@
          double bv = -s;
          if (a.ess[c] && a.ess[c][n]) { bv = 0.0; }
          const size_t i = (size_t)c * a.N + n;
-         bout[(size_t)c * a.N + (a.ncaller ? a.ncaller[n] : n)] = bv;
+         if (STORE_B) { bout[(size_t)c * a.N + (a.ncaller ? a.ncaller[n] : n)] = bv; }
          a.r[i] = bv;
          a.x[i] = 0.0;
          part[c] = __dmul_rn(bv, di) * bv;
@@ -123,6 +123,7 @@
       }
    }
 }
+template <bool STORE_B>
 __global__ void __launch_bounds__(256)
 vcg_init_force_z_k(const VcgArgs a, const double *__restrict__ FE, const unsigned compb_fe, const unsigned *__restrict__ ellf,
                    double *__restrict__ bout)
@@ -167,7 +168,7 @@
       if (ok)
       {
          const size_t i = (size_t)c * a.N + n;
-         bout[(size_t)c * a.N + (a.ncaller ? a.ncaller[n] : n)] = bv;
+         if (STORE_B) { bout[(size_t)c * a.N + (a.ncaller ? a.ncaller[n] : n)] = bv; }
          a.r[i] = bv;
          a.x[i] = 0.0;
       }
@@ -891,7 +892,7 @@
    int ls_limit, ls_before;
 };
 
-static int vcg_start(lgh_ctx *c, VcgPlan &plan, double *B, const double *force_E)
+static int vcg_start(lgh_ctx *c, VcgPlan &plan, double *B, const double *force_E, const bool store_b)
 {
    VcgArgs &a = plan.a;
    const VcgAux *aux = plan.aux;
@@ -901,8 +902,14 @@
    if (force_E)
    {
       if (!plan.mode.direct) { set_error("vcg_solve: fused init is single-rank, degree <= 8"); return LGH_ERR_ARG; }
-      if (aux->ellf && aux->essbits) { hipLaunchKernelGGL(vcg_init_force_z_k, dim3(nb), dim3(256), 0, c->stream, a, force_E, 8u * (unsigned)c->ND, aux->ellf, B); }
-      else { hipLaunchKernelGGL(vcg_init_force_k<8>, dim3(nb), dim3(256), 0, c->stream, a, force_E, c->ND, B, aux->o_ellc ? aux->o_ellc : c->t_ell, c->t_deg); }
+      const int *ellc = aux->o_ellc ? aux->o_ellc.p : c->t_ell.p;
+      if (aux->ellf && aux->essbits)
+      {
+         if (store_b) { hipLaunchKernelGGL(vcg_init_force_z_k<true>, dim3(nb), dim3(256), 0, c->stream, a, force_E, 8u * (unsigned)c->ND, aux->ellf, B); }
+         else { hipLaunchKernelGGL(vcg_init_force_z_k<false>, dim3(nb), dim3(256), 0, c->stream, a, force_E, 8u * (unsigned)c->ND, aux->ellf, B); }
+      }
+      else if (store_b) { hipLaunchKernelGGL((vcg_init_force_k<8, true>), dim3(nb), dim3(256), 0, c->stream, a, force_E, c->ND, B, ellc, c->t_deg); }
+      else { hipLaunchKernelGGL((vcg_init_force_k<8, false>), dim3(nb), dim3(256), 0, c->stream, a, force_E, c->ND, B, ellc, c->t_deg); }
    }
    else
    {
@@ -1046,7 +1053,7 @@
    return LGH_OK;
 }
 
-int vcg_solve(lgh_ctx *c, double *B, double *X, double rel_tol, int max_iter, int iters[3], const double *force_E)
+int vcg_solve(lgh_ctx *c, double *B, double *X, double rel_tol, int max_iter, int iters[3], const double *force_E, const bool store_b)
 {
    if (!vcg_available(c)) { return LGH_ERR_UNSUPPORTED; }
    VcgPlan plan;
@@ -1061,7 +1068,7 @@
    r.chunk = c->vcg_last > 0 ? c->vcg_last : 8;
    r.ls_limit = m.ls ? std::min(l2_lockstep_limit(c), max_iter) : 0;
    r.ls_before = m.ls ? comm_ranks_before(c) : 0;
-   LGH_VCG_TRY(vcg_start(c, plan, B, force_E));
+   LGH_VCG_TRY(vcg_start(c, plan, B, force_E, store_b));
    for (bool first_look = true;; first_look = false)
    {
       if (!first_look || max_iter <= 0)
diff --git a/laghos_amd/host/laghos_solver.cpp b/laghos_amd/host/laghos_solver.cpp
--- a/laghos_amd/host/laghos_solver.cpp
+++ b/laghos_amd/host/laghos_solver.cpp
@@ -120,14 +120,14 @@
 void LagrangianHydroOperator::Mult(const Vector &S, Vector &dS_dt) const
 {
    UpdateMesh(S);
-   LGH_VERIFY(lgh_vec_copy(ctx, dS_dt.Write(), S.Read() + H1Vsize, H1Vsize));
-   UpdateQuadratureData(S);
    if (source_type == 1) { LGH_VERIFY(lgh_tg_source_2d(ctx, S.Read(), e_source.Write())); }
-   LGH_VERIFY(lgh_solve_energy_begin(ctx, S.Read(), S.Read() + H1Vsize, dS_dt.Write(), e_rhs.Write(),
-                                     source_type == 1 ? e_source.Read() : nullptr, cg_rel_tol, cg_max_iter));
-   SolveVelocity(S, dS_dt);
-   int it = 0;
-   LGH_VERIFY(lgh_solve_energy_end(ctx, &it));
+   unsigned long gen = 0;
+   int f1 = 0, ftv = 0;
+   LGH_VERIFY(lgh_quadrature_generation(ctx, &gen, &f1, &ftv));
+   const bool current = qdata_is_current && gen == qdata_gen;
+   int h1_it = 0, l2_it = 0;
+   LGH_VERIFY(lgh_hydro_mult(ctx, S.Read(), dS_dt.Write(), rhs.Write(), B.Write(), e_rhs.Write(),
+                             source_type == 1 ? e_source.Read() : nullptr, current ? 1 : 0, cg_rel_tol, cg_max_iter, &h1_it, &l2_it));
    qdata_is_current = false;
 }
 
@@ -149,14 +149,17 @@
                                cg_rel_tol, cg_max_iter, &it));
 }
 
-void LagrangianHydroOperator::UpdateQuadratureData(const Vector &S) const
+void LagrangianHydroOperator::UpdateQuadratureData(const Vector &S) const { UpdateQuadratureData(S, false); }
+
+void LagrangianHydroOperator::UpdateQuadratureData(const Vector &S, bool for_mult) const
 {
    unsigned long gen = 0;
    int f1 = 0, ftv = 0;
    LGH_VERIFY(lgh_quadrature_generation(ctx, &gen, &f1, &ftv));
-   if (qdata_is_current && gen == qdata_gen) { return; }
+   if (qdata_is_current && gen == qdata_gen && (for_mult || ftv != 2)) { return; }
    qdata_is_current = true;
-   qupdate->UpdateQuadratureData(S, *qdata);
+   if (for_mult) { LGH_VERIFY(lgh_qupdate_state(ctx, S.Read())); }
+   else { qupdate->UpdateQuadratureData(S, *qdata); }
    LGH_VERIFY(lgh_quadrature_generation(ctx, &gen, &f1, &ftv));
    qdata_gen = gen;
 }
@@ -164,7 +167,7 @@
 double LagrangianHydroOperator::GetTimeStepEstimate(const Vector &S) const
 {
    UpdateMesh(S);
-   UpdateQuadratureData(S);
+   UpdateQuadratureData(S, !solves_in_pieces);
    double dt = qdata->GetDtEst();
    if (disc.part.nranks > 1) { LGH_VERIFY(lgh_allreduce(ctx, &dt, 1)); }
    return dt;
@@ -545,6 +548,7 @@
 void RK2AvgSolver::Init(hydrodynamics::LagrangianHydroOperator &op)
 {
    ODESolver::Init(op);
+   op.SolveInPieces(true);
    V.SetSize(op.H1VSize());
    dS_dt.SetSize(op.Size());
    S0.SetSize(op.Size());
diff --git a/laghos_amd/host/laghos_solver.hpp b/laghos_amd/host/laghos_solver.hpp
--- a/laghos_amd/host/laghos_solver.hpp
+++ b/laghos_amd/host/laghos_solver.hpp
@@ -45,6 +45,8 @@
    std::unique_ptr<QuadratureData> qdata;
    mutable bool qdata_is_current;
    mutable unsigned long qdata_gen = 0;
+   bool solves_in_pieces = false;
+   void UpdateQuadratureData(const Vector &S, bool for_mult) const;
    std::unique_ptr<ForcePAOperator> ForcePA;
    std::unique_ptr<MassPAOperator> VMassPA, EMassPA;
    std::unique_ptr<QUpdate> qupdate;
@@ -70,6 +72,7 @@
    void SolveEnergy(const Vector &S, const Vector &v, Vector &dS_dt) const;
    void UpdateMesh(const Vector &) const {}
    void UpdateQuadratureData(const Vector &S) const;
+   void SolveInPieces(bool on) { solves_in_pieces = on; }
    double GetTimeStepEstimate(const Vector &S) const;
    void ResetTimeStepEstimate() const;
    void ResetQuadratureData() const { qdata_is_current = false; LGH_VERIFY(lgh_reset_quadrature_data(ctx)); }
```

After: 1742 Mdofs*steps/s (median of 2 runs). No clear change (+0.7%).
